# callmeray/PointMVSNet

Hardware: AMD Instinct MI355X
Metric: depth-maps/sec (DTU 640x512, 3 src views, 2 flow iters) (higher is better)
Workload: dtype f32

## Files before the change

include/pointflow_hip.h:

```cpp
#ifndef POINTFLOW_HIP_H_
#define POINTFLOW_HIP_H_

#include <stdint.h>

#ifdef __cplusplus
extern "C" {
#endif

#define PF_OK 0
#define PF_ERR_INVALID_ARG (-1)
#define PF_ERR_UNSUPPORTED (-2)

#define PF_STATUS_BAD_INDEX 1u

#define PF_MAX_VIEWS 8
#define PF_GEMM_TILE 64

#define PF_CAM_KREF_INV 0
#define PF_CAM_RREF_INV 9
#define PF_CAM_TREF 18
#define PF_CAM_MEAN 21
#define PF_CAM_STD 24
#define PF_CAM_VIEWS 27
#define PF_CAM_VIEW_STRIDE 21
#define PF_CAM_FLOATS(V) (PF_CAM_VIEWS + PF_CAM_VIEW_STRIDE * (V))

const char* pf_version(void);
const char* pf_error_string(int code);
int pf_device_info(int* cu_count, int* lds_bytes_per_block, char* arch_host, int arch_len);
int pf_debug_timestamp(long long* slot, void* stream);
int pf_check_status(unsigned* status_host, void* stream);

int pf_gather_knn_forward_f32(const float* feature, const int64_t* index, float* out,
                              int64_t B, int64_t C, int64_t N, int64_t K, void* stream);
int pf_gather_knn_forward_f64(const double* feature, const int64_t* index, double* out,
                              int64_t B, int64_t C, int64_t N, int64_t K, void* stream);
int pf_gather_knn_backward_f32(const float* grad_out, const int64_t* index, float* grad_in,
                               int64_t B, int64_t C, int64_t N, int64_t K, const uint32_t* inv_order,
                               const uint32_t* inv_start, void* stream);
int pf_gather_knn_backward_f64(const double* grad_out, const int64_t* index, double* grad_in,
                               int64_t B, int64_t C, int64_t N, int64_t K, const uint32_t* inv_order,
                               const uint32_t* inv_start, void* stream);

int pf_knn_lattice_f32(const float* xyz, const int64_t* strides_host, int64_t B, int64_t D, int64_t H,
                       int64_t W, int kernel_size, int knn, int64_t* idx_out, uint8_t* code_out,
                       void* stream);

int pf_fetch_forward_f32(const float* maps, const float* pts, const float* K, const float* E, float* out,
                         int64_t B, int64_t V, int64_t C, int64_t H, int64_t W, int64_t N, void* stream);
int pf_fetch_backward_f32(const float* grad_out, const float* pts, const float* K, const float* E,
                          float* grad_maps, int64_t B, int64_t V, int64_t C, int64_t H, int64_t W,
                          int64_t N, void* stream);

int pf_fetch_variance_f32(const float* maps, const float* pts, const float* K, const float* E, float* out,
                          int64_t B, int64_t V, int64_t C, int64_t H, int64_t W, int64_t N,
                          int ref_override, void* stream);
int pf_frustum_variance_f32(const float* maps, const float* kinv, const float* rinv, const float* t,
                            const float* depths, const float* K, const float* E, float* out, float* world,
                            int64_t B, int64_t V, int64_t C, int64_t H, int64_t W, int64_t D, void* stream);

int pf_frustum_variance_cl_f32(const float* maps_cl, const float* kinv, const float* rinv, const float* t,
                               const float* depths, const float* K, const float* E, float* out, float* world,
                               int64_t B, int64_t V, int64_t C, int64_t H, int64_t W, int64_t D, void* stream);
int pf_nchw_to_nhwc_f32(const float* in, float* out, int64_t P, int64_t C, int64_t S, void* stream);

int pf_resize_bilinear_f32(const float* in, float* out, int64_t P, int64_t IH, int64_t IW, int64_t OH,
                           int64_t OW, void* stream);

int pf_flow_pyramid_f32(const float* in1, int c1, int h1, int w1, const float* in2, int c2, int h2, int w2,
                        const float* in3, int c3, int h3, int w3, int V, int h, int w, float* out1, float* out2,
                        float* out3, const float* const* in_scale, const float* const* in_shift, void* stream);

int pf_flow_features_f32(const float* maps1, const float* maps2, const float* maps3, int c1, int c2, int c3,
                         int V, int h, int w, const float* depth_in, int dh, int dw, const float* interval,
                         const float* cam, int ratio, float* feature, float* xyz, void* stream);

int pf_stat_blocks(int G, int Ng);
int pf_gemm_blocks(int G, int Ng);

int pf_bn_finalize_f32(const double* partials, int T, int pcols, int col0, int C, double count,
                       double unbias_n, const float* gamma, const float* beta, float* running_mean,
                       float* running_var, float momentum, float eps, int G, int groups_per_stat,
                       float* scale, float* shift, int ld_affine, void* stream);

typedef struct pf_bn_job {
  const double* partials;
  int32_t T, pcols, col0, C;
  double count, unbias_n;
  const float* gamma;
  const float* beta;
  float* running_mean;
  float* running_var;
  float momentum, eps;
  int32_t G, groups_per_stat;
  float* scale;
  float* shift;
  int32_t ld_affine;
  int32_t rows4;
} pf_bn_job;
int pf_bn_finalize_jobs_f32(const pf_bn_job* jobs, int njobs, void* stream);


int pf_pointwise_gemm_f32(const float* X, int x_point_major, int64_t ldx, const float* Wt, float* Y,
                          int64_t ldy, int G, int Ng, int K, int Nc, int Nc_store, const float* in_scale,
                          const float* in_shift, const pf_bn_job* in_bn, int groups_per_stat, double* col_partials,
                          void* stream);

int pf_edge_stats_f32(const float* LE, int64_t ldle, int C, const int64_t* idx, int k, int G, int Ng,
                      double* partials, const uint8_t* codes, int lat_ks, int lat_h, int lat_w, void* stream);


int pf_edge_apply_f32(const float* LE, int64_t ldle, int C, const int64_t* idx, int k, int G, int Ng,
                      const float* scale, const float* shift, int ld_affine, int groups_per_stat,
                      int concat, float* Y, int64_t ldy, const uint8_t* codes, int lat_ks, int lat_h, int lat_w,
                      void* stream);

int pf_edge_backward_reduce_f32(const float* LE, int64_t ldle, int C, const int64_t* idx, int k, int G, int Ng,
                                const float* grad_y, int64_t ldg, const float* scale, const float* shift,
                                const float* mean, const float* invstd, int ld_affine, int groups_per_stat,
                                int concat, double* partials, void* stream);
int pf_edge_backward_apply_f32(const float* LE, int64_t ldle, int C, const int64_t* idx, int k, int G, int Ng,
                               const float* grad_y, int64_t ldg, const float* scale, const float* shift,
                               const float* mean, const float* invstd, const float* c1, const float* c2,
                               int ld_affine, int groups_per_stat, int concat, float* grad_le,
                               const uint32_t* inv_order, const uint32_t* inv_start, void* stream);

int pf_edge_backward_sums_f32(const float* LE, int64_t ldle, int C, const int64_t* idx, int k, int G, int Ng,
                              const float* grad_y, int64_t ldg, const float* scale, const float* shift,
                              const float* mean, const float* invstd, int ld_affine, int groups_per_stat, int concat,
                              double* partials, float* grad_le, float* grad_acc, int64_t ld_acc, int plane,
                              void* stream);
int pf_edge_backward_finish_f32(const float* LE, int64_t ldle, int C, int k, int G, int Ng, const float* grad_y,
                                int64_t ldg, const float* scale, const float* shift, const float* mean,
                                const float* invstd, const float* c1, const float* c2, int ld_affine,
                                int groups_per_stat, int concat, float* grad_le, const uint32_t* inv_order,
                                const uint32_t* inv_start, int plane, void* stream);

int pf_edge_backward_coeffs_f32(const double* partials, int G, int T, int cbn, int C, int concat, int groups_per_stat,
                                int Ng, int k, float* c1, float* c2, float* dgamma, float* dbeta, int accumulate,
                                void* stream);

int64_t pf_knn_inverse_workspace(int G, int Ng, int k);
int pf_knn_inverse(const int64_t* idx, int k, int G, int Ng, uint32_t* order, uint32_t* start, void* workspace,
                   int64_t workspace_bytes, void* stream);

int pf_norm_blocks(int64_t S);
int pf_channel_stats_f32(const float* x, int64_t N, int64_t C, int64_t S, double* partials, void* stream);
int pf_channel_affine_f32(const float* x, float* y, const float* scale, const float* shift, int64_t N, int64_t C,
                          int64_t S, int samples_per_stat, int relu, void* stream);
int pf_channel_bn_apply_f32(const float* x, float* y, const double* partials, int T, int64_t N, int64_t C, int64_t S,
                            int samples_per_stat, double count, const float* gamma, const float* beta,
                            float* running_mean, float* running_var, float momentum, float eps, int relu,
                            const float* addend, void* stream);
int pf_channel_bn_apply2_f32(const float* x1, const double* partials1, int T1, const float* gamma1, const float* beta1,
                             float* running_mean1, float* running_var1, float momentum1, float eps1, const float* x2,
                             const double* partials2, int T2, const float* gamma2, const float* beta2,
                             float* running_mean2, float* running_var2, float momentum2, float eps2, float* y, int64_t N,
                             int64_t C, int64_t S, int samples_per_stat, double count, void* stream);
int pf_channel_bn_fused_f32(const float* x, float* y, int64_t N, int64_t C, int64_t S, int samples_per_stat,
                            const float* gamma, const float* beta, float* running_mean, float* running_var,
                            float momentum, float eps, int relu, float* scale, float* shift, int ld_affine,
                            void* stream);

int pf_conv3d_blocks(int64_t Cin, int64_t Cout, int64_t Di, int64_t Hi, int64_t Wi, int stride);
int pf_conv3d_k3_f32(const float* x, const float* wp, float* y, int64_t N, int64_t Cin, int64_t Cout, int64_t Di,
                     int64_t Hi, int64_t Wi, int stride, const float* in_scale, const float* in_shift,
                     const pf_bn_job* in_bn, int samples_per_stat, double* partials, void* stream);
int pf_conv3d_pair_blocks(int64_t Cin, int64_t Cout, int64_t D, int64_t H, int64_t W);
int pf_conv3d_k3_pair_f32(const float* x, const float* wp, float* y, int64_t N, int64_t Cin, int64_t Cout, int64_t D,
                          int64_t H, int64_t W, double* partials, void* stream);
int pf_conv3d_k3_few_f32(const float* x, const float* w, float* y, int64_t N, int64_t Cin, int64_t Cout, int64_t D,
                         int64_t H, int64_t W, void* stream);

int pf_deconv3d_blocks(int64_t D, int64_t H, int64_t W);
int pf_deconv3d_k3s2_f32(const float* xa, const float* xb, const float* w, float* y, int64_t N, int64_t Cin,
                         int64_t Cout, int64_t D, int64_t H, int64_t W, const float* in_scale, const float* in_shift,
                         const pf_bn_job* in_bn, int samples_per_stat, double* partials, void* stream);

int pf_conv3d_bottom_supported(int64_t Cin, int64_t Cout, int stride);
int pf_conv3d_bottom_blocks(int64_t Di, int64_t Hi, int64_t Wi, int stride);
int pf_conv3d_bottom_f32(const float* x, const float* wp, float* y, int64_t N, int64_t Cin, int64_t Cout, int64_t Di,
                         int64_t Hi, int64_t Wi, int stride, const float* in_scale, const float* in_shift,
                         const pf_bn_job* in_bn, int samples_per_stat, double* partials, void* stream);
int pf_deconv3d_bottom_supported(int64_t Cin, int64_t Cout);
int pf_deconv3d_bottom_blocks(int64_t Di, int64_t Hi, int64_t Wi);
int pf_deconv3d_bottom_f32(const float* x, const float* wp, float* y, int64_t N, int64_t Cin, int64_t Cout, int64_t Di,
                           int64_t Hi, int64_t Wi, const float* in_scale, const float* in_shift, const pf_bn_job* in_bn,
                           int samples_per_stat, double* partials, void* stream);

int pf_conv2d_wide_supported(int64_t Cin, int64_t Cout, int kernel_size, int stride);
int pf_conv2d_wide_blocks(int64_t Cout, int64_t Hi, int64_t Wi, int stride);
int pf_conv2d_wide_f32(const float* x, const float* wp, float* y, int64_t N, int64_t Cin, int64_t Cout, int64_t Hi,
                       int64_t Wi, int kernel_size, int stride, const float* in_scale, const float* in_shift,
                       const pf_bn_job* in_bn, int samples_per_stat, double* partials, int out_channel_last,
                       void* stream);
int pf_conv2d_wide_sets_f32(const float* x, int x_layout, const float* wp, int64_t wp_set_stride, int sets, float* y,
                            int64_t N, int64_t Cin, int64_t Cout, int64_t Hi, int64_t Wi, int kernel_size, int stride,
                            const float* in_scale, const float* in_shift, const pf_bn_job* in_bn, int samples_per_stat,
                            double* partials, int out_channel_last, void* stream);

int pf_flow_head_f32(const float* Z, int64_t ldz, const float* scale, const float* shift, int ld_affine,
                     const pf_bn_job* in_bn, const float* w_out, const float* depth_in, int dh, int dw,
                     const float* interval, int h, int w, int ratio, float* flow_prob, float* depth_out,
                     void* stream);

int pf_softargmin_prob_f32(const float* cost, const float* params, float* depth, float* prob, int64_t B,
                           int64_t D, int64_t HW, void* stream);

int pf_eval_pack_map_f32(const float* src, float* dst, int h, int w, int flip_rows, void* stream);
int pf_eval_flow_prob_f32(const float* prob, float* dst, int h, int w, int flip_rows, void* stream);
int pf_eval_prob_filter_f32(const float* depth, const float* flow_conf, const float* init_conf, int h, int w, int ih,
                            int iw, float flow_threshold, float init_threshold, float* dst, int flip_rows,
                            void* stream);

#define PF_FUSE_VIEW_FLOATS 12
#define PF_FUSE_PAIR_FLOATS 16
int pf_fuse_stage_a_f32(const float* depth, const unsigned char* colour, const float* view_maps, const float* pair_maps,
                        int V, int h, int w, float disp_threshold, float depth_min, float depth_max, int* count,
                        float* point, unsigned char* colour_out, int* match, void* stream);
int pf_fuse_mark(const int* count, const int* match, unsigned char* used, unsigned char* emit, int V, int view, int h,
                 int w, int num_consistent, void* stream);
int pf_fuse_compact_f32(const unsigned char* emit, const int64_t* rank, const float* point, const unsigned char* colour,
                        int64_t n, int64_t rows, float* out_point, unsigned char* out_colour, void* stream);

#define PF_CLOUD_MAX_CELLS 131072
#define PF_CLOUD_MAX_POINTS 2000000000
int pf_cloud_cell_keys_f32(const float* points, int64_t n, float ox, float oy, float oz, float edge, int nx, int ny, int nz,
                           int64_t* keys, void* stream);
int pf_cloud_pack_f32(const float* points, const int64_t* order, int64_t n, int hashed, void* packed, void* stream);
int pf_cloud_thin_round(const void* packed, const int64_t* keys, int64_t n, int nx, int ny, int nz, float t,
                        const unsigned char* state_in, unsigned char* state_out, int* pending, void* stream);
int pf_cloud_nn_cells_f32(const float* query, int64_t nq, const void* packed, const int64_t* keys, int64_t nt, float ox,
                          float oy, float oz, float edge, int nx, int ny, int nz, int rings, float max_dist, float* dist,
                          int* index, unsigned char* done, void* stream);
int pf_cloud_nn_wave_f32(const float* query, const int64_t* todo, int64_t ntodo, int64_t nq, const void* packed,
                         const int64_t* keys, int64_t nt, float ox, float oy, float oz, float edge, int nx, int ny, int nz,
                         float max_dist, float* dist, int* index, void* stream);
int pf_cloud_obs_mask_f32(const float* points, int64_t n, const unsigned char* mask, int X, int Y, int Z, float bx, float by,
                          float bz, float res, unsigned char* inside, void* stream);
int pf_cloud_above_plane_f32(const float* points, int64_t n, float a, float b, float c, float d, unsigned char* above,
                             void* stream);

#define PF_PREPROCESS_TILE_X 256
int pf_preprocess_resize_u8(const unsigned char* src, int V, int h_src, int w_src, const int* xi, const float* xw,
                            const int* yi, const float* yw, int H, int W, int span, unsigned char* ref,
                            unsigned long long* sums, void* stream);
int pf_preprocess_standardise_f32(const unsigned char* ref, const unsigned long long* sums, int V, int H, int W,
                                  float* out, void* stream);

#define PF_SCAN_NEAREST 0
#define PF_SCAN_BILINEAR 1
#define PF_SCAN_CUBIC 2
#define PF_SCAN_LANCZOS4 4
#define PF_SCAN_FILTER_TILE_X 32
#define PF_SCAN_FILTER_TILE_Y 8
int pf_scan_filter_supported(int mode, int h, int w, int fh, int fw, int ih, int iw);
int pf_scan_filter_f32(const float* depth, const float* flow_prob, const float* flow_conf, int fh, int fw,
                       const float* init_conf, int ih, int iw, int V, int h, int w, int mode, const int* flow_ys,
                       const float* flow_yw, const int* flow_xs, const float* flow_xw, const int* init_ys,
                       const float* init_yw, const int* init_xs, const float* init_xw, float flow_threshold,
                       float init_threshold, float* filtered, int* kept, float* flow_resized, float* init_resized,
                       void* stream);

int pf_bn_train_rows_f32(const double* partials, int T, int pcols, int col0, int C, double count, double unbias_n,
                         const float* gamma, const float* beta, float* running_mean, float* running_var,
                         float momentum, float eps, int G, int groups_per_stat, float* rows, int ld_rows, int col_out,
                         int ch0, void* stream);
int pf_bn_bwd_reduce_f32(const float* g, const float* y, const float* rows, int64_t N, int64_t C, int64_t S,
// ... 100 lines not shown
```

pointmvsnet_amd/_lib.py:

```python
import ctypes
import os

import torch

_HERE = os.path.dirname(os.path.abspath(__file__))
LIB_PATH = os.environ.get("PF_LIB_PATH") or os.path.join(_HERE, "libpointflow_hip.so")

_vp, _i, _i64, _f, _d = ctypes.c_void_p, ctypes.c_int, ctypes.c_int64, ctypes.c_float, ctypes.c_double



class BnJob(ctypes.Structure):
    _fields_ = [("partials", _vp), ("T", ctypes.c_int32), ("pcols", ctypes.c_int32), ("col0", ctypes.c_int32),
                ("C", ctypes.c_int32), ("count", _d), ("unbias_n", _d), ("gamma", _vp), ("beta", _vp),
                ("running_mean", _vp), ("running_var", _vp), ("momentum", _f), ("eps", _f),
                ("G", ctypes.c_int32), ("groups_per_stat", ctypes.c_int32), ("scale", _vp), ("shift", _vp),
                ("ld_affine", ctypes.c_int32), ("rows4", ctypes.c_int32)]


class WgradItem(ctypes.Structure):
    _fields_ = [("gr", _vp), ("x", _vp)] + [(n, _i64) for n in ("N", "Cg", "Cx", "Do", "Ho", "Wo", "Di", "Hi", "Wi")] + \
               [(n, ctypes.c_int32) for n in ("KD", "KH", "KW", "stride", "pd", "ph", "pw", "x_samples_per_stat")] + \
               [("x_scale", _vp), ("x_shift", _vp), ("workspace", _vp), ("workspace_bytes", _i64)] + \
               [(n, _i64) for n in ("rows_P", "ldg", "ldx", "x_rows_per_stat")]


PROTOTYPES = {
    "pf_version": ([], ctypes.c_char_p),
    "pf_error_string": ([_i], ctypes.c_char_p),
    "pf_device_info": ([ctypes.POINTER(_i), ctypes.POINTER(_i), ctypes.c_char_p, _i], _i),
    "pf_debug_timestamp": ([_vp, _vp], _i),
    "pf_check_status": ([ctypes.POINTER(ctypes.c_uint), _vp], _i),
    "pf_gather_knn_forward_f32": ([_vp, _vp, _vp, _i64, _i64, _i64, _i64, _vp], _i),
    "pf_gather_knn_forward_f64": ([_vp, _vp, _vp, _i64, _i64, _i64, _i64, _vp], _i),
    "pf_gather_knn_backward_f32": ([_vp, _vp, _vp, _i64, _i64, _i64, _i64, _vp, _vp, _vp], _i),
    "pf_gather_knn_backward_f64": ([_vp, _vp, _vp, _i64, _i64, _i64, _i64, _vp, _vp, _vp], _i),
    "pf_knn_lattice_f32": ([_vp, ctypes.POINTER(_i64), _i64, _i64, _i64, _i64, _i, _i, _vp, _vp, _vp], _i),
    "pf_fetch_forward_f32": ([_vp, _vp, _vp, _vp, _vp, _i64, _i64, _i64, _i64, _i64, _i64, _vp], _i),
    "pf_fetch_backward_f32": ([_vp, _vp, _vp, _vp, _vp, _i64, _i64, _i64, _i64, _i64, _i64, _vp], _i),
    "pf_fetch_variance_f32": ([_vp, _vp, _vp, _vp, _vp, _i64, _i64, _i64, _i64, _i64, _i64, _i, _vp], _i),
    "pf_frustum_variance_f32": ([_vp, _vp, _vp, _vp, _vp, _vp, _vp, _vp, _vp, _i64, _i64, _i64, _i64, _i64, _i64, _vp], _i),
    "pf_frustum_variance_cl_f32": ([_vp, _vp, _vp, _vp, _vp, _vp, _vp, _vp, _vp, _i64, _i64, _i64, _i64, _i64, _i64, _vp], _i),
    "pf_nchw_to_nhwc_f32": ([_vp, _vp, _i64, _i64, _i64, _vp], _i),
    "pf_resize_bilinear_f32": ([_vp, _vp, _i64, _i64, _i64, _i64, _i64, _vp], _i),
    "pf_flow_pyramid_f32": ([_vp, _i, _i, _i, _vp, _i, _i, _i, _vp, _i, _i, _i, _i, _i, _i, _vp, _vp, _vp,
                             ctypes.POINTER(_vp), ctypes.POINTER(_vp), _vp], _i),
    "pf_flow_features_f32": ([_vp, _vp, _vp, _i, _i, _i, _i, _i, _i, _vp, _i, _i, _vp, _vp, _i, _vp, _vp, _vp], _i),
    "pf_stat_blocks": ([_i, _i], _i),
    "pf_gemm_blocks": ([_i, _i], _i),
    "pf_pointwise_gemm_f32": ([_vp, _i, _i64, _vp, _vp, _i64, _i, _i, _i, _i, _i, _vp, _vp, ctypes.POINTER(BnJob), _i,
                               _vp, _vp], _i),
    "pf_conv3d_blocks": ([_i64, _i64, _i64, _i64, _i64, _i], _i),
    "pf_conv3d_k3_f32": ([_vp, _vp, _vp, _i64, _i64, _i64, _i64, _i64, _i64, _i, _vp, _vp, ctypes.POINTER(BnJob), _i,
                          _vp, _vp], _i),
    "pf_conv3d_pair_blocks": ([_i64, _i64, _i64, _i64, _i64], _i),
    "pf_conv3d_k3_pair_f32": ([_vp, _vp, _vp, _i64, _i64, _i64, _i64, _i64, _i64, _vp, _vp], _i),
    "pf_conv3d_k3_few_f32": ([_vp, _vp, _vp, _i64, _i64, _i64, _i64, _i64, _i64, _vp], _i),
    "pf_deconv3d_blocks": ([_i64, _i64, _i64], _i),
    "pf_deconv3d_k3s2_f32": ([_vp, _vp, _vp, _vp, _i64, _i64, _i64, _i64, _i64, _i64, _vp, _vp, ctypes.POINTER(BnJob), _i,
                              _vp, _vp], _i),
    "pf_conv3d_bottom_supported": ([_i64, _i64, _i], _i),
    "pf_conv3d_bottom_blocks": ([_i64, _i64, _i64, _i], _i),
    "pf_conv3d_bottom_f32": ([_vp, _vp, _vp, _i64, _i64, _i64, _i64, _i64, _i64, _i, _vp, _vp, ctypes.POINTER(BnJob), _i,
                              _vp, _vp], _i),
    "pf_deconv3d_bottom_supported": ([_i64, _i64], _i),
    "pf_deconv3d_bottom_blocks": ([_i64, _i64, _i64], _i),
    "pf_deconv3d_bottom_f32": ([_vp, _vp, _vp, _i64, _i64, _i64, _i64, _i64, _i64, _vp, _vp, ctypes.POINTER(BnJob), _i,
                                _vp, _vp], _i),
    "pf_conv2d_wide_supported": ([_i64, _i64, _i, _i], _i),
    "pf_conv2d_wide_blocks": ([_i64, _i64, _i64, _i], _i),
    "pf_conv2d_wide_f32": ([_vp, _vp, _vp, _i64, _i64, _i64, _i64, _i64, _i, _i, _vp, _vp, ctypes.POINTER(BnJob), _i,
                            _vp, _i, _vp], _i),
    "pf_conv2d_wide_sets_f32": ([_vp, _i, _vp, _i64, _i, _vp, _i64, _i64, _i64, _i64, _i64, _i, _i, _vp, _vp,
                                 ctypes.POINTER(BnJob), _i, _vp, _i, _vp], _i),
    "pf_norm_blocks": ([_i64], _i),
    "pf_channel_stats_f32": ([_vp, _i64, _i64, _i64, _vp, _vp], _i),
    "pf_channel_affine_f32": ([_vp, _vp, _vp, _vp, _i64, _i64, _i64, _i, _i, _vp], _i),
    "pf_channel_bn_apply_f32": ([_vp, _vp, _vp, _i, _i64, _i64, _i64, _i, _d, _vp, _vp, _vp, _vp, _f, _f, _i, _vp, _vp], _i),
    "pf_channel_bn_apply2_f32": ([_vp, _vp, _i, _vp, _vp, _vp, _vp, _f, _f, _vp, _vp, _i, _vp, _vp, _vp, _vp, _f, _f, _vp,
                                  _i64, _i64, _i64, _i, _d, _vp], _i),
    "pf_channel_bn_fused_f32": ([_vp, _vp, _i64, _i64, _i64, _i, _vp, _vp, _vp, _vp, _f, _f, _i, _vp, _vp, _i, _vp], _i),
    "pf_edge_stats_f32": ([_vp, _i64, _i, _vp, _i, _i, _i, _vp, _vp, _i, _i, _i, _vp], _i),
    "pf_edge_backward_reduce_f32": ([_vp, _i64, _i, _vp, _i, _i, _i, _vp, _i64, _vp, _vp, _vp, _vp, _i, _i, _i, _vp, _vp], _i),
    "pf_edge_backward_apply_f32": ([_vp, _i64, _i, _vp, _i, _i, _i, _vp, _i64, _vp, _vp, _vp, _vp, _vp, _vp, _i, _i, _i,
                                    _vp, _vp, _vp, _vp], _i),
    "pf_edge_backward_sums_f32": ([_vp, _i64, _i, _vp, _i, _i, _i, _vp, _i64, _vp, _vp, _vp, _vp, _i, _i, _i, _vp, _vp, _vp,
                                   _i64, _i, _vp], _i),
    "pf_edge_backward_finish_f32": ([_vp, _i64, _i, _i, _i, _i, _vp, _i64, _vp, _vp, _vp, _vp, _vp, _vp, _i, _i, _i,
                                     _vp, _vp, _vp, _i, _vp], _i),
    "pf_knn_inverse_workspace": ([_i, _i, _i], _i64),
    "pf_knn_inverse": ([_vp, _i, _i, _i, _vp, _vp, _vp, _i64, _vp], _i),
    "pf_bn_finalize_f32": ([_vp, _i, _i, _i, _i, _d, _d, _vp, _vp, _vp, _vp, _f, _f, _i, _i, _vp, _vp, _i, _vp], _i),
    "pf_bn_finalize_jobs_f32": ([ctypes.POINTER(BnJob), _i, _vp], _i),
    "pf_edge_apply_f32": ([_vp, _i64, _i, _vp, _i, _i, _i, _vp, _vp, _i, _i, _i, _vp, _i64, _vp, _i, _i, _i, _vp], _i),
    "pf_flow_head_f32": ([_vp, _i64, _vp, _vp, _i, ctypes.POINTER(BnJob), _vp, _vp, _i, _i, _vp, _i, _i, _i, _vp, _vp,
                          _vp], _i),
    "pf_eval_pack_map_f32": ([_vp, _vp, _i, _i, _i, _vp], _i),
    "pf_eval_flow_prob_f32": ([_vp, _vp, _i, _i, _i, _vp], _i),
    "pf_eval_prob_filter_f32": ([_vp, _vp, _vp, _i, _i, _i, _i, _f, _f, _vp, _i, _vp], _i),
    "pf_fuse_stage_a_f32": ([_vp, _vp, _vp, _vp, _i, _i, _i, _f, _f, _f, _vp, _vp, _vp, _vp, _vp], _i),
    "pf_fuse_mark": ([_vp, _vp, _vp, _vp, _i, _i, _i, _i, _i, _vp], _i),
    "pf_fuse_compact_f32": ([_vp, _vp, _vp, _vp, _i64, _i64, _vp, _vp, _vp], _i),
    "pf_cloud_cell_keys_f32": ([_vp, _i64, _f, _f, _f, _f, _i, _i, _i, _vp, _vp], _i),
    "pf_cloud_pack_f32": ([_vp, _vp, _i64, _i, _vp, _vp], _i),
    "pf_cloud_thin_round": ([_vp, _vp, _i64, _i, _i, _i, _f, _vp, _vp, _vp, _vp], _i),
    "pf_cloud_nn_cells_f32": ([_vp, _i64, _vp, _vp, _i64, _f, _f, _f, _f, _i, _i, _i, _i, _f, _vp, _vp, _vp, _vp], _i),
    "pf_cloud_nn_wave_f32": ([_vp, _vp, _i64, _i64, _vp, _vp, _i64, _f, _f, _f, _f, _i, _i, _i, _f, _vp, _vp, _vp], _i),
    "pf_cloud_obs_mask_f32": ([_vp, _i64, _vp, _i, _i, _i, _f, _f, _f, _f, _vp, _vp], _i),
    "pf_cloud_above_plane_f32": ([_vp, _i64, _f, _f, _f, _f, _vp, _vp], _i),
    "pf_preprocess_resize_u8": ([_vp, _i, _i, _i, _vp, _vp, _vp, _vp, _i, _i, _i, _vp, _vp, _vp], _i),
    "pf_preprocess_standardise_f32": ([_vp, _vp, _i, _i, _i, _vp, _vp], _i),
    "pf_scan_filter_supported": ([_i] * 7, _i),
    "pf_scan_filter_f32": ([_vp, _vp, _vp, _i, _i, _vp, _i, _i, _i, _i, _i, _i] + [_vp] * 8 + [_f, _f, _vp, _vp, _vp, _vp, _vp], _i),
    "pf_softargmin_prob_f32": ([_vp, _vp, _vp, _vp, _i64, _i64, _i64, _vp], _i),
    "pf_bn_train_rows_f32": ([_vp, _i, _i, _i, _i, _d, _d, _vp, _vp, _vp, _vp, _f, _f, _i, _i, _vp, _i, _i, _i, _vp], _i),
    "pf_bn_bwd_reduce_f32": ([_vp, _vp, _vp, _i64, _i64, _i64, _i, _i, _vp, _vp], _i),
    "pf_softargmin_backward_f32": ([_vp, _vp, _vp, _vp, _vp, _i64, _i64, _i64, _vp], _i),
    "pf_flow_head_train_f32": ([_vp, _i64, _vp, _vp, _i64, _vp, _vp, _vp], _i),
    "pf_flow_head_backward_workspace": ([_i64], _i64),
    "pf_flow_head_backward_f32": ([_vp, _i64, _vp, _vp, _vp, _vp, _i64, _vp, _vp, _i, _vp, _i64, _vp], _i),
    "pf_rmsprop_f32": ([_vp, _vp, _vp, _vp, _i64, _f, _f, _f, _vp], _i),
    "pf_masked_mae_f32": ([_vp, _vp, _vp, _i, _i, _i, _i, _i, _f, _vp, _vp, _vp], _i),
    "pf_masked_mae_backward_f32": ([_vp, _vp, _vp, _vp, _i, _i, _i, _i, _i, _vp, _vp], _i),
    "pf_wgrad_reduce_batch_f32": ([_vp, _vp, _vp, _vp, _vp, _vp, _vp, _i, _i, _vp], _i),
    "pf_conv_wgrad_batch_f32": ([ctypes.POINTER(WgradItem), _i, _vp], _i),
    "pf_bn_bwd_apply_fused_f32": ([_vp, _vp, _vp, _vp, _i, _d, _vp, _i64, _i64, _i64, _i, _i, _vp, _vp, _i, _vp], _i),
    "pf_bn_bwd_plane_supported": ([_i64, _i], _i),
    "pf_bn_bwd_plane_f32": ([_vp, _vp, _vp, _i64, _i64, _i64, _i, _vp, _vp, _vp, _i, _vp], _i),
    "pf_edge_backward_coeffs_f32": ([_vp, _i, _i, _i, _i, _i, _i, _i, _i, _vp, _vp, _vp, _vp, _i, _vp], _i),
    "pf_bn_bwd_coeffs_f32": ([_vp, _i, _i, _i, _i, _d, _i, _i, _vp, _vp, _vp, _vp, _i, _vp], _i),
    "pf_bn_bwd_apply_f32": ([_vp, _vp, _vp, _vp, _vp, _i64, _i64, _i64, _i, _i, _vp], _i),
    "pf_rows_bn_blocks": ([_i, _i], _i),
    "pf_rows_bn_bwd_reduce_f32": ([_vp, _i64, _vp, _i64, _vp, _i, _i, _i, _i, _i, _vp, _vp], _i),
    "pf_rows_bn_bwd_apply_f32": ([_vp, _i64, _vp, _i64, _vp, _vp, _vp, _i64, _i, _i, _i, _i, _i, _vp], _i),
    "pf_rows_affine_f32": ([_vp, _i64, _vp, _vp, _i64, _i, _i, _i, _i, _i, _vp], _i),
    "pf_conv_wgrad_workspace": ([_i64] * 9 + [_i] * 4, _i64),
    "pf_conv_wgrad_f32": ([_vp, _vp, _vp] + [_i64] * 9 + [_i] * 7 + [_vp, _vp, _i, _vp, _i64, _i, _vp], _i),
    "pf_conv_wgrad_plan": ([_i64] * 9 + [_i] * 4 + [ctypes.POINTER(_i)], _i),
    "pf_rows_wgrad_plan": ([_i64, _i, _i, ctypes.POINTER(_i)], _i),
    "pf_rows_wgrad_workspace": ([_i64, _i, _i], _i64),
    "pf_rows_wgrad_f32": ([_vp, _i64, _vp, _i64, _vp, _i64, _i, _i, _vp, _vp, _i64, _vp, _i64, _i, _vp], _i),
    "pf_deconv2d_k5s2_supported": ([_i64, _i64], _i),
    "pf_deconv2d_k5s2_f32": ([_vp, _vp, _vp, _i64, _i64, _i64, _i64, _i64, _vp], _i),
    "pf_conv3d_k3_c1_f32": ([_vp, _vp, _vp, _i64, _i64, _i64, _i64, _i64, _vp], _i),
    "pf_sort_pairs_workspace": ([_i64, _i64], _i64),
    "pf_sort_pairs_by_key": ([_vp, _i64, _i64, _vp, _vp, _vp, _i64, _vp], _i),
    "pf_warp_taps_flow_f32": ([_vp, _vp, _vp, _i, _i, _i, _vp, _vp, _vp], _i),
    "pf_warp_taps_frustum_f32": ([_vp, _vp, _vp, _vp, _vp, _vp, _i, _i, _i, _i, _i, _vp, _vp, _vp], _i),
    "pf_variance_grad_f32": ([_vp, _i, _vp, _i, _vp, _i, _i, _i, _i, _i64, _vp, _vp, _vp, _i64, _i, _vp, _vp], _i),
    "pf_warp_gather_f32": ([_vp, _vp, _vp, _vp, _i, _i, _i, _i, _i, _vp, _vp], _i),
    "pf_flow_depth_grad_f32": ([_vp, _i64, _i, _vp, _i, _i, _vp, _vp], _i),
    "pf_resize_bilinear_backward_f32": ([_vp, _i, _i, _i, _i, _i, _i, _i, _i, _vp, _vp], _i),
    "pf_pack_desc_bytes": ([], _i),
    "pf_pack_gather_f32": ([_vp, _i, ctypes.c_longlong, _vp], _i),
}

_lib = None


def load():
    global _lib
    if _lib is not None:
        return _lib
    if not os.path.exists(LIB_PATH):
        raise RuntimeError(
            "pointmvsnet_amd: %s is missing. Build it with `python -m pointmvsnet_amd.build` "
            "(hipcc --offload-arch=gfx950). There is no CPU or eager fallback for the hot path." % LIB_PATH)
    try:
        lib = ctypes.CDLL(LIB_PATH)
    except OSError as exc:
        raise RuntimeError("pointmvsnet_amd: cannot load %s: %s" % (LIB_PATH, exc))
    for name, (argtypes, restype) in PROTOTYPES.items():
        fn = getattr(lib, name)
        fn.argtypes = argtypes
        fn.restype = restype
    _lib = lib
    return lib


def check(code, what=""):
    if code != 0:
        msg = load().pf_error_string(int(code)).decode()
        raise RuntimeError("pointflow_hip %s failed (%d): %s" % (what, code, msg))


def ptr(t):
    return None if t is None else ctypes.c_void_p(t.data_ptr())


def stream():
    return ctypes.c_void_p(torch._C._cuda_getCurrentRawStream(torch._C._cuda_getDevice()))


class _NoGuard(object):
    def __enter__(self):
        return None

    def __exit__(self, *exc):
        return False


_NO_GUARD = _NoGuard()


def on_device(dev):
    if dev.index is None or dev.index == torch._C._cuda_getDevice():
        return _NO_GUARD
    return torch.cuda.device(dev)


def require_gpu(*tensors):
    for t in tensors:
        if t is not None and not t.is_cuda:
            raise RuntimeError("pointmvsnet_amd: expected a GPU (HIP) tensor; this operator has no CPU path")


def status():
    val = ctypes.c_uint(0)
    check(load().pf_check_status(ctypes.byref(val), stream()), "pf_check_status")
    return int(val.value)


class KernelTimer(object):

    def __init__(self, only=None):
        self.only = only
        self.records = []

    def wants(self, name):
        return self.only is None or name == self.only

    @staticmethod
    def _pair_overhead_ms():
        vals = []
        for _ in range(21):
# ... 57 lines not shown
```

pointmvsnet_amd/csrc/edgeconv.hip:

```cpp
#include <stdlib.h>

#include "pf_common.h"
#include "pf_bn_resolve.h"

namespace {

typedef float f32x16 __attribute__((ext_vector_type(16)));

constexpr int TILE = PF_GEMM_TILE;

constexpr int GT = 128;
constexpr int LDA = GT + 2;

template <bool POINT_MAJOR, int NT>
__global__ __launch_bounds__(256, 2) void pointwise_gemm_kernel(
    const float* __restrict__ X, int64_t ldx, const float* __restrict__ Wt, float* __restrict__ Y, int64_t ldy,
    int Ng, int K, int Nc_store, const float* __restrict__ in_scale, const float* __restrict__ in_shift,
    int groups_per_stat, double* __restrict__ partials, int T) {
  constexpr int NC = NT * 32;
  constexpr int KC = NT == 4 ? 16 : 32;
  constexpr int NA = KC * GT / 256;
  constexpr int NW = KC * NC / 256;
  __shared__ __attribute__((aligned(16))) float As[2][KC][LDA];
  __shared__ __attribute__((aligned(16))) float Ws[2][KC][NC];
// ... 248 lines not shown
          av[3] = fmaxf(fmaf(av[3], s1.w, s0.w), 0.0f);
        }
#pragma unroll
        for (int i = 0; i < 4; ++i)
#pragma unroll
          for (int t = 0; t < NT; ++t)
            acc[t] = __builtin_amdgcn_mfma_f32_32x32x2f32(av[i], bcur[i][t], acc[t], 0, 0, 0);
#pragma unroll
        for (int i = 0; i < 4; ++i)
#pragma unroll
          for (int t = 0; t < NT; ++t) bcur[i][t] = bnxt[i][t];
        __builtin_amdgcn_sched_barrier(0);
      }
    }
  };

  float4 a0[J0], a1[J1 > 0 ? J1 : 1];
  if (tb < tiles) load_half(row_ptr(tb), a0, 0, J0);
  for (int tile = tb; tile < tiles; tile += T) {
    const int n0 = tile * GT + 32 * wave;
    const int rows = min(32, Ng - n0);
    f32x16 acc[NT];
#pragma unroll
    for (int t = 0; t < NT; ++t)
#pragma unroll
      for (int q = 0; q < 16; ++q) acc[t][q] = 0.0f;
    if (J1 > 0) load_half(row_ptr(tile), a1, J0, J1);
    mma_half(a0, 0, J0, acc);
    if (tile + T < tiles) load_half(row_ptr(tile + T), a0, 0, J0);
    if (J1 > 0) mma_half(a1, J0, J1, acc);
    if (rows > 0) {
      float* yrow = Y + ((int64_t)g * Ng + n0 + 4 * hi) * ldy + lo;
#pragma unroll
      for (int t = 0; t < NT; ++t) {
        const int col = 32 * t + lo;
        float cs = 0.0f, cq = 0.0f;
        if (rows == 32) {
#pragma unroll
          for (int q = 0; q < 16; ++q) {
            const float v = acc[t][q];
            if (col < Nc_store) yrow[(int64_t)((q & 3) + 8 * (q >> 2)) * ldy + 32 * t] = v;
            cs += v;
            cq += v * v;
          }
        } else {
#pragma unroll
          for (int q = 0; q < 16; ++q) {
            const int row = (q & 3) + 8 * (q >> 2) + 4 * hi;
            const float v = acc[t][q];
            if (row < rows) {
              if (col < Nc_store) yrow[(int64_t)((q & 3) + 8 * (q >> 2)) * ldy + 32 * t] = v;
              cs += v;
              cq += v * v;
            }
          }
        }
        csum[t] += (double)cs;
        csq[t] += (double)cq;
      }
    }
  }

  if (partials != nullptr) {
    __syncthreads();
#pragma unroll
    for (int t = 0; t < NT; ++t) {
      double s = csum[t], q = csq[t];
      s += __shfl_xor(s, 32);
      q += __shfl_xor(q, 32);
      if (lane < 32) {
        red[((wave * NC) + 32 * t + lane) * 2 + 0] = s;
        red[((wave * NC) + 32 * t + lane) * 2 + 1] = q;
      }
    }
    __syncthreads();
    if (tid < NC) {
      double s = 0.0, q = 0.0;
#pragma unroll
      for (int w = 0; w < 4; ++w) {
        s += red[((w * NC) + tid) * 2 + 0];
        q += red[((w * NC) + tid) * 2 + 1];
      }
      double* o = partials + (((int64_t)g * T + tb) * NC + tid) * 2;
      o[0] = s;
      o[1] = q;
    }
  }
}

__device__ __forceinline__ float4 ld4(const float* p) { return *reinterpret_cast<const float4*>(p); }

template <int C, int K>
__device__ __forceinline__ void gather_rows(const float* __restrict__ LE, int64_t ldle, const int64_t* __restrict__ ip,
                                            int64_t gbase, int Ng, int q, float4 (&e)[K], bool& bad) {
  long long ii[K];
  static_assert(K % 2 == 0, "K must be even");
#pragma unroll
  for (int j = 0; j < K / 2; ++j) {
    const longlong2 v = *reinterpret_cast<const longlong2*>(ip + 2 * j);
    ii[2 * j] = v.x;
    ii[2 * j + 1] = v.y;
  }
#pragma unroll
  for (int j = 0; j < K; ++j) {
    long long i = ii[j];
    if (i < 0 || i >= Ng) {
      bad = true;
      i = i < 0 ? 0 : Ng - 1;
    }
    e[j] = ld4(LE + (gbase + i) * ldle + C + 4 * q);
  }
}

struct Lattice {
  int ks, H, W;
  int band;
};

__device__ __forceinline__ int xcd_tile(int tb, const Lattice& lat) {
  if (lat.band == 0) return tb;
  const int x = tb & 7, j = tb >> 3;
  const int d = j / lat.band, o = j - d * lat.band;
  return d * (lat.band * 8) + x * lat.band + o;
}

__device__ __forceinline__ void build_code_lut(int* lut, const Lattice& lat) {
  const int hk = lat.ks >> 1, k2 = lat.ks * lat.ks;
  for (int c = threadIdx.x; c < 256; c += blockDim.x) {
    int off = 0;
    if (c < k2 * lat.ks) {
      const int pd = c / k2, rem = c - pd * k2, ph = rem / lat.ks, pw = rem - ph * lat.ks;
      off = (pd - hk) * lat.H * lat.W + (ph - hk) * lat.W + (pw - hk);
    }
    lut[c] = off;
  }
  __syncthreads();
}

template <int C>
__device__ __forceinline__ void gather_rows_codes(const float* __restrict__ LE, int64_t ldle,
                                                  const uint8_t* __restrict__ cp, const int* lut, int64_t gbase, int n,
                                                  int Ng, int q, float4 (&e)[16]) {
  const uint4 cw = *reinterpret_cast<const uint4*>(cp);
  const unsigned w[4] = {cw.x, cw.y, cw.z, cw.w};
#pragma unroll
  for (int j = 0; j < 16; ++j) {
    const int code = (int)((w[j >> 2] >> (8 * (j & 3))) & 255u);
    int i = n + lut[code];
    i = i < 0 ? 0 : (i > Ng - 1 ? Ng - 1 : i);
    e[j] = ld4(LE + (gbase + i) * ldle + C + 4 * q);
  }
}

template <int C, int K>
__global__ __launch_bounds__(256) void edge_stats_kernel(const float* __restrict__ LE, int64_t ldle,
                                                         const int64_t* __restrict__ idx, int k, int Ng,
                                                         double* __restrict__ partials, int T,
                                                         unsigned* __restrict__ status,
                                                         const uint8_t* __restrict__ codes, Lattice lat) {
  constexpr int Q = C / 4;
  constexpr int PPB = 256 / Q;
  __shared__ double red[256 * 8];
  __shared__ int lut[256];
  if (K == 16 && codes != nullptr) build_code_lut(lut, lat);
  const int tid = threadIdx.x;
  const int q = tid % Q, pl = tid / Q;
  const int g = blockIdx.y, tb = blockIdx.x;
  const int tiles = (Ng + TILE - 1) / TILE;
  const int64_t gbase = (int64_t)g * Ng;
  double ds[4] = {0, 0, 0, 0}, dq[4] = {0, 0, 0, 0};
  bool bad = false;
  const int tile0 = xcd_tile(tb, lat);
  for (int tile = tile0; tile < tiles; tile += T) {
    const int n0 = tile * TILE;
    for (int p = pl; p < TILE; p += PPB) {
      const int n = n0 + p;
      if (n >= Ng) break;
      const int64_t row = gbase + n;
      const float4 l = ld4(LE + row * ldle + 4 * q);
      const int64_t* ip = idx + row * k;
      float4 s = {0, 0, 0, 0}, s2 = {0, 0, 0, 0};
      if constexpr (K > 0) {
        float4 e[K > 0 ? K : 1];
        if constexpr (K == 16) {
          if (codes != nullptr) gather_rows_codes<C>(LE, ldle, codes + row * 16, lut, gbase, n, Ng, q, e);
          else gather_rows<C, 16>(LE, ldle, ip, gbase, Ng, q, e, bad);
        } else {
          gather_rows<C, (K > 0 ? K : 2)>(LE, ldle, ip, gbase, Ng, q, e, bad);
        }
#pragma unroll
        for (int j = 0; j < K; ++j) {
          const float dx = e[j].x - l.x, dy = e[j].y - l.y, dz = e[j].z - l.z, dw = e[j].w - l.w;
          s.x += dx; s.y += dy; s.z += dz; s.w += dw;
          s2.x += dx * dx; s2.y += dy * dy; s2.z += dz * dz; s2.w += dw * dw;
        }
      } else {
        for (int j = 0; j < k; ++j) {
          int64_t i = ip[j];
          if (i < 0 || i >= Ng) {
            bad = true;
            i = i < 0 ? 0 : Ng - 1;
          }
          const float4 e = ld4(LE + (gbase + i) * ldle + C + 4 * q);
          const float dx = e.x - l.x, dy = e.y - l.y, dz = e.z - l.z, dw = e.w - l.w;
          s.x += dx; s.y += dy; s.z += dz; s.w += dw;
          s2.x += dx * dx; s2.y += dy * dy; s2.z += dz * dz; s2.w += dw * dw;
        }
      }
      ds[0] += (double)s.x; ds[1] += (double)s.y; ds[2] += (double)s.z; ds[3] += (double)s.w;
      dq[0] += (double)s2.x; dq[1] += (double)s2.y; dq[2] += (double)s2.z; dq[3] += (double)s2.w;
    }
  }
  if (bad) atomicOr(status, PF_STATUS_BAD_INDEX);
#pragma unroll
  for (int c = 0; c < 4; ++c) {
    red[tid * 8 + c] = ds[c];
    red[tid * 8 + 4 + c] = dq[c];
  }
  __syncthreads();
  if (tid < 2 * C) {
    const int qq = tid / 8, comp = tid % 8;
    double acc = 0.0;
    for (int s = 0; s < PPB; ++s) acc += red[(s * Q + qq) * 8 + comp];
    double* o = partials + (((int64_t)g * T + tile0) * C + 4 * qq + (comp & 3)) * 2 + (comp >> 2);
    *o = acc;
  }
}

template <int C, int K>
__global__ __launch_bounds__(256) void edge_apply_kernel(const float* __restrict__ LE, int64_t ldle,
                                                         const int64_t* __restrict__ idx, int k, int Ng,
                                                         const float* __restrict__ scale,
                                                         const float* __restrict__ shift, int ld_affine,
                                                         int groups_per_stat, int concat, float* __restrict__ Y,
                                                         int64_t ldy, int T, const uint8_t* __restrict__ codes,
                                                         Lattice lat) {
  constexpr int Q = C / 4;
  constexpr int PPB = 256 / Q;
  __shared__ int lut[256];
  if (K == 16 && codes != nullptr) build_code_lut(lut, lat);
  const int tid = threadIdx.x;
  const int q = tid % Q, pl = tid / Q;
  const int g = blockIdx.y, tb = blockIdx.x;
  const int tiles = (Ng + TILE - 1) / TILE;
  const int64_t gbase = (int64_t)g * Ng;
  const int64_t so = (int64_t)(g / groups_per_stat) * ld_affine;
  const int doff = concat ? C : 0;
  const float4 dsc = ld4(scale + so + doff + 4 * q), dsh = ld4(shift + so + doff + 4 * q);
  float4 csc = {0, 0, 0, 0}, csh = {0, 0, 0, 0};
  if (concat) {
    csc = ld4(scale + so + 4 * q);
    csh = ld4(shift + so + 4 * q);
  }
  const float kf = (float)k;
  bool bad = false;
  for (int tile = xcd_tile(tb, lat); tile < tiles; tile += T) {
    const int n0 = tile * TILE;
    for (int p = pl; p < TILE; p += PPB) {
      const int n = n0 + p;
      if (n >= Ng) break;
      const int64_t row = gbase + n;
      const float4 l = ld4(LE + row * ldle + 4 * q);
      const int64_t* ip = idx + row * k;
      float4 a = {0, 0, 0, 0};
      if constexpr (K > 0) {
        float4 e[K > 0 ? K : 1];
        if constexpr (K == 16) {
          if (codes != nullptr) gather_rows_codes<C>(LE, ldle, codes + row * 16, lut, gbase, n, Ng, q, e);
          else gather_rows<C, 16>(LE, ldle, ip, gbase, Ng, q, e, bad);
        } else {
          gather_rows<C, (K > 0 ? K : 2)>(LE, ldle, ip, gbase, Ng, q, e, bad);
        }
#pragma unroll
        for (int j = 0; j < K; ++j) {
          a.x += fmaxf(fmaf(e[j].x - l.x, dsc.x, dsh.x), 0.0f);
          a.y += fmaxf(fmaf(e[j].y - l.y, dsc.y, dsh.y), 0.0f);
          a.z += fmaxf(fmaf(e[j].z - l.z, dsc.z, dsh.z), 0.0f);
          a.w += fmaxf(fmaf(e[j].w - l.w, dsc.w, dsh.w), 0.0f);
        }
      } else {
        for (int j = 0; j < k; ++j) {
          int64_t i = ip[j];
          i = i < 0 ? 0 : (i >= Ng ? Ng - 1 : i);
          const float4 e = ld4(LE + (gbase + i) * ldle + C + 4 * q);
          a.x += fmaxf(fmaf(e.x - l.x, dsc.x, dsh.x), 0.0f);
          a.y += fmaxf(fmaf(e.y - l.y, dsc.y, dsh.y), 0.0f);
          a.z += fmaxf(fmaf(e.z - l.z, dsc.z, dsh.z), 0.0f);
          a.w += fmaxf(fmaf(e.w - l.w, dsc.w, dsh.w), 0.0f);
        }
      }
      float4 yd = {a.x / kf, a.y / kf, a.z / kf, a.w / kf};
      float* yo = Y + row * ldy + 4 * q;
      if (concat) {
        float4 yc = {fmaxf(fmaf(l.x, csc.x, csh.x), 0.0f), fmaxf(fmaf(l.y, csc.y, csh.y), 0.0f),
                     fmaxf(fmaf(l.z, csc.z, csh.z), 0.0f), fmaxf(fmaf(l.w, csc.w, csh.w), 0.0f)};
        *reinterpret_cast<float4*>(yo) = yc;
        *reinterpret_cast<float4*>(yo + C) = yd;
      } else {
        *reinterpret_cast<float4*>(yo) = yd;
      }
    }
  }
  (void)bad;
}

struct EdgeBwdAffine {
  const float* scale;
  const float* shift;
  const float* mean;
  const float* invstd;
  const float* c1;
  const float* c2;
  int ld, groups_per_stat, concat;
};

template <int C, int K, bool SUMS>
__global__ __launch_bounds__(256) void edge_bwd_reduce_kernel(const float* __restrict__ LE, int64_t ldle,
                                                              const int64_t* __restrict__ idx, int k, int Ng,
                                                              const float* __restrict__ Gy, int64_t ldg,
                                                              EdgeBwdAffine A, double* __restrict__ partials, int T,
                                                              unsigned* __restrict__ status, float* __restrict__ sums,
                                                              float* __restrict__ gacc, int64_t lda, int band) {
  constexpr int Q = C / 4;
  constexpr int PPB = 256 / Q;
  __shared__ double red[256 * 16];
  const int tid = threadIdx.x;
  const int q = tid % Q, pl = tid / Q;
  const int g = blockIdx.y, tb = blockIdx.x;
  const int tiles = (Ng + TILE - 1) / TILE;
  const int64_t gbase = (int64_t)g * Ng;
  const int64_t so = (int64_t)(g / A.groups_per_stat) * A.ld;
  const int doff = A.concat ? C : 0;
  const float4 a = ld4(A.scale + so + doff + 4 * q), b = ld4(A.shift + so + doff + 4 * q);
  const float4 mu = ld4(A.mean + so + doff + 4 * q), is = ld4(A.invstd + so + doff + 4 * q);
  float4 ac = {0, 0, 0, 0}, bc = {0, 0, 0, 0}, muc = {0, 0, 0, 0}, isc = {0, 0, 0, 0};
  if (A.concat) {
    ac = ld4(A.scale + so + 4 * q);
    bc = ld4(A.shift + so + 4 * q);
    muc = ld4(A.mean + so + 4 * q);
    isc = ld4(A.invstd + so + 4 * q);
  }
  const float kf = (float)k;
  double acc[16];
#pragma unroll
  for (int i = 0; i < 16; ++i) acc[i] = 0.0;
  bool bad = false;
  const Lattice xo{0, 1, 1, band};
  const int tile0 = xcd_tile(tb, xo);
  for (int tile = tile0; tile < tiles; tile += T) {
    const int n0 = tile * TILE;
    for (int p = pl; p < TILE; p += PPB) {
      const int n = n0 + p;
      if (n >= Ng) break;
      const int64_t row = gbase + n;
      const float4 l = ld4(LE + row * ldle + 4 * q);
      float4 gy = ld4(Gy + row * ldg + doff + 4 * q);
      if (SUMS && gacc != nullptr) {
        float* ga = gacc + row * lda + doff + 4 * q;
        const float4 h = ld4(ga);
        gy = make_float4(gy.x + h.x, gy.y + h.y, gy.z + h.z, gy.w + h.w);
        *reinterpret_cast<float4*>(ga) = gy;
      }
      const float gd[4] = {gy.x / kf, gy.y / kf, gy.z / kf, gy.w / kf};
      const float lv[4] = {l.x, l.y, l.z, l.w};
      const float av[4] = {a.x, a.y, a.z, a.w}, bv[4] = {b.x, b.y, b.z, b.w};
      const float mv[4] = {mu.x, mu.y, mu.z, mu.w}, iv[4] = {is.x, is.y, is.z, is.w};
      float sg[4] = {0, 0, 0, 0}, sx[4] = {0, 0, 0, 0}, sd[4] = {0, 0, 0, 0};
      const int64_t* ip = idx + row * k;
      auto pair = [&](const float4& e) {
        const float ev[4] = {e.x, e.y, e.z, e.w};
#pragma unroll
        for (int c = 0; c < 4; ++c) {
          const float d = ev[c] - lv[c];
          const float u = fmaf(d, av[c], bv[c]);
          const float gg = u > 0.0f ? gd[c] : 0.0f;
          sg[c] += gg;
          sx[c] += gg * ((d - mv[c]) * iv[c]);
          if (SUMS) sd[c] += d;
        }
      };
      if constexpr (K > 0) {
        float4 e[K > 0 ? K : 1];
        gather_rows<C, (K > 0 ? K : 2)>(LE, ldle, ip, gbase, Ng, q, e, bad);
#pragma unroll
        for (int j = 0; j < K; ++j) pair(e[j]);
      } else {
        for (int j = 0; j < k; ++j) {
          int64_t i = ip[j];
          if (i < 0 || i >= Ng) {
            bad = true;
            i = i < 0 ? 0 : Ng - 1;
          }
          pair(ld4(LE + (gbase + i) * ldle + C + 4 * q));
        }
      }
#pragma unroll
      for (int c = 0; c < 4; ++c) {
        acc[c] += (double)sg[c];
        acc[4 + c] += (double)sx[c];
      }
      if (SUMS) {
        float* o = sums + row * ldle + 4 * q;
        *reinterpret_cast<float4*>(o) = make_float4(sg[0], sg[1], sg[2], sg[3]);
        *reinterpret_cast<float4*>(o + C) = make_float4((sd[0] - kf * mv[0]) * iv[0], (sd[1] - kf * mv[1]) * iv[1],
                                                        (sd[2] - kf * mv[2]) * iv[2], (sd[3] - kf * mv[3]) * iv[3]);
      }
      if (A.concat) {
        float4 gc4 = ld4(Gy + row * ldg + 4 * q);
        if (SUMS && gacc != nullptr) {
          float* ga = gacc + row * lda + 4 * q;
          const float4 h = ld4(ga);
// ... 447 lines not shown
  const float interval = interval_p[0];
#pragma unroll
  for (int d = 0; d < 5; ++d) {
    const float p = e[d] / den;
    flow_prob[(int64_t)d * h * w + i] = p;
    flow += p * ((float)(d - 2) * interval);
  }
  const float scy = (float)dh / (float)h, scx = (float)dw / (float)w;
  int sy = (int)floorf((float)y * scy);
  int sx = (int)floorf((float)x * scx);
  sy = sy > dh - 1 ? dh - 1 : sy;
  sx = sx > dw - 1 ? dw - 1 : sx;
  depth_out[i] = depth_in[sy * dw + sx] + flow;
}

}

extern "C" {

int pf_stat_blocks(int G, int Ng) {
  if (G <= 0 || Ng <= 0) return 0;
  const int tiles = (Ng + TILE - 1) / TILE;
#ifndef PF_STAT_CAP
#define PF_STAT_CAP 4096
#endif
  int cap = PF_STAT_CAP / G;
  cap = cap < 32 ? 32 : cap;
  if (tiles <= cap) return tiles;
  const int per = (tiles + cap - 1) / cap;
  return (tiles + per - 1) / per;
}

int pf_gemm_blocks(int G, int Ng) {
  if (G <= 0 || Ng <= 0) return 0;
  const int tiles = (Ng + GT - 1) / GT;
#ifndef PF_GEMM_CAP
#define PF_GEMM_CAP 512
#endif
  int cap = PF_GEMM_CAP / G;
  cap = cap < 16 ? 16 : cap;
  if (tiles <= cap) return tiles;
  const int per = (tiles + cap - 1) / cap;
  return (tiles + per - 1) / per;
}

static int bn_materialize_rows(const pf_bn_job* in_bn, hipStream_t s) {
  PF_REQUIRE(in_bn->scale != nullptr && in_bn->shift != nullptr && in_bn->ld_affine >= in_bn->C);
  pf_bn_job j = *in_bn;
  j.running_mean = j.running_var = nullptr;
  return pf_bn_finalize_jobs_f32(&j, 1, s);
}

int pf_pointwise_gemm_f32(const float* X, int x_point_major, int64_t ldx, const float* Wt, float* Y, int64_t ldy,
                          int G, int Ng, int K, int Nc, int Nc_store, const float* in_scale,
                          const float* in_shift, const pf_bn_job* in_bn, int groups_per_stat, double* col_partials,
                          void* stream) {
  PF_REQUIRE(in_bn == nullptr || in_scale == nullptr);
  if (in_bn != nullptr && G > 0 && Ng > 0) {
    PF_REQUIRE(groups_per_stat >= 1 && G % groups_per_stat == 0);
    const int rc = pf_bn_in_check(in_bn, K, G / groups_per_stat);
    if (rc != PF_OK && rc != PF_ERR_UNSUPPORTED) return rc;
    const int kj = (K + 7) / 8, nt = Nc / 32;
    const bool shape = (kj == 17 && nt == 2) || (kj == 4 && nt == 2) || (kj == 8 && nt == 4) || (kj == 28 && nt == 2) ||
                       (kj == 8 && nt == 2) || (kj == 8 && nt == 1);
    const bool direct = rc == PF_OK && shape && x_point_major && (K % 4) == 0 && (ldx % 4) == 0 &&
                        kj * 8 * Nc <= 16384 && (reinterpret_cast<uintptr_t>(X) % 16) == 0 && K <= 256;
    if (!direct) {
      const int rc2 = bn_materialize_rows(in_bn, (hipStream_t)stream);
      if (rc2 != PF_OK) return rc2;
      PF_REQUIRE(in_bn->ld_affine == K);
      return pf_pointwise_gemm_f32(X, x_point_major, ldx, Wt, Y, ldy, G, Ng, K, Nc, Nc_store, in_bn->scale,
                                   in_bn->shift, nullptr, groups_per_stat, col_partials, stream);
    }
  }
  PF_REQUIRE(G >= 0 && Ng >= 0 && K >= 1 && Nc >= 32 && Nc_store >= 1 && Nc_store <= Nc);
  PF_REQUIRE(Nc % 32 == 0 && groups_per_stat >= 1);
  if (Nc != 32 && Nc != 64 && Nc != 128) return PF_ERR_UNSUPPORTED;
  PF_REQUIRE((in_scale == nullptr) == (in_shift == nullptr));
  PF_REQUIRE(G <= 65535);
  if (G == 0 || Ng == 0) return PF_OK;
  PF_REQUIRE(X && Wt && Y && ldy >= Nc_store);
  if (x_point_major) PF_REQUIRE(ldx >= K);
  const int T = pf_gemm_blocks(G, Ng);
  dim3 grid((unsigned)T, (unsigned)G);
  hipStream_t s = (hipStream_t)stream;
  {
    const pf_bn_job no_bn = {};
    const int kj = (K + 7) / 8, nt = Nc / 32;
    const bool direct = x_point_major && (K % 4) == 0 && (ldx % 4) == 0 && kj * 8 * Nc <= 16384 &&
                        (reinterpret_cast<uintptr_t>(X) % 16) == 0;
#define PF_GEMM_DIRECT(KJV, NTV)                                                                                   \
  if (direct && kj == KJV && nt == NTV) {                                                                          \
    if (in_bn != nullptr)                                                                                          \
      hipLaunchKernelGGL((pointwise_gemm_direct_kernel<KJV, NTV, 2>), grid, dim3(256), 0, s, X, ldx, Wt, Y, ldy,   \
                         Ng, K, Nc_store, in_scale, in_shift, groups_per_stat, col_partials, T, *in_bn);           \
    else if (in_scale != nullptr)                                                                                  \
      hipLaunchKernelGGL((pointwise_gemm_direct_kernel<KJV, NTV, 1>), grid, dim3(256), 0, s, X, ldx, Wt, Y, ldy,   \
                         Ng, K, Nc_store, in_scale, in_shift, groups_per_stat, col_partials, T, no_bn);            \
    else                                                                                                           \
      hipLaunchKernelGGL((pointwise_gemm_direct_kernel<KJV, NTV, 0>), grid, dim3(256), 0, s, X, ldx, Wt, Y, ldy,   \
                         Ng, K, Nc_store, in_scale, in_shift, groups_per_stat, col_partials, T, no_bn);            \
    return pf_launch_status();                                                                                     \
  }
    PF_GEMM_DIRECT(17, 2)
    PF_GEMM_DIRECT(4, 2)
    PF_GEMM_DIRECT(8, 4)
    PF_GEMM_DIRECT(28, 2)
    PF_GEMM_DIRECT(8, 2)
    PF_GEMM_DIRECT(8, 1)
#undef PF_GEMM_DIRECT
  }
#define PF_GEMM_LAUNCH(PM, NTV)                                                                                  \
  hipLaunchKernelGGL((pointwise_gemm_kernel<PM, NTV>), grid, dim3(256), 0, s, X, ldx, Wt, Y, ldy, Ng, K, Nc_store, \
                     in_scale, in_shift, groups_per_stat, col_partials, T)
  if (x_point_major) {
    if (Nc == 32) PF_GEMM_LAUNCH(true, 1);
    else if (Nc == 64) PF_GEMM_LAUNCH(true, 2);
    else PF_GEMM_LAUNCH(true, 4);
  } else {
    if (Nc == 32) PF_GEMM_LAUNCH(false, 1);
    else if (Nc == 64) PF_GEMM_LAUNCH(false, 2);
    else PF_GEMM_LAUNCH(false, 4);
  }
#undef PF_GEMM_LAUNCH
  return pf_launch_status();
}

static int check_lattice(const int64_t* idx, const uint8_t* codes, int k, int Ng, int lat_ks, int lat_h, int lat_w,
                         Lattice& lat) {
  lat.ks = 0;
  lat.H = lat.W = 1;
  lat.band = 0;
  if (codes == nullptr) {
    PF_REQUIRE(idx != nullptr);
    if (lat_ks == 0 && lat_h >= 1 && lat_w >= 1 && (int64_t)lat_h * lat_w > 1 && Ng % ((int64_t)lat_h * lat_w) == 0) {
      lat.H = lat_h;
      lat.W = lat_w;
    }
    return PF_OK;
  }
  PF_REQUIRE(k == 16 && (lat_ks == 3 || lat_ks == 5) && lat_h >= 1 && lat_w >= 1);
  PF_REQUIRE(Ng % (lat_h * lat_w) == 0);
  lat.ks = lat_ks;
  lat.H = lat_h;
  lat.W = lat_w;
  return PF_OK;
}

static int xcd_band(int64_t plane, int unit, int64_t Ng, int64_t blocks) {
  static const bool on = !(getenv("PF_EDGE_XCD") && atoi(getenv("PF_EDGE_XCD")) == 0);
  if (!on || plane <= 1 || plane % unit != 0 || (plane / unit) % 8 != 0 || Ng % plane != 0 || blocks != Ng / unit) return 0;
  return (int)(plane / unit / 8);
}
static void lattice_band(Lattice& lat, int Ng, int T) { lat.band = xcd_band((int64_t)lat.H * lat.W, TILE, Ng, T); }

int pf_edge_stats_f32(const float* LE, int64_t ldle, int C, const int64_t* idx, int k, int G, int Ng,
                      double* partials, const uint8_t* codes, int lat_ks, int lat_h, int lat_w, void* stream) {
  PF_REQUIRE(G >= 0 && Ng >= 0 && k >= 1 && ldle >= 2 * (int64_t)C && (ldle % 4) == 0 && G <= 65535);
  if (C != 32 && C != 64 && C != 128) return PF_ERR_UNSUPPORTED;
  if (G == 0 || Ng == 0) return PF_OK;
  PF_REQUIRE(LE && partials);
  Lattice lat;
  {
    const int rc = check_lattice(idx, codes, k, Ng, lat_ks, lat_h, lat_w, lat);
    if (rc != PF_OK) return rc;
  }
  unsigned* status = pf_status_ptr();
  PF_REQUIRE(status != nullptr);
  const int T = pf_stat_blocks(G, Ng);
  lattice_band(lat, Ng, T);
  dim3 grid((unsigned)T, (unsigned)G);
  hipStream_t s = (hipStream_t)stream;
#define PF_ES(CV, KV) hipLaunchKernelGGL((edge_stats_kernel<CV, KV>), grid, dim3(256), 0, s, LE, ldle, idx, k, Ng, partials, T, status, codes, lat)
  if (k == 16) {
    if (C == 32) PF_ES(32, 16); else if (C == 64) PF_ES(64, 16); else PF_ES(128, 16);
  } else {
    if (C == 32) PF_ES(32, 0); else if (C == 64) PF_ES(64, 0); else PF_ES(128, 0);
  }
#undef PF_ES
  return pf_launch_status();
}

int pf_bn_finalize_jobs_f32(const pf_bn_job* jobs, int njobs, void* stream) {
  PF_REQUIRE(jobs != nullptr && njobs >= 1 && njobs <= kBnJobs);
  BnJobs packed;
  int cmax = 0;
  for (int i = 0; i < njobs; ++i) {
    const pf_bn_job& j = jobs[i];
    PF_REQUIRE(j.T >= 1 && j.pcols >= 1 && j.col0 >= 0 && j.C >= 1 && j.col0 + j.C <= j.pcols && j.count > 0.0);
    PF_REQUIRE(j.G >= 1 && j.groups_per_stat >= 1 && (j.G % j.groups_per_stat) == 0 && j.ld_affine >= j.C);
    PF_REQUIRE(j.partials && j.gamma && j.beta && j.scale && j.shift);
    PF_REQUIRE((j.running_mean == nullptr) == (j.running_var == nullptr));
    packed.j[i] = j;
    cmax = j.C > cmax ? j.C : cmax;
  }
  for (int i = njobs; i < kBnJobs; ++i) packed.j[i] = jobs[0];
  const int cb = bn_channels_per_block();
  hipLaunchKernelGGL(bn_finalize_kernel, dim3((unsigned)pf_cdiv(cmax, cb), (unsigned)njobs), dim3(kBnThreads), 0,
                     (hipStream_t)stream, packed, cb);
  return pf_launch_status();
}

int pf_bn_finalize_f32(const double* partials, int T, int pcols, int col0, int C, double count, double unbias_n,
                       const float* gamma, const float* beta, float* running_mean, float* running_var,
                       float momentum, float eps, int G, int groups_per_stat, float* scale, float* shift,
                       int ld_affine, void* stream) {
  pf_bn_job j;
  j.partials = partials;
  j.T = T;
  j.pcols = pcols;
  j.col0 = col0;
  j.C = C;
  j.count = count;
  j.unbias_n = unbias_n;
  j.gamma = gamma;
  j.beta = beta;
  j.running_mean = running_mean;
  j.running_var = running_var;
  j.momentum = momentum;
  j.eps = eps;
  j.G = G;
  j.groups_per_stat = groups_per_stat;
  j.scale = scale;
  j.shift = shift;
  j.ld_affine = ld_affine;
  j.rows4 = 0;
  return pf_bn_finalize_jobs_f32(&j, 1, stream);
}

int pf_edge_apply_f32(const float* LE, int64_t ldle, int C, const int64_t* idx, int k, int G, int Ng,
                      const float* scale, const float* shift, int ld_affine, int groups_per_stat, int concat,
                      float* Y, int64_t ldy, const uint8_t* codes, int lat_ks, int lat_h, int lat_w, void* stream) {
  PF_REQUIRE(G >= 0 && Ng >= 0 && k >= 1 && ldle >= 2 * (int64_t)C && (ldle % 4) == 0 && G <= 65535);
  PF_REQUIRE(groups_per_stat >= 1 && (ldy % 4) == 0 && ldy >= (concat ? 2 : 1) * (int64_t)C);
  PF_REQUIRE((ld_affine % 4) == 0 && ld_affine >= (concat ? 2 : 1) * C);
  if (C != 32 && C != 64 && C != 128) return PF_ERR_UNSUPPORTED;
  if (G == 0 || Ng == 0) return PF_OK;
  PF_REQUIRE(LE && scale && shift && Y);
  Lattice lat;
  {
    const int rc = check_lattice(idx, codes, k, Ng, lat_ks, lat_h, lat_w, lat);
    if (rc != PF_OK) return rc;
  }
  const int T = pf_stat_blocks(G, Ng);
  lattice_band(lat, Ng, T);
  dim3 grid((unsigned)T, (unsigned)G);
  hipStream_t s = (hipStream_t)stream;
#define PF_EA(CV, KV)                                                                                         \
  hipLaunchKernelGGL((edge_apply_kernel<CV, KV>), grid, dim3(256), 0, s, LE, ldle, idx, k, Ng, scale, shift, \
                     ld_affine, groups_per_stat, concat, Y, ldy, T, codes, lat)
  if (k == 16) {
    if (C == 32) PF_EA(32, 16); else if (C == 64) PF_EA(64, 16); else PF_EA(128, 16);
  } else {
    if (C == 32) PF_EA(32, 0); else if (C == 64) PF_EA(64, 0); else PF_EA(128, 0);
  }
#undef PF_EA
  return pf_launch_status();
}

extern "C++" {
static int edge_backward_reduce(const float* LE, int64_t ldle, int C, const int64_t* idx, int k, int G, int Ng,
                                const float* grad_y, int64_t ldg, const float* scale, const float* shift,
                                const float* mean, const float* invstd, int ld_affine, int groups_per_stat,
                                int concat, double* partials, float* sums, float* gacc, int64_t lda, int plane,
                                void* stream) {
  PF_REQUIRE(G >= 0 && Ng >= 0 && k >= 1 && ldle >= 2 * (int64_t)C && (ldle % 4) == 0 && G <= 65535);
  PF_REQUIRE(gacc == nullptr || (sums != nullptr && (lda % 4) == 0 && lda >= (concat ? 2 : 1) * (int64_t)C));
  PF_REQUIRE(groups_per_stat >= 1 && (ldg % 4) == 0 && ldg >= (concat ? 2 : 1) * (int64_t)C);
  PF_REQUIRE((ld_affine % 4) == 0 && ld_affine >= (concat ? 2 : 1) * C);
  if (C != 32 && C != 64) return PF_ERR_UNSUPPORTED;
  if (G == 0 || Ng == 0) return PF_OK;
  PF_REQUIRE(LE && idx && grad_y && scale && shift && mean && invstd && partials);
  unsigned* status = pf_status_ptr();
  PF_REQUIRE(status != nullptr);
  const EdgeBwdAffine A{scale, shift, mean, invstd, nullptr, nullptr, ld_affine, groups_per_stat, concat};
  const int T = pf_stat_blocks(G, Ng);
  const int band = xcd_band(plane, TILE, Ng, T);
  dim3 grid((unsigned)T, (unsigned)G);
  hipStream_t s = (hipStream_t)stream;
#define PF_EBR(CV, KV, SV) hipLaunchKernelGGL((edge_bwd_reduce_kernel<CV, KV, SV>), grid, dim3(256), 0, s, LE, ldle, idx, k, Ng, grad_y, ldg, A, partials, T, status, sums, gacc, lda, band)
  if (sums != nullptr) {
    if (k == 16) {
      if (C == 32) PF_EBR(32, 16, true); else PF_EBR(64, 16, true);
    } else {
      if (C == 32) PF_EBR(32, 0, true); else PF_EBR(64, 0, true);
    }
  } else if (k == 16) {
    if (C == 32) PF_EBR(32, 16, false); else PF_EBR(64, 16, false);
  } else {
    if (C == 32) PF_EBR(32, 0, false); else PF_EBR(64, 0, false);
  }
#undef PF_EBR
  return pf_launch_status();
}
}

int pf_edge_backward_reduce_f32(const float* LE, int64_t ldle, int C, const int64_t* idx, int k, int G, int Ng,
                                const float* grad_y, int64_t ldg, const float* scale, const float* shift,
                                const float* mean, const float* invstd, int ld_affine, int groups_per_stat,
                                int concat, double* partials, void* stream) {
  return edge_backward_reduce(LE, ldle, C, idx, k, G, Ng, grad_y, ldg, scale, shift, mean, invstd, ld_affine,
                              groups_per_stat, concat, partials, nullptr, nullptr, 0, 0, stream);
}

int pf_edge_backward_sums_f32(const float* LE, int64_t ldle, int C, const int64_t* idx, int k, int G, int Ng,
                              const float* grad_y, int64_t ldg, const float* scale, const float* shift,
                              const float* mean, const float* invstd, int ld_affine, int groups_per_stat, int concat,
                              double* partials, float* grad_le, float* grad_acc, int64_t ld_acc, int plane,
                              void* stream) {
  PF_REQUIRE(grad_le != nullptr || G == 0 || Ng == 0);
  PF_REQUIRE(plane >= 0);
  return edge_backward_reduce(LE, ldle, C, idx, k, G, Ng, grad_y, ldg, scale, shift, mean, invstd, ld_affine,
                              groups_per_stat, concat, partials, grad_le, grad_acc, ld_acc, plane, stream);
}

extern "C++" {
template <bool FINISH>
static void edge_backward_inverse_launch(const float* LE, int64_t ldle, int C, int k, int G, int Ng, const float* grad_y,
                                         int64_t ldg, const EdgeBwdAffine& A, const uint32_t* inv_order,
                                         const uint32_t* inv_start, float* grad_le, int plane, hipStream_t s) {
  const int64_t rows = (int64_t)G * Ng;
  const int ppb = 256 / (C / 4);
  int64_t blocks = pf_cdiv(rows, ppb);
  if (blocks > 16384) blocks = 16384;
  const int band = G == 1 ? xcd_band(plane, ppb, Ng, blocks) : 0;
  static const int dbg = getenv("PF_EDGE_FINISH_DBG") ? atoi(getenv("PF_EDGE_FINISH_DBG")) : 0;
  if (C == 32)
    hipLaunchKernelGGL((edge_bwd_inverse_kernel<32, FINISH>), dim3((unsigned)blocks), dim3(256), 0, s, LE, ldle, k, Ng,
                       grad_y, ldg, A, inv_order, inv_start, grad_le, rows, dbg, band);
  else
    hipLaunchKernelGGL((edge_bwd_inverse_kernel<64, FINISH>), dim3((unsigned)blocks), dim3(256), 0, s, LE, ldle, k, Ng,
                       grad_y, ldg, A, inv_order, inv_start, grad_le, rows, dbg, band);
}
}

int pf_edge_backward_apply_f32(const float* LE, int64_t ldle, int C, const int64_t* idx, int k, int G, int Ng,
                               const float* grad_y, int64_t ldg, const float* scale, const float* shift,
                               const float* mean, const float* invstd, const float* c1, const float* c2,
                               int ld_affine, int groups_per_stat, int concat, float* grad_le,
                               const uint32_t* inv_order, const uint32_t* inv_start, void* stream) {
  PF_REQUIRE(G >= 0 && Ng >= 0 && k >= 1 && ldle >= 2 * (int64_t)C && (ldle % 4) == 0 && G <= 65535);
  PF_REQUIRE((inv_order == nullptr) == (inv_start == nullptr));
  PF_REQUIRE(groups_per_stat >= 1 && (ldg % 4) == 0 && ldg >= (concat ? 2 : 1) * (int64_t)C);
  PF_REQUIRE((ld_affine % 4) == 0 && ld_affine >= (concat ? 2 : 1) * C);
  if (C != 32 && C != 64) return PF_ERR_UNSUPPORTED;
  if (G == 0 || Ng == 0) return PF_OK;
  PF_REQUIRE(LE && idx && grad_y && scale && shift && mean && invstd && c1 && c2 && grad_le);
  hipStream_t s = (hipStream_t)stream;
  const bool scatter = inv_order == nullptr;
  if (scatter) {
    const int zrc = pf_zero_async(grad_le, sizeof(float) * (size_t)G * Ng * ldle, s);
    if (zrc != PF_OK) return zrc;
  }
  const EdgeBwdAffine A{scale, shift, mean, invstd, c1, c2, ld_affine, groups_per_stat, concat};
  const int T = pf_stat_blocks(G, Ng);
  dim3 grid((unsigned)T, (unsigned)G);
#define PF_EBA(CV, KV, SV) hipLaunchKernelGGL((edge_bwd_apply_kernel<CV, KV, SV>), grid, dim3(256), 0, s, LE, ldle, idx, k, Ng, grad_y, ldg, A, grad_le, T)
  if (scatter) {
    if (k == 16) {
      if (C == 32) PF_EBA(32, 16, true); else PF_EBA(64, 16, true);
    } else {
      if (C == 32) PF_EBA(32, 0, true); else PF_EBA(64, 0, true);
    }
    return pf_launch_status();
  }
  if (k == 16) {
    if (C == 32) PF_EBA(32, 16, false); else PF_EBA(64, 16, false);
  } else {
    if (C == 32) PF_EBA(32, 0, false); else PF_EBA(64, 0, false);
  }
#undef PF_EBA
  edge_backward_inverse_launch<false>(LE, ldle, C, k, G, Ng, grad_y, ldg, A, inv_order, inv_start, grad_le, 0, s);
  return pf_launch_status();
}

int pf_edge_backward_finish_f32(const float* LE, int64_t ldle, int C, int k, int G, int Ng, const float* grad_y,
                                int64_t ldg, const float* scale, const float* shift, const float* mean,
                                const float* invstd, const float* c1, const float* c2, int ld_affine,
                                int groups_per_stat, int concat, float* grad_le, const uint32_t* inv_order,
                                const uint32_t* inv_start, int plane, void* stream) {
  PF_REQUIRE(G >= 0 && Ng >= 0 && k >= 1 && ldle >= 2 * (int64_t)C && (ldle % 4) == 0 && G <= 65535 && plane >= 0);
  PF_REQUIRE(groups_per_stat >= 1 && (ldg % 4) == 0 && ldg >= (concat ? 2 : 1) * (int64_t)C);
  PF_REQUIRE((ld_affine % 4) == 0 && ld_affine >= (concat ? 2 : 1) * C);
  if (C != 32 && C != 64) return PF_ERR_UNSUPPORTED;
  if (G == 0 || Ng == 0) return PF_OK;
  PF_REQUIRE(LE && grad_y && scale && shift && mean && invstd && c1 && c2 && grad_le && inv_order && inv_start);
  const EdgeBwdAffine A{scale, shift, mean, invstd, c1, c2, ld_affine, groups_per_stat, concat};
  edge_backward_inverse_launch<true>(LE, ldle, C, k, G, Ng, grad_y, ldg, A, inv_order, inv_start, grad_le, plane,
                                     (hipStream_t)stream);
  return pf_launch_status();
}

int pf_flow_head_f32(const float* Z, int64_t ldz, const float* scale, const float* shift, int ld_affine,
                     const pf_bn_job* in_bn, const float* w_out, const float* depth_in, int dh, int dw,
                     const float* interval, int h, int w, int ratio, float* flow_prob, float* depth_out,
                     void* stream) {
  PF_REQUIRE(h >= 1 && w >= 1 && dh >= 1 && dw >= 1 && ratio >= 1 && h % ratio == 0 && w % ratio == 0);
  PF_REQUIRE(ldz >= 16 && (ldz % 4) == 0 && (int64_t)h * w <= INT32_MAX);
  PF_REQUIRE(Z && w_out && depth_in && interval && flow_prob && depth_out);
  PF_REQUIRE((in_bn != nullptr) != (scale != nullptr) && (scale == nullptr) == (shift == nullptr));
  dim3 grid((unsigned)pf_cdiv((int64_t)h * w, 256));
  hipStream_t s = (hipStream_t)stream;
  if (in_bn != nullptr) {
// ... 24 lines not shown
```

pointmvsnet_amd/csrc/fetch.hip:

```cpp
#include <type_traits>

#include <stdlib.h>

#include "pf_common.h"

namespace {

__global__ __launch_bounds__(256) void fetch_fwd_kernel(const float* __restrict__ maps,
                                                        const float* __restrict__ pts,
                                                        const float* __restrict__ Kmat,
                                                        const float* __restrict__ Emat, float* __restrict__ out,
                                                        int V, int C, int H, int W, int64_t N) {
  const int64_t n = (int64_t)blockIdx.x * blockDim.x + threadIdx.x;
  const int v = blockIdx.y;
  const int64_t b = blockIdx.z;
  if (n >= N) return;
  const float* pb = pts + b * 3 * N;
  PfTaps t;
  pf_project_taps(pb[n], pb[N + n], pb[2 * N + n], Kmat + (b * V + v) * 9,
                  Emat ? Emat + (b * V + v) * 12 : nullptr, H, W, t);
  const int64_t HW = (int64_t)H * W;
  const float* m = maps + (b * V + v) * C * HW;
  float* o = out + (b * V + v) * C * N + n;
  for (int c = 0; c < C; ++c) o[(int64_t)c * N] = pf_sample(m + (int64_t)c * HW, t);
}

__global__ __launch_bounds__(256) void fetch_bwd_kernel(const float* __restrict__ gout,
                                                        const float* __restrict__ pts,
                                                        const float* __restrict__ Kmat,
                                                        const float* __restrict__ Emat,
                                                        float* __restrict__ gmaps, int V, int C, int H, int W,
                                                        int64_t N) {
  const int64_t n = (int64_t)blockIdx.x * blockDim.x + threadIdx.x;
  const int v = blockIdx.y;
  const int64_t b = blockIdx.z;
  if (n >= N) return;
  const float* pb = pts + b * 3 * N;
  PfTaps t;
  pf_project_taps(pb[n], pb[N + n], pb[2 * N + n], Kmat + (b * V + v) * 9,
                  Emat ? Emat + (b * V + v) * 12 : nullptr, H, W, t);
  const int64_t HW = (int64_t)H * W;
  float* gm = gmaps + (b * V + v) * C * HW;
  const float* g = gout + (b * V + v) * C * N + n;
  for (int c = 0; c < C; ++c) {
    const float go = g[(int64_t)c * N];
    float* plane = gm + (int64_t)c * HW;
#pragma unroll
    for (int k = 0; k < 4; ++k)
      if (t.ok[k]) unsafeAtomicAdd(plane + t.off[k], go * t.wgt[k]);
  }
}

__device__ __forceinline__ float pf_bilerp(float a, float b, float c, float d, float w0, float w1, float w2, float w3) {
  return fmaf(d, w3, fmaf(c, w2, fmaf(b, w1, a * w0)));
}
__device__ __forceinline__ float pf_variance(float s, float s2, float inv_v) {
  const float m1 = s * inv_v;
  return fmaf(-m1, m1, s2 * inv_v);
}

struct Frustum {
  const float* kinv;
  const float* rinv;
  const float* t;
  const float* depths;
  float* world;
  int D;
};

template <int V, bool FRUSTUM>
__global__ __launch_bounds__(256) void fetch_variance_kernel(const float* __restrict__ maps,
                                                             const float* __restrict__ pts, Frustum fr,
                                                             const float* __restrict__ Kmat,
                                                             const float* __restrict__ Emat,
                                                             float* __restrict__ out, int C, int H, int W,
                                                             int64_t N, int ref_override) {
  const int64_t n = (int64_t)blockIdx.x * blockDim.x + threadIdx.x;
  const int64_t b = blockIdx.y;
  if (n >= N) return;
  float X, Y, Z;
  if (FRUSTUM) {
    const int hw = H * W;
    const int d = (int)(n / hw);
    const int pix = (int)(n - (int64_t)d * hw);
    const int py = pix / W, px = pix - py * W;
    const float gx = (float)px + 0.5f, gy = (float)py + 0.5f;
    const float* ki = fr.kinv + b * 9;
    const float* ri = fr.rinv + b * 9;
    const float* tt = fr.t + b * 3;
    const float depth = fr.depths[b * fr.D + d];
    const float u0 = fmaf(ki[2], 1.0f, fmaf(ki[1], gy, ki[0] * gx));
    const float u1 = fmaf(ki[5], 1.0f, fmaf(ki[4], gy, ki[3] * gx));
    const float u2 = fmaf(ki[8], 1.0f, fmaf(ki[7], gy, ki[6] * gx));
    const float c0 = u0 * depth - tt[0], c1 = u1 * depth - tt[1], c2 = u2 * depth - tt[2];
    X = fmaf(ri[2], c2, fmaf(ri[1], c1, ri[0] * c0));
    Y = fmaf(ri[5], c2, fmaf(ri[4], c1, ri[3] * c0));
    Z = fmaf(ri[8], c2, fmaf(ri[7], c1, ri[6] * c0));
    if (fr.world != nullptr) {
      float* wb = fr.world + b * 3 * N;
      wb[n] = X;
      wb[N + n] = Y;
      wb[2 * N + n] = Z;
    }
  } else {
    const float* pb = pts + b * 3 * N;
    X = pb[n];
    Y = pb[N + n];
    Z = pb[2 * N + n];
  }
  PfTaps t[V];
#pragma unroll
  for (int v = 0; v < V; ++v)
    pf_project_taps(X, Y, Z, Kmat + (b * V + v) * 9, Emat ? Emat + (b * V + v) * 12 : nullptr, H, W, t[v]);
  const int64_t HW = (int64_t)H * W;
  const int ref_off = (int)(n % HW);
  const float* mb = maps + b * V * C * HW;
  float* o = out + b * C * N + n;
#pragma unroll 2
  for (int c = 0; c < C; ++c) {
    float s = 0.0f, s2 = 0.0f;
#pragma unroll
    for (int v = 0; v < V; ++v) {
      const float* plane = mb + ((int64_t)v * C + c) * HW;
      const float f = (v == 0 && ref_override)
                          ? plane[ref_off]
                          : pf_bilerp(plane[t[v].off[0]], plane[t[v].off[1]], plane[t[v].off[2]], plane[t[v].off[3]],
                                      t[v].wgt[0], t[v].wgt[1], t[v].wgt[2], t[v].wgt[3]);
      if (v == 0) {
        s = f;
        s2 = f * f;
      } else {
        s = s + f;
        s2 = fmaf(f, f, s2);
      }
    }
    o[(int64_t)c * N] = pf_variance(s, s2, 1.0f / (float)V);
  }
}

__global__ __launch_bounds__(256) void nchw_to_nhwc_kernel(const float* __restrict__ in, float* __restrict__ out,
                                                           int C, int64_t S) {
  __shared__ float tile[64][65];
  const int64_t p = blockIdx.z;
  const int64_t s0 = (int64_t)blockIdx.x * 64;
  const int c0 = blockIdx.y * 64;
  const int tx = threadIdx.x & 63, ty = threadIdx.x >> 6;
  for (int r = ty; r < 64; r += 4) {
    const int c = c0 + r;
    const int64_t s = s0 + tx;
    tile[r][tx] = (c < C && s < S) ? in[(p * C + c) * S + s] : 0.0f;
  }
  __syncthreads();
  for (int r = ty; r < 64; r += 4) {
    const int64_t s = s0 + r;
    const int c = c0 + tx;
    if (s < S && c < C) out[(p * S + s) * C + c] = tile[tx][r];
  }
}

template <int V>
__global__ __launch_bounds__(256) void frustum_variance_cl_kernel(const float* __restrict__ maps, Frustum fr,
                                                                  const float* __restrict__ Kmat,
                                                                  const float* __restrict__ Emat,
                                                                  float* __restrict__ out, int C, int H, int W,
                                                                  int64_t N) {
  constexpr int PTS = 64;
  __shared__ float tile[64 + 3][PTS + 1];
  const int q = threadIdx.x & 15, pl = threadIdx.x >> 4;
  const int64_t b = blockIdx.y;
  const int hw = H * W;
  unsigned ptile = blockIdx.x;
  if ((PF_XCD & PF_XCD_FRUSTUM) != 0 && hw % PTS == 0 && (int64_t)gridDim.x * PTS == N && (gridDim.x & 7u) == 0u)
    ptile = pf_xcd_band(ptile, (unsigned)(hw / PTS));
  const int64_t n0 = (int64_t)ptile * PTS;
  const float* ki = fr.kinv + b * 9;
  const float* ri = fr.rinv + b * 9;
  const float* tt = fr.t + b * 3;
  const float* mb = maps + b * V * (int64_t)hw * C;
  for (int c0 = 0; c0 < C; c0 += 64) {
#pragma unroll 1
    for (int pass = 0; pass < PTS / 16; ++pass) {
      const int p = pass * 16 + pl;
      int64_t n = n0 + p;
      n = n < N ? n : N - 1;
      const int d = (int)(n / hw);
      const int pix = (int)(n - (int64_t)d * hw);
      const int py = pix / W, px = pix - py * W;
      const float gx = (float)px + 0.5f, gy = (float)py + 0.5f;
      const float depth = fr.depths[b * fr.D + d];
      const float u0 = fmaf(ki[2], 1.0f, fmaf(ki[1], gy, ki[0] * gx));
      const float u1 = fmaf(ki[5], 1.0f, fmaf(ki[4], gy, ki[3] * gx));
      const float u2 = fmaf(ki[8], 1.0f, fmaf(ki[7], gy, ki[6] * gx));
      const float q0 = u0 * depth - tt[0], q1 = u1 * depth - tt[1], q2 = u2 * depth - tt[2];
      const float X = fmaf(ri[2], q2, fmaf(ri[1], q1, ri[0] * q0));
      const float Y = fmaf(ri[5], q2, fmaf(ri[4], q1, ri[3] * q0));
      const float Z = fmaf(ri[8], q2, fmaf(ri[7], q1, ri[6] * q0));
      if (c0 == 0 && q < 3) tile[64 + q][p] = q == 0 ? X : (q == 1 ? Y : Z);
      PfTaps t[V];
      if (V > 1) {
        const int vq = 1 + (q % (V > 1 ? V - 1 : 1));
        PfTaps mine;
        pf_project_taps(X, Y, Z, Kmat + (b * V + vq) * 9, Emat ? Emat + (b * V + vq) * 12 : nullptr, H, W, mine);
#pragma unroll
        for (int v = 1; v < V; ++v) {
#pragma unroll
          for (int k = 0; k < 4; ++k) {
            t[v].off[k] = __shfl(mine.off[k], v - 1, 16);
            t[v].wgt[k] = __shfl(mine.wgt[k], v - 1, 16);
          }
        }
      }
      const int c = c0 + 4 * q;
      if (c < C) {
        const float4 r0 = *reinterpret_cast<const float4*>(mb + (int64_t)pix * C + c);
        float s[4] = {r0.x, r0.y, r0.z, r0.w};
        float s2[4] = {r0.x * r0.x, r0.y * r0.y, r0.z * r0.z, r0.w * r0.w};
#pragma unroll
        for (int v = 1; v < V; ++v) {
          const float* mv = mb + (int64_t)v * hw * C + c;
          const float4 a = *reinterpret_cast<const float4*>(mv + (int64_t)t[v].off[0] * C);
          const float4 bb = *reinterpret_cast<const float4*>(mv + (int64_t)t[v].off[1] * C);
          const float4 cc = *reinterpret_cast<const float4*>(mv + (int64_t)t[v].off[2] * C);
          const float4 dd = *reinterpret_cast<const float4*>(mv + (int64_t)t[v].off[3] * C);
          const float w0 = t[v].wgt[0], w1 = t[v].wgt[1], w2 = t[v].wgt[2], w3 = t[v].wgt[3];
          const float f[4] = {pf_bilerp(a.x, bb.x, cc.x, dd.x, w0, w1, w2, w3), pf_bilerp(a.y, bb.y, cc.y, dd.y, w0, w1, w2, w3),
                              pf_bilerp(a.z, bb.z, cc.z, dd.z, w0, w1, w2, w3), pf_bilerp(a.w, bb.w, cc.w, dd.w, w0, w1, w2, w3)};
#pragma unroll
          for (int i = 0; i < 4; ++i) {
            s[i] = s[i] + f[i];
            s2[i] = fmaf(f[i], f[i], s2[i]);
          }
        }
#pragma unroll
        for (int i = 0; i < 4; ++i) tile[4 * q + i][p] = pf_variance(s[i], s2[i], 1.0f / (float)V);
      }
    }
    __syncthreads();
    const int tx = threadIdx.x & 63, ty = threadIdx.x >> 6;
    const bool inb = n0 + tx < N;
    const int rows = min(64, C - c0);
    for (int r = ty; r < rows; r += 4)
      if (inb) out[(b * C + c0 + r) * N + n0 + tx] = tile[r][tx];
    if (c0 == 0 && fr.world != nullptr && ty < 3 && inb) fr.world[(b * 3 + ty) * N + n0 + tx] = tile[64 + ty][tx];
    __syncthreads();
  }
}

__device__ __forceinline__ void resize_axis(int o, float scale, int in_size, int& i0, int& i1, float& l0,
                                            float& l1) {
  float src = scale * ((float)o + 0.5f) - 0.5f;
  src = src < 0.0f ? 0.0f : src;
  i0 = (int)src;
  if (i0 > in_size - 1) i0 = in_size - 1;
  i1 = i0 + ((i0 < in_size - 1) ? 1 : 0);
  l1 = fminf(fmaxf(src - (float)i0, 0.0f), 1.0f);
  l0 = 1.0f - l1;
}

__global__ __launch_bounds__(256) void resize_bilinear_kernel(const float* __restrict__ in,
                                                              float* __restrict__ out, int IH, int IW, int OH,
                                                              int OW, float sy, float sx) {
  const int64_t p = blockIdx.y;
  const int i = blockIdx.x * blockDim.x + threadIdx.x;
  if (i >= OH * OW) return;
  const int oy = i / OW, ox = i - oy * OW;
  const float* src = in + p * IH * IW;
  float v;
  if (IH == OH && IW == OW) {
    v = src[i];
  } else {
    int y0, y1, x0, x1;
    float ly0, ly1, lx0, lx1;
    resize_axis(oy, sy, IH, y0, y1, ly0, ly1);
    resize_axis(ox, sx, IW, x0, x1, lx0, lx1);
    const float a = src[y0 * IW + x0], b = src[y0 * IW + x1];
    const float c = src[y1 * IW + x0], d = src[y1 * IW + x1];
    v = ly0 * (lx0 * a + lx1 * b) + ly1 * (lx0 * c + lx1 * d);
  }
  out[p * OH * OW + i] = v;
}

struct PyramidLevel {
  const float* in;
  float* out;
  const float* scale;
  const float* shift;
  int C, IH, IW;
};
struct Pyramid {
  PyramidLevel l[3];
};

__global__ __launch_bounds__(256) void pyramid_resize_kernel(Pyramid py, int V, int OH, int OW, int cq_max) {
  const PyramidLevel L = py.l[blockIdx.z];
  const int v = blockIdx.y / cq_max, cq = blockIdx.y - v * cq_max;
  const int i = blockIdx.x * blockDim.x + threadIdx.x;
  if (4 * cq >= L.C || i >= OH * OW) return;
  const int oy = i / OW, ox = i - oy * OW;
  const int plane = L.IH * L.IW;
  const float* src = L.in + ((int64_t)v * L.C + 4 * cq) * plane;
  float r[4];
  float sc[4] = {1.0f, 1.0f, 1.0f, 1.0f}, sh[4] = {0.0f, 0.0f, 0.0f, 0.0f};
  const bool aff = L.scale != nullptr;
  if (aff) {
#pragma unroll
    for (int c = 0; c < 4; ++c) {
      sc[c] = L.scale[(int64_t)v * L.C + 4 * cq + c];
      sh[c] = L.shift[(int64_t)v * L.C + 4 * cq + c];
    }
  }
  auto act = [&](float x, int c) { return aff ? fmaxf(fmaf(x, sc[c], sh[c]), 0.0f) : x; };
  if (L.IH == OH && L.IW == OW) {
#pragma unroll
    for (int c = 0; c < 4; ++c) r[c] = act(src[(int64_t)c * plane + i], c);
  } else {
    int y0, y1, x0, x1;
    float ly0, ly1, lx0, lx1;
    resize_axis(oy, (float)L.IH / (float)OH, L.IH, y0, y1, ly0, ly1);
    resize_axis(ox, (float)L.IW / (float)OW, L.IW, x0, x1, lx0, lx1);
#pragma unroll
    for (int c = 0; c < 4; ++c) {
      const float* pc = src + (int64_t)c * plane;
      const float a = act(pc[y0 * L.IW + x0], c), b = act(pc[y0 * L.IW + x1], c);
      const float cc = act(pc[y1 * L.IW + x0], c), d = act(pc[y1 * L.IW + x1], c);
      r[c] = ly0 * (lx0 * a + lx1 * b) + ly1 * (lx0 * cc + lx1 * d);
    }
  }
  *reinterpret_cast<float4*>(L.out + ((int64_t)v * OH * OW + i) * L.C + 4 * cq) = make_float4(r[0], r[1], r[2], r[3]);
}

constexpr int kFeatLanes = 8;
constexpr int kFeatPY = 4, kFeatPX = 8;
static_assert(kFeatPY * kFeatPX * kFeatLanes == 256, "one point per 8 lanes");

template <int V, bool ROLLV>
__global__ __launch_bounds__(256) void flow_features_hyp_kernel(const float* __restrict__ maps1,
                                                                const float* __restrict__ maps2,
                                                                const float* __restrict__ maps3, int c1, int c2,
                                                                int c3, int h, int w,
                                                                const float* __restrict__ depth_in, int dh, int dw,
                                                                const float* __restrict__ interval_p,
                                                                const float* __restrict__ cam, int ratio,
                                                                float* __restrict__ feature, float* __restrict__ xyz) {
  constexpr int PTS = kFeatPY * kFeatPX;
  constexpr int kUnrollV = ROLLV ? 1 : V;
  __shared__ int tap_off[PTS][V * 5][4];
  __shared__ float tap_wgt[PTS][V * 5][4];
  __shared__ float nxyz[PTS][5][4];
  const int hs = h / ratio, ws = w / ratio;
  const int64_t Ng = (int64_t)5 * hs * ws;
  const int q = threadIdx.x & (kFeatLanes - 1);
  const int pl = threadIdx.x / kFeatLanes;
  const int tiles_x = (w + kFeatPX - 1) / kFeatPX;
  const unsigned blk = (PF_XCD & PF_XCD_FETCH) ? pf_xcd_chunk(blockIdx.x, gridDim.x) : blockIdx.x;
  const int bx = (int)blk % tiles_x, by = (int)blk / tiles_x;
  const int y_raw = by * kFeatPY + pl / kFeatPX, x_raw = bx * kFeatPX + pl % kFeatPX;
  const bool live = y_raw < h && x_raw < w;
  const int y = live ? y_raw : h - 1, x = live ? x_raw : w - 1;
  const int g = (y % ratio) * ratio + (x % ratio);
  const int64_t loc0 = (int64_t)(y / ratio) * ws + x / ratio;

  const float scy = (float)dh / (float)h, scx = (float)dw / (float)w;
  int sy = (int)floorf((float)y * scy);
  int sx = (int)floorf((float)x * scx);
  sy = sy > dh - 1 ? dh - 1 : sy;
  sx = sx > dw - 1 ? dw - 1 : sx;
  const float depth0 = depth_in[sy * dw + sx];
  const float interval = interval_p[0];
  const float* Ki = cam + PF_CAM_KREF_INV;
  const float* Ri = cam + PF_CAM_RREF_INV;
  const float* t0 = cam + PF_CAM_TREF;
  const float px = (float)x + 0.5f, py = (float)y + 0.5f;
  const float u0 = fmaf(Ki[2], 1.0f, fmaf(Ki[1], py, Ki[0] * px));
  const float u1 = fmaf(Ki[5], 1.0f, fmaf(Ki[4], py, Ki[3] * px));
  const float u2 = fmaf(Ki[8], 1.0f, fmaf(Ki[7], py, Ki[6] * px));
  auto world = [&](int d, float& X, float& Y, float& Z) {
    const float depth = depth0 + interval * (float)(d - 2);
    const float q0 = u0 * depth - t0[0], q1 = u1 * depth - t0[1], q2 = u2 * depth - t0[2];
    X = fmaf(Ri[2], q2, fmaf(Ri[1], q1, Ri[0] * q0));
    Y = fmaf(Ri[5], q2, fmaf(Ri[4], q1, Ri[3] * q0));
    Z = fmaf(Ri[8], q2, fmaf(Ri[7], q1, Ri[6] * q0));
  };
  for (int p = q; p < V * 5; p += kFeatLanes) {
    const int v = p / 5, d = p - v * 5;
    float X, Y, Z;
    world(d, X, Y, Z);
    PfTaps t;
    const float* cv = cam + PF_CAM_VIEWS + v * PF_CAM_VIEW_STRIDE;
    pf_project_taps(X, Y, Z, cv, cv + 9, h, w, t);
#pragma unroll
    for (int k = 0; k < 4; ++k) {
      tap_off[pl][p][k] = t.off[k];
      tap_wgt[pl][p][k] = t.wgt[k];
    }
  }
  if (q < 5) {
    float X, Y, Z;
    world(q, X, Y, Z);
    const float nx = (X - cam[PF_CAM_MEAN + 0]) / cam[PF_CAM_STD + 0];
    const float ny = (Y - cam[PF_CAM_MEAN + 1]) / cam[PF_CAM_STD + 1];
    const float nz = (Z - cam[PF_CAM_MEAN + 2]) / cam[PF_CAM_STD + 2];
    nxyz[pl][q][0] = nx;
    nxyz[pl][q][1] = ny;
    nxyz[pl][q][2] = nz;
    if (live) {
      float* xo = xyz + (int64_t)g * 3 * Ng + (int64_t)q * hs * ws + loc0;
      xo[0] = nx;
      xo[Ng] = ny;
      xo[2 * Ng] = nz;
    }
  }
  __syncthreads();

  const int ctot = c1 + c2 + c3 + 24;
  float* frow0 = feature + ((int64_t)g * Ng + loc0) * ctot;
  const int64_t dstride = (int64_t)hs * ws * ctot;
  const int64_t hw = (int64_t)h * w;
  int ch = 0;
#pragma unroll 1
  for (int level = 0; level < 3; ++level) {
    const float* maps = level == 0 ? maps1 : (level == 1 ? maps2 : maps3);
    const int cl = level == 0 ? c1 : (level == 1 ? c2 : c3);
#pragma unroll 1
    for (int c0 = 0; c0 < cl; c0 += 4 * kFeatLanes) {
      const int c = c0 + 4 * q;
      if (c < cl) {
        float s[5][4], s2[5][4];
#pragma unroll
        for (int d = 0; d < 5; ++d)
#pragma unroll
          for (int i = 0; i < 4; ++i) s[d][i] = s2[d][i] = 0.0f;
#pragma unroll kUnrollV
        for (int v = 0; v < V; ++v) {
          const float* mv = maps + (int64_t)v * hw * cl + c;
#pragma unroll
          for (int d = 0; d < 5; ++d) {
            const int4 o = *reinterpret_cast<const int4*>(&tap_off[pl][v * 5 + d][0]);
            const float4 wg = *reinterpret_cast<const float4*>(&tap_wgt[pl][v * 5 + d][0]);
            const float4 a = *reinterpret_cast<const float4*>(mv + (int64_t)o.x * cl);
            const float4 b = *reinterpret_cast<const float4*>(mv + (int64_t)o.y * cl);
            const float4 cc = *reinterpret_cast<const float4*>(mv + (int64_t)o.z * cl);
            const float4 dd = *reinterpret_cast<const float4*>(mv + (int64_t)o.w * cl);
            const float f[4] = {pf_bilerp(a.x, b.x, cc.x, dd.x, wg.x, wg.y, wg.z, wg.w),
                                pf_bilerp(a.y, b.y, cc.y, dd.y, wg.x, wg.y, wg.z, wg.w),
                                pf_bilerp(a.z, b.z, cc.z, dd.z, wg.x, wg.y, wg.z, wg.w),
                                pf_bilerp(a.w, b.w, cc.w, dd.w, wg.x, wg.y, wg.z, wg.w)};
#pragma unroll
            for (int i = 0; i < 4; ++i) {
              s[d][i] = s[d][i] + f[i];
              s2[d][i] = fmaf(f[i], f[i], s2[d][i]);
            }
          }
        }
        if (live) {
#pragma unroll
          for (int d = 0; d < 5; ++d) {
            float o[4];
// ... 56 lines not shown
  __syncthreads();
  if (q != 0 || !ok) return;
  acc = ((sh[0][lane] + sh[1][lane]) + sh[2][lane]) + sh[3][lane];
  depth[b * HW + i] = acc;
  const float fi = (acc - start) / interval;
  float lo = floorf(fi), hi = ceilf(fi);
  lo = fminf(fmaxf(lo, 0.0f), (float)(D - 1));
  hi = fminf(fmaxf(hi, 0.0f), (float)(D - 1));
  const float plo = expf(-c[(int64_t)(int)lo * HW] - mx) / den;
  const float phi = expf(-c[(int64_t)(int)hi * HW] - mx) / den;
  prob[b * HW + i] = plo + phi;
}

template <typename F>
int dispatch_views(int V, F&& f) {
  switch (V) {
    case 1: return f(std::integral_constant<int, 1>());
    case 2: return f(std::integral_constant<int, 2>());
    case 3: return f(std::integral_constant<int, 3>());
    case 4: return f(std::integral_constant<int, 4>());
    case 5: return f(std::integral_constant<int, 5>());
    case 6: return f(std::integral_constant<int, 6>());
    case 7: return f(std::integral_constant<int, 7>());
    case 8: return f(std::integral_constant<int, 8>());
    default: return PF_ERR_UNSUPPORTED;
  }
}

}

extern "C" {

int pf_fetch_forward_f32(const float* maps, const float* pts, const float* K, const float* E, float* out,
                         int64_t B, int64_t V, int64_t C, int64_t H, int64_t W, int64_t N, void* stream) {
  PF_REQUIRE(B >= 0 && V >= 0 && C >= 0 && H >= 1 && W >= 1 && N >= 0);
  PF_REQUIRE(B <= 65535 && V <= 65535 && H * W <= INT32_MAX && C <= INT32_MAX);
  if (B == 0 || V == 0 || C == 0 || N == 0) return PF_OK;
  PF_REQUIRE(maps && pts && K && out);
  dim3 grid((unsigned)pf_cdiv(N, 256), (unsigned)V, (unsigned)B);
  hipLaunchKernelGGL(fetch_fwd_kernel, grid, dim3(256), 0, (hipStream_t)stream, maps, pts, K, E, out, (int)V,
                     (int)C, (int)H, (int)W, N);
  return pf_launch_status();
}

int pf_fetch_backward_f32(const float* grad_out, const float* pts, const float* K, const float* E,
                          float* grad_maps, int64_t B, int64_t V, int64_t C, int64_t H, int64_t W, int64_t N,
                          void* stream) {
  PF_REQUIRE(B >= 0 && V >= 0 && C >= 0 && H >= 1 && W >= 1 && N >= 0);
  PF_REQUIRE(B <= 65535 && V <= 65535 && H * W <= INT32_MAX && C <= INT32_MAX);
  if (B == 0 || V == 0 || C == 0) return PF_OK;
  PF_REQUIRE(grad_maps != nullptr);
  {
    const int zrc = pf_zero_async(grad_maps, sizeof(float) * (size_t)(B * V * C * H * W), (hipStream_t)stream);
    if (zrc != PF_OK) return zrc;
  }
  if (N == 0) return PF_OK;
  PF_REQUIRE(grad_out && pts && K);
  dim3 grid((unsigned)pf_cdiv(N, 256), (unsigned)V, (unsigned)B);
  hipLaunchKernelGGL(fetch_bwd_kernel, grid, dim3(256), 0, (hipStream_t)stream, grad_out, pts, K, E, grad_maps,
                     (int)V, (int)C, (int)H, (int)W, N);
  return pf_launch_status();
}

int pf_fetch_variance_f32(const float* maps, const float* pts, const float* K, const float* E, float* out,
                          int64_t B, int64_t V, int64_t C, int64_t H, int64_t W, int64_t N, int ref_override,
                          void* stream) {
  PF_REQUIRE(B >= 0 && V >= 1 && C >= 0 && H >= 1 && W >= 1 && N >= 0);
  PF_REQUIRE(B <= 65535 && H * W <= INT32_MAX && C <= INT32_MAX);
  if (V > PF_MAX_VIEWS) return PF_ERR_UNSUPPORTED;
  if (B == 0 || C == 0 || N == 0) return PF_OK;
  PF_REQUIRE(maps && pts && K && out);
  dim3 grid((unsigned)pf_cdiv(N, 256), (unsigned)B);
  return dispatch_views((int)V, [&](auto vtag) {
    constexpr int VV = decltype(vtag)::value;
    hipLaunchKernelGGL((fetch_variance_kernel<VV, false>), grid, dim3(256), 0, (hipStream_t)stream, maps, pts,
                       Frustum{}, K, E, out, (int)C, (int)H, (int)W, N, ref_override);
    return pf_launch_status();
  });
}

int pf_frustum_variance_f32(const float* maps, const float* kinv, const float* rinv, const float* t,
                            const float* depths, const float* K, const float* E, float* out, float* world,
                            int64_t B, int64_t V, int64_t C, int64_t H, int64_t W, int64_t D, void* stream) {
  PF_REQUIRE(B >= 0 && V >= 1 && C >= 0 && H >= 1 && W >= 1 && D >= 0);
  PF_REQUIRE(B <= 65535 && H * W <= INT32_MAX && C <= INT32_MAX && D <= INT32_MAX);
  if (V > PF_MAX_VIEWS) return PF_ERR_UNSUPPORTED;
  const int64_t N = D * H * W;
  if (B == 0 || N == 0) return PF_OK;
  PF_REQUIRE(maps && kinv && rinv && t && depths && K && out);
  Frustum fr;
  fr.kinv = kinv;
  fr.rinv = rinv;
  fr.t = t;
  fr.depths = depths;
  fr.world = world;
  fr.D = (int)D;
  dim3 grid((unsigned)pf_cdiv(N, 256), (unsigned)B);
  return dispatch_views((int)V, [&](auto vtag) {
    constexpr int VV = decltype(vtag)::value;
    hipLaunchKernelGGL((fetch_variance_kernel<VV, true>), grid, dim3(256), 0, (hipStream_t)stream, maps, nullptr, fr,
                       K, E, out, (int)C, (int)H, (int)W, N, 1);
    return pf_launch_status();
  });
}

int pf_nchw_to_nhwc_f32(const float* in, float* out, int64_t P, int64_t C, int64_t S, void* stream) {
  PF_REQUIRE(P >= 0 && C >= 1 && S >= 1 && P <= 65535 && C <= INT32_MAX && pf_cdiv(C, 64) <= 65535);
  if (P == 0) return PF_OK;
  PF_REQUIRE(in && out);
  dim3 grid((unsigned)pf_cdiv(S, 64), (unsigned)pf_cdiv(C, 64), (unsigned)P);
  hipLaunchKernelGGL(nchw_to_nhwc_kernel, grid, dim3(256), 0, (hipStream_t)stream, in, out, (int)C, S);
  return pf_launch_status();
}

int pf_frustum_variance_cl_f32(const float* maps_cl, const float* kinv, const float* rinv, const float* t,
                               const float* depths, const float* K, const float* E, float* out, float* world,
                               int64_t B, int64_t V, int64_t C, int64_t H, int64_t W, int64_t D, void* stream) {
  PF_REQUIRE(B >= 0 && V >= 1 && C >= 0 && H >= 1 && W >= 1 && D >= 0);
  PF_REQUIRE(B <= 65535 && H * W <= INT32_MAX && C <= INT32_MAX && D <= INT32_MAX);
  if (V > PF_MAX_VIEWS || (C % 4) != 0) return PF_ERR_UNSUPPORTED;
  const int64_t N = D * H * W;
  if (B == 0 || N == 0 || C == 0) return PF_OK;
  PF_REQUIRE(maps_cl && kinv && rinv && t && depths && K && out);
  PF_REQUIRE(H * W * C <= (int64_t)INT32_MAX * 4);
  Frustum fr;
  fr.kinv = kinv;
  fr.rinv = rinv;
  fr.t = t;
  fr.depths = depths;
  fr.world = world;
  fr.D = (int)D;
  dim3 grid((unsigned)pf_cdiv(N, 64), (unsigned)B);
  return dispatch_views((int)V, [&](auto vtag) {
    constexpr int VV = decltype(vtag)::value;
    hipLaunchKernelGGL((frustum_variance_cl_kernel<VV>), grid, dim3(256), 0, (hipStream_t)stream, maps_cl, fr, K, E,
                       out, (int)C, (int)H, (int)W, N);
    return pf_launch_status();
  });
}

int pf_resize_bilinear_f32(const float* in, float* out, int64_t P, int64_t IH, int64_t IW, int64_t OH,
                           int64_t OW, void* stream) {
  PF_REQUIRE(P >= 0 && IH >= 1 && IW >= 1 && OH >= 1 && OW >= 1);
  PF_REQUIRE(P <= 65535 && IH * IW <= INT32_MAX && OH * OW <= INT32_MAX);
  if (P == 0) return PF_OK;
  PF_REQUIRE(in && out);
  dim3 grid((unsigned)pf_cdiv(OH * OW, 256), (unsigned)P);
  const float sy = (float)IH / (float)OH, sx = (float)IW / (float)OW;
  hipLaunchKernelGGL(resize_bilinear_kernel, grid, dim3(256), 0, (hipStream_t)stream, in, out, (int)IH, (int)IW,
                     (int)OH, (int)OW, sy, sx);
  return pf_launch_status();
}

int pf_flow_pyramid_f32(const float* in1, int c1, int h1, int w1, const float* in2, int c2, int h2, int w2,
                        const float* in3, int c3, int h3, int w3, int V, int h, int w, float* out1, float* out2,
                        float* out3, const float* const* in_scale, const float* const* in_shift, void* stream) {
  PF_REQUIRE(V >= 1 && h >= 1 && w >= 1 && c1 >= 0 && c2 >= 0 && c3 >= 0);
  PF_REQUIRE((in_scale == nullptr) == (in_shift == nullptr));
  const float* sc[3] = {nullptr, nullptr, nullptr};
  const float* sh[3] = {nullptr, nullptr, nullptr};
  for (int l = 0; in_scale != nullptr && l < 3; ++l) {
    PF_REQUIRE((in_scale[l] == nullptr) == (in_shift[l] == nullptr));
    sc[l] = in_scale[l];
    sh[l] = in_shift[l];
  }
  PF_REQUIRE(h1 >= 1 && w1 >= 1 && h2 >= 1 && w2 >= 1 && h3 >= 1 && w3 >= 1);
  if ((c1 % 4) != 0 || (c2 % 4) != 0 || (c3 % 4) != 0) return PF_ERR_UNSUPPORTED;
  PF_REQUIRE((int64_t)h * w <= INT32_MAX && (int64_t)h1 * w1 <= INT32_MAX && (int64_t)h2 * w2 <= INT32_MAX &&
             (int64_t)h3 * w3 <= INT32_MAX);
  int cmax = c1 > c2 ? c1 : c2;
  cmax = cmax > c3 ? cmax : c3;
  if (cmax == 0) return PF_OK;
  PF_REQUIRE((c1 == 0 || (in1 && out1)) && (c2 == 0 || (in2 && out2)) && (c3 == 0 || (in3 && out3)));
  PF_REQUIRE((int64_t)V * (cmax / 4) <= 65535);
  Pyramid py;
  py.l[0] = PyramidLevel{in1, out1, sc[0], sh[0], c1, h1, w1};
  py.l[1] = PyramidLevel{in2, out2, sc[1], sh[1], c2, h2, w2};
  py.l[2] = PyramidLevel{in3, out3, sc[2], sh[2], c3, h3, w3};
  dim3 grid((unsigned)pf_cdiv((int64_t)h * w, 256), (unsigned)(V * (cmax / 4)), 3);
  hipLaunchKernelGGL(pyramid_resize_kernel, grid, dim3(256), 0, (hipStream_t)stream, py, V, h, w, cmax / 4);
  return pf_launch_status();
}

int pf_flow_features_f32(const float* maps1, const float* maps2, const float* maps3, int c1, int c2, int c3,
                         int V, int h, int w, const float* depth_in, int dh, int dw, const float* interval,
                         const float* cam, int ratio, float* feature, float* xyz, void* stream) {
  PF_REQUIRE(c1 >= 0 && c2 >= 0 && c3 >= 0 && V >= 1 && h >= 1 && w >= 1 && dh >= 1 && dw >= 1 && ratio >= 1);
  if ((c1 % 4) != 0 || (c2 % 4) != 0 || (c3 % 4) != 0) return PF_ERR_UNSUPPORTED;
  PF_REQUIRE(h % ratio == 0 && w % ratio == 0);
  PF_REQUIRE(ratio * ratio <= 65535);
  if (V > PF_MAX_VIEWS) return PF_ERR_UNSUPPORTED;
  PF_REQUIRE(maps1 && maps2 && maps3 && depth_in && interval && cam && feature && xyz);
  const int64_t Ng = (int64_t)5 * (h / ratio) * (w / ratio);
  (void)Ng;
  PF_REQUIRE(pf_cdiv(h, kFeatPY) * pf_cdiv(w, kFeatPX) * 5 <= INT32_MAX);
  dim3 gridh((unsigned)(pf_cdiv(h, kFeatPY) * pf_cdiv(w, kFeatPX)));
  return dispatch_views(V, [&](auto vtag) {
    constexpr int VV = decltype(vtag)::value;
    hipLaunchKernelGGL((flow_features_hyp_kernel<VV, false>), gridh, dim3(256), 0, (hipStream_t)stream, maps1, maps2,
                       maps3, c1, c2, c3, h, w, depth_in, dh, dw, interval, cam, ratio, feature, xyz);
    return pf_launch_status();
  });
}

int pf_softargmin_prob_f32(const float* cost, const float* params, float* depth, float* prob, int64_t B,
                           int64_t D, int64_t HW, void* stream) {
  PF_REQUIRE(B >= 0 && D >= 1 && HW >= 0 && B <= 65535 && D <= INT32_MAX);
  if (B == 0 || HW == 0) return PF_OK;
  PF_REQUIRE(cost && params && depth && prob);
  dim3 grid((unsigned)pf_cdiv(HW, 64), (unsigned)B);
  hipLaunchKernelGGL(softargmin_prob_kernel, grid, dim3(256), 0, (hipStream_t)stream, cost, params, depth, prob,
                     (int)D, HW);
  return pf_launch_status();
}

}
```

pointmvsnet_amd/csrc/pf_bn_resolve.h:

```cpp
#pragma once

#include "pf_common.h"

#ifndef PF_RESOLVE_BATCH
#define PF_RESOLVE_BATCH 5
#endif
constexpr int kResolveBatch = PF_RESOLVE_BATCH;
constexpr int kResolveMaxRows = 4096;
static inline int pf_bn_in_check(const pf_bn_job* j, int C, int stat_groups) {
  PF_REQUIRE(j != nullptr && j->partials != nullptr && j->gamma != nullptr && j->beta != nullptr);
  PF_REQUIRE(j->T >= 1 && j->pcols >= 1 && j->col0 >= 0 && j->C == C && C >= 1 && C <= 256 && j->col0 + C <= j->pcols);
  PF_REQUIRE(j->count > 0.0 && j->G >= 1 && j->groups_per_stat >= 1 && (j->G % j->groups_per_stat) == 0);
  PF_REQUIRE(j->G / j->groups_per_stat == stat_groups);
  if ((int64_t)j->groups_per_stat * j->T > kResolveMaxRows) return PF_ERR_UNSUPPORTED;
  return PF_OK;
}

#if defined(__HIPCC__)
template <int THREADS>
__device__ __forceinline__ void pf_bn_resolve(const pf_bn_job& J, int s, float* sm_scale, float* sm_shift,
                                              double* red) {
  const int tid = threadIdx.x;
  const int C = J.C;
  const int per_stat = J.groups_per_stat * J.T;
  int slices = THREADS / C;
  if (slices > per_stat) slices = per_stat;
  const int per = (per_stat + slices - 1) / slices;
  const int c = tid % C, sl = tid / C;
  double a = 0.0, b = 0.0;
  if (sl < slices) {
    const double2* base = reinterpret_cast<const double2*>(J.partials) + (int64_t)s * per_stat * J.pcols + J.col0 + c;
    const int r0 = sl * per, r1 = min(per_stat, r0 + per);
    for (int r = r0; r < r1; r += kResolveBatch) {
      double2 v[kResolveBatch];
#pragma unroll
      for (int u = 0; u < kResolveBatch; ++u) v[u] = base[(int64_t)min(r + u, r1 - 1) * J.pcols];
#pragma unroll
      for (int u = 0; u < kResolveBatch; ++u) {
        a += (r + u < r1) ? v[u].x : 0.0;
        b += (r + u < r1) ? v[u].y : 0.0;
      }
    }
  }
  red[2 * tid + 0] = a;
  red[2 * tid + 1] = b;
  __syncthreads();
  if (tid < C) {
    double sum = 0.0, sq = 0.0;
    for (int i = 0; i < slices; ++i) {
      sum += red[2 * (i * C + tid) + 0];
      sq += red[2 * (i * C + tid) + 1];
    }
    const double mean = sum / J.count;
    double var = sq / J.count - mean * mean;
    var = var < 0.0 ? 0.0 : var;
    const float invstd = (float)(1.0 / sqrt(var + (double)J.eps));
    const float a_ = invstd * J.gamma[tid];
    sm_scale[tid] = a_;
    sm_shift[tid] = J.beta[tid] - (float)mean * a_;
  }
  __syncthreads();
}
#endif
```

pointmvsnet_amd/model.py:

```python
import collections
import os

import torch
import torch.nn as nn
import torch.nn.functional as F

from . import networks as _networks
from . import pointflow
from . import train_ops
from .functions.functions import get_pixel_grids, get_propability_map
from .networks import (EdgeConv, EdgeConvNoC, ImageConv, VolumeConv, MAELoss, Valid_MAELoss, tower_pair_supported,
                       tower_pair_views)
from .nn.mlp import SharedMLP
from .utils.feature_fetcher import ChannelLast, FeatureFetcher, frustum_variance
from .utils.torch_utils import get_knn_3d

_HYPOTHESES = (-2, -1, 0, 1, 2)

FUSED_TRAIN = 1

TRAIN_FORK = int(os.environ.get("PF_TRAIN_FORK", "2"))
_FORK_STREAMS = {}


# ... 183 lines not shown
        entries = [("K_coarse", (B, V, 3, 3)), ("ext", (B, V, 3, 4)), ("Kinv0", (B, 1, 3, 3)), ("Rinv0", (B, 1, 3, 3)),
                   ("t0", (B, 1, 3, 1)), ("depths", (B, self.D)), ("d_start", (B,)), ("d_int", (B,)),
                   ("mean", (B, 3, 1)), ("std", (B, 3, 1)), ("sa_params", (B, 3))]
        for i in range(len(self.img_scales)):
            entries += [("interval%d" % i, (B,)), ("K_flow%d" % i, (B, V, 3, 3)), ("Kinv_flow%d" % i, (B, 1, 3, 3)),
                        ("pack%d" % i, (B, 27 + 21 * V + 1))]
        self._layout, off = {}, 0
        for name, shape in entries:
            n = 1
            for d in shape:
                n *= d
            self._layout[name] = (off, n, shape)
            off += (n + 3) // 4 * 4
        self.host = torch.zeros(off, dtype=torch.float32)
        if torch.cuda.is_available():
            self.host = self.host.pin_memory()
        self.dev = torch.zeros(off, dtype=torch.float32, device=device)
        self._copied = None

    def _h(self, name):
        off, n, shape = self._layout[name]
        return self.host[off:off + n].view(shape)

    def d(self, name):
        off, n, shape = self._layout[name]
        return self.dev[off:off + n].view(shape)

    def matches(self, device, B, V, num_depth, img_scales, inter_scales, is_test):
        return (self.device == device and (self.B, self.V, self.D) == (B, V, int(num_depth))
                and self.img_scales == tuple(img_scales) and self.inter_scales == tuple(inter_scales)
                and self.is_test == bool(is_test))

    def fill_host_(self, data_batch):
        cam = _Cameras(_host_cams(data_batch), self.is_test)
        if cam.num_depth != self.D:
            raise RuntimeError("TrainPlan: num_depth changed (%d -> %d); build a new plan" % (self.D, cam.num_depth))
        mean_h = data_batch["mean_host"] if "mean_host" in data_batch else data_batch["mean"].detach().cpu()
        std_h = data_batch["std_host"] if "std_host" in data_batch else data_batch["std"].detach().cpu()
        if self._copied is not None:
            self._copied.synchronize()
        self._h("K_coarse").copy_(cam.K_coarse)
        self._h("ext").copy_(cam.ext)
        self._h("Kinv0").copy_(torch.inverse(cam.K_coarse[:, 0]).unsqueeze(1))
        self._h("Rinv0").copy_(cam.R_inv[:, 0:1])
        self._h("t0").copy_(cam.t[:, 0:1])
        for b in range(self.B):
            self._h("depths")[b].copy_(torch.linspace(float(cam.depth_start[b]), float(cam.depth_end[b]), self.D))
        self._h("d_start").copy_(cam.depth_start)
        self._h("d_int").copy_(cam.depth_interval)
        self._h("sa_params").copy_(torch.stack([cam.depth_start, cam.depth_end, cam.depth_interval], dim=1))
        self._h("mean").copy_(mean_h.float().reshape(self.B, 3, 1))
        self._h("std").copy_(std_h.float().reshape(self.B, 3, 1))
        for i, (s, inter) in enumerate(zip(self.img_scales, self.inter_scales)):
            K_flow = cam.flow_intrinsics(s)
            self._h("interval%d" % i).copy_(inter * cam.depth_interval)
            self._h("K_flow%d" % i).copy_(K_flow)
            self._h("Kinv_flow%d" % i).copy_(torch.inverse(K_flow[:, 0]).unsqueeze(1))
            self._h("pack%d" % i).copy_(cam.packed(K_flow, mean_h.float().reshape(self.B, 3),
                                                   std_h.float().reshape(self.B, 3), inter * cam.depth_interval))
        return self

    def upload_(self):
        self.dev.copy_(self.host, non_blocking=True)
        if self.dev.is_cuda:
            self._copied = torch.cuda.Event()
            self._copied.record()
        return self

    def update_(self, data_batch):
        return self.fill_host_(data_batch).upload_()


class PointMVSNet(nn.Module):
    def __init__(self, img_base_channels=8, vol_base_channels=8, flow_channels=(64, 64, 16, 1), k=16):
        super(PointMVSNet, self).__init__()
        self.k = k
        self.feature_fetcher = FeatureFetcher()
        self.coarse_img_conv = ImageConv(img_base_channels)
        self.coarse_vol_conv = VolumeConv(self.coarse_img_conv.out_channels, vol_base_channels)
        self.flow_img_conv = ImageConv(img_base_channels)
        self.flow_edge_conv = nn.ModuleList([EdgeConvNoC(136, 32), EdgeConv(32, 32), EdgeConv(64, 64)])
        self.flow_mlp = nn.Sequential(
            SharedMLP(32 + 32 * 2 + 64 * 2, flow_channels[:-1]),
            nn.Conv1d(flow_channels[-2], flow_channels[-1], 1, bias=False),
        )
        self._grid_cache = {}
        self._plan = None
        self._tplan = None

    def _pixel_grid(self, h, w, device):
        key = (h, w, str(device))
        if key not in self._grid_cache:
            self._grid_cache[key] = get_pixel_grids(h, w).to(device)
        return self._grid_cache[key]

    def _hypotheses(self, device):
        key = ("hyp", str(device))
        if key not in self._grid_cache:
            self._grid_cache[key] = torch.tensor(_HYPOTHESES, dtype=torch.float32, device=device)
        return self._grid_cache[key]

    def _needs_graph(self):
        return torch.is_grad_enabled() and any(p.requires_grad for p in self.parameters())

    def make_plan(self, data_batch, img_scales, inter_scales, isTest):
        img_list = data_batch["img_list"]
        B, V, _, H, W = img_list.shape
        D = int(_host_cams(data_batch)[0, 0, 1, 3, 2].long())
        plan = ScenePlan(img_list.device, B, V, H, W, img_scales, inter_scales, isTest, D)
        return plan.update_(data_batch)

    def forward(self, data_batch, img_scales, inter_scales, isFlow, isTest=False):
        img_list = data_batch["img_list"]
        if not img_list.is_cuda:
            raise RuntimeError("pointmvsnet_amd.PointMVSNet runs on a GPU (HIP) device only; the CPU "
                               "restatement lives in oracle/ and is test infrastructure")
        B, V, _, H, W = img_list.shape
        if self._needs_graph() or B > 1:
            return self._forward_autograd(data_batch, img_scales, inter_scales, isFlow, isTest)
        D = int(_host_cams(data_batch)[0, 0, 1, 3, 2].long())
        plan = self._plan
        if plan is None or not plan.matches(img_list.device, B, V, H, W, img_scales, inter_scales, isTest, D):
            plan = self._plan = ScenePlan(img_list.device, B, V, H, W, img_scales, inter_scales, isTest, D)
        plan.update_(data_batch)
        return self.run(plan, img_list, isFlow)

    def run(self, plan, img_list, isFlow=True):
        dev = img_list.device
        main = torch.cuda.current_stream()
        pointflow.stamp("start")
        if isFlow and pointflow.CONCURRENCY < 1 and tower_pair_supported(self.coarse_img_conv, self.flow_img_conv,
                                                                         img_list):
            coarse_cl, pyramids = tower_pair_views(self.coarse_img_conv, self.flow_img_conv, img_list)
            pointflow.stamp("coarse_tower_end")
            preds = self.run_coarse_stage(plan, ChannelLast(coarse_cl))
            return self.run_flows(plan, pyramids, preds)
        feature_list = self.run_coarse_tower(img_list)
        pointflow.stamp("coarse_tower_end")
        if not isFlow:
            preds = self.run_coarse_stage(plan, feature_list)
            pointflow.flush_counters()
            return preds
        if pointflow.CONCURRENCY < 1:
            pyramids = self.run_flow_tower(img_list, raw=True)
            preds = self.run_coarse_stage(plan, feature_list)
            return self.run_flows(plan, pyramids, preds)
        side = pointflow.side_stream(dev, 0)
        side.wait_stream(main)
        with torch.cuda.stream(side):
            pyramids = self.run_flow_tower(img_list, raw=True)
            pointflow.stamp("flow_tower_end")
            for p in pyramids.values():
                if isinstance(p, pointflow.RawLevel):
                    for t in (p.raw,) + (tuple(pointflow.affine_rows(p.affine)) if p.affine is not None else ()):
                        t.record_stream(main)
                else:
                    p.record_stream(main)
        preds = self.run_coarse_stage(plan, feature_list)
        main.wait_stream(side)
        return self.run_flows(plan, pyramids, preds)

    def run_coarse_tower(self, img_list):
        out = self.coarse_img_conv.forward_views(img_list, need=("conv3",), channel_last=("conv3",))
        if "conv3_cl" in out:
            return ChannelLast(out["conv3_cl"].contiguous())
        return out["conv3"].contiguous()

    def run_flow_tower(self, img_list, raw=False):
        if raw and img_list.shape[0] == 1:
            out = self.flow_img_conv.forward_views(img_list, raw=("conv1", "conv2", "conv3"))
            return {n: out[n + "_raw"] if n + "_raw" in out else out[n] for n in ("conv1", "conv2", "conv3")}
        return self.flow_img_conv.forward_views(img_list)

    def run_coarse_stage(self, plan, feature_list):
        B, D = plan.B, plan.D
        preds = collections.OrderedDict()
        if isinstance(feature_list, ChannelLast):
            FH, FW, C = feature_list.maps.shape[2:]
        else:
            C, FH, FW = feature_list.shape[2:]
        cost, world_points = frustum_variance(feature_list, plan.d("Kinv0"), plan.d("Rinv0"), plan.d("t0"),
                                              plan.d("depths"), plan.d("K_coarse"), plan.d("ext"))
        pointflow.stamp("warp_end")
        preds["world_points"] = world_points
        filtered = self.coarse_vol_conv.forward_fused(cost.view(B, C, D, FH, FW)).squeeze(1)
        pred_depth, prob_map = pointflow.soft_argmin_params(filtered, plan.d("sa_params"))
        pointflow.stamp("coarse_stage_end")
        preds["coarse_depth_map"] = pred_depth
        preds["coarse_prob_map"] = prob_map
        return preds

    def run_flows(self, plan, pyramids, preds):
        B, H, W = plan.B, plan.H, plan.W
        pred_depth = preds["coarse_depth_map"]
        names = ("conv1", "conv2", "conv3")
        for it, img_scale in enumerate(plan.img_scales):
            h, w = int(H * img_scale), int(W * img_scale)
            ratio = int(img_scale * 8) if (plan.is_test and img_scale != 0.125) else 1
            packed = plan.d("pack%d" % it)
            outs, probs = [], []
            for b in range(B):
                pyr_b = [pyramids[n] if isinstance(pyramids[n], pointflow.RawLevel) else pyramids[n][b].contiguous()
                         for n in names]
                d_b, p_b = pointflow.flow_iteration(pyr_b, pred_depth[b, 0], packed[b, -1:], packed[b], h, w, ratio,
                                                    self.flow_edge_conv, self.flow_mlp, k=self.k)
                outs.append(d_b)
                probs.append(p_b)
            pred_depth = torch.stack(outs, dim=0).unsqueeze(1) if B > 1 else outs[0].view(1, 1, h, w)
            flow_prob = torch.stack(probs, dim=0) if B > 1 else probs[0].unsqueeze(0)
            preds["flow{}_prob".format(it + 1)] = flow_prob
            preds["flow{}".format(it + 1)] = pred_depth
            pointflow.stamp("flow%d_end" % (it + 1))
        pointflow.flush_counters()
        return preds

    def make_train_plan(self, data_batch, img_scales, inter_scales, isTest=False):
        img_list = data_batch["img_list"]
        B, V = img_list.shape[:2]
        D = int(_host_cams(data_batch)[0, 0, 1, 3, 2].long())
        return TrainPlan(img_list.device, B, V, D, img_scales, inter_scales, isTest).update_(data_batch)

    def _forward_autograd(self, data_batch, img_scales, inter_scales, isFlow, isTest, tplan=None):
        img_list = data_batch["img_list"]
        dev = img_list.device
        B, V, _, H, W = img_list.shape
        if tplan is None:
            D = int(_host_cams(data_batch)[0, 0, 1, 3, 2].long())
            tplan = self._tplan
            if tplan is None or not tplan.matches(dev, B, V, D, img_scales, inter_scales, isTest):
                tplan = self._tplan = TrainPlan(dev, B, V, D, img_scales, inter_scales, isTest)
            tplan.update_(data_batch)
        return self.run_autograd(tplan, img_list, isFlow)

    def _coarse_cost_autograd(self, feature_list, world_points, K_coarse, ext, D):
        B, V, C = feature_list.shape[:3]
        point_features = self.feature_fetcher(feature_list, world_points, K_coarse, ext)
        ref = feature_list[:, 0].unsqueeze(2).expand(-1, -1, D, -1, -1).contiguous().view(B, C, -1)
        point_features = torch.cat([ref.unsqueeze(1), point_features[:, 1:]], dim=1)
        avg = point_features.mean(dim=1)
        return (point_features ** 2).mean(dim=1) - avg ** 2

    def _fused_train(self, img_list):
        return bool(FUSED_TRAIN and _networks.FUSED_TRAIN and img_list.shape[0] == 1 and self.training
                    and torch.is_grad_enabled()
                    and train_ops.tower_supported(self.coarse_img_conv, img_list[0])
                    and train_ops.tower_supported(self.flow_img_conv, img_list[0]))

    def run_autograd(self, tplan, img_list, isFlow=True):
        if not self._fused_train(img_list):
            return self._run_autograd(tplan, img_list, isFlow, False)
        from .train_packs import TrainPacks
        packs = getattr(self, "_train_packs", None)
        if packs is None or packs.stale():
            packs = TrainPacks(self)
            object.__setattr__(self, "_train_packs", packs)
        with torch.cuda.device(img_list.device):
            packs.run()
        side = self._fork_stream(img_list.device) if (TRAIN_FORK and isFlow and img_list.is_cuda) else None
        with train_ops.use_packs(packs), pointflow.deferred_counters(), train_ops.side_stream(side, TRAIN_FORK):
            return self._run_autograd(tplan, img_list, isFlow, True)

    def _fork_stream(self, dev):
        streams = _FORK_STREAMS
        key = (dev.type, dev.index if dev.index is not None else torch.cuda.current_device())
        if key not in streams:
            streams[key] = torch.cuda.Stream(device=dev)
            quiet = getattr(torch.autograd.graph, "set_warn_on_accumulate_grad_stream_mismatch", None)
            if quiet is not None:
                quiet(False)
        return streams[key]

    def _run_autograd(self, tplan, img_list, isFlow, fused):
        dev = img_list.device
        B, V, _, H, W = img_list.shape
        isTest, img_scales = tplan.is_test, tplan.img_scales
        preds = collections.OrderedDict()
        K_coarse = tplan.d("K_coarse")
        ext = tplan.d("ext")

        names = ("conv1", "conv2", "conv3")
        levels = side = None
        if fused and isFlow and TRAIN_FORK and img_list.is_cuda:
            main = torch.cuda.current_stream(dev)
            side = self._fork_stream(dev)
            side.wait_stream(main)
            with torch.cuda.stream(side):
                levels = train_ops.tower_train(self.flow_img_conv, img_list[0], names)
        if fused:
            maps3 = train_ops.tower_train(self.coarse_img_conv, img_list[0], ("conv3",))["conv3"]
            feature_list = maps3.unsqueeze(0)
        else:
            coarse_maps = [self.coarse_img_conv(img_list[:, v])["conv3"] for v in range(V)]
            feature_list = torch.stack(coarse_maps, dim=1)
        C, FH, FW = feature_list.shape[2:]
        D = tplan.D
        depths = tplan.d("depths")
        R_inv0 = tplan.d("Rinv0")
        t0 = tplan.d("t0")
        if not (fused and C % 4 == 0 and V <= 8):
            grid = self._pixel_grid(FH, FW, dev).view(1, 1, 3, -1).expand(B, 1, 3, -1)
            uv = torch.matmul(tplan.d("Kinv0"), grid)
            cam_points = (uv.unsqueeze(3) * depths.view(B, 1, 1, D, 1)).view(B, 1, 3, -1)
            world_points = torch.matmul(R_inv0, cam_points - t0).transpose(1, 2).contiguous().view(B, 3, -1)
            preds["world_points"] = world_points

        if fused and C % 4 == 0 and V <= 8:
            cost, world_points = train_ops.coarse_volume_train(maps3, tplan.d("Kinv0"), R_inv0, t0, depths,
# ... 218 lines not shown
```

pointmvsnet_amd/networks.py:

```python
import torch
import torch.nn as nn
import torch.nn.functional as F

from . import _lib
from . import pointflow
from .functions.gather_knn import gather_knn
from .nn.conv import *
from .nn.conv import Conv2d, Conv3d, Deconv3d


class _EdgeConvTrain(torch.autograd.Function):

    @staticmethod
    def forward(ctx, feature, knn_inds, w1, w2, gamma, beta, bn, concat):
        B, cin, N = feature.shape
        C = w1.shape[0]
        k = knn_inds.shape[2]
        width = (2 if concat else 1) * C
        x = feature.detach().float().contiguous()
        idx = knn_inds.contiguous()
        out = torch.empty((B * N, width), dtype=torch.float32, device=x.device)
        keep = {}
        with _lib.on_device(x.device):
            pointflow.edge_conv_fused(x, False, 0, cin, B, N, idx, w1, w2, bn, concat, out, width,
# ... 36 lines not shown
        if not torch.is_grad_enabled():
            return False
        return feature.requires_grad or any(p.requires_grad for p in self.parameters())

    def _forward_autograd(self, feature, knn_inds):
        k = knn_inds.shape[2]
        local_feature = self.conv1(feature)
        edge_feature = self.conv2(feature)
        neighbour = gather_knn(edge_feature, knn_inds)
        central = local_feature.unsqueeze(-1).expand(-1, -1, -1, k)
        diff = neighbour - central
        edge = torch.cat([central, diff], dim=1) if self.concat else diff
        edge = F.relu(self.bn(edge), inplace=True)
        return torch.mean(edge, dim=3)

    def _forward_fused(self, feature, knn_inds):
        B, cin, N = feature.shape
        cout = self.conv1.weight.shape[0]
        width = (2 if self.concat else 1) * cout
        x = feature.detach().float().contiguous()
        idx = knn_inds.contiguous()
        out = torch.empty((B * N, width), dtype=torch.float32, device=x.device)
        with _lib.on_device(x.device):
            pointflow.edge_conv_fused(x, False, 0, cin, B, N, idx, self.conv1.weight, self.conv2.weight,
                                      self.bn, self.concat, out, width, groups_per_stat=B)
            pointflow.flush_counters()
        return out.view(B, N, width).transpose(1, 2).contiguous()

    def forward(self, feature, knn_inds):
        _lib.require_gpu(feature, knn_inds)
        if feature.dim() != 3 or knn_inds.dim() != 3 or knn_inds.dtype != torch.int64:
            raise RuntimeError("EdgeConv: expected feature (B,C,N) and int64 knn_inds (B,N,k)")
        if self._needs_graph(feature):
            if (FUSED_TRAIN and self.bn.training and self.bn.momentum is not None and self.bn.affine
                    and self.conv1.weight.shape[0] in (32, 64) and knn_inds.shape[2] >= 1):
                return _EdgeConvTrain.apply(feature, knn_inds, self.conv1.weight, self.conv2.weight,
                                            self.bn.weight, self.bn.bias, self.bn, self.concat)
            return self._forward_autograd(feature, knn_inds)
        if self.conv1.weight.shape[0] not in (32, 64) or knn_inds.shape[2] < 1:
            with torch.no_grad():
                return self._forward_autograd(feature, knn_inds)
        if feature.dtype == torch.float32:
            from . import graph
            return graph.module_forward(self, self._forward_fused, feature, knn_inds)
        return self._forward_fused(feature, knn_inds)


class EdgeConv(_EdgeConvBase):
    concat = True


class EdgeConvNoC(_EdgeConvBase):
    concat = False


def _deconv_block_ok(block):
    conv = getattr(block, "conv", None)
    return (type(conv) is nn.ConvTranspose3d and conv.kernel_size == (3, 3, 3) and conv.stride == (2, 2, 2)
            and conv.padding == (1, 1, 1) and conv.output_padding == (1, 1, 1) and conv.dilation == (1, 1, 1)
            and conv.groups == 1 and conv.bias is None)


def _deconv_fusable(block, x):
    return _deconv_block_ok(block) and x[0, 0].numel() >= 2048


def _conv3d_fusable(conv, x):
    return (type(conv) is nn.Conv3d and conv.kernel_size == (3, 3, 3) and conv.padding == (1, 1, 1)
            and conv.stride in ((1, 1, 1), (2, 2, 2)) and conv.dilation == (1, 1, 1) and conv.groups == 1
            and conv.bias is None and conv.in_channels % 4 == 0 and conv.out_channels <= 32
            and x[0, 0].numel() // (conv.stride[0] ** 3) >= 2048)


def _block_fused(block, x, samples_per_stat):
    skip = None
    if isinstance(x, tuple):
        x, skip = x
    if (skip is not None or hasattr(block, "bn")) and _deconv_fusable(block, x):
        training_bn = block.bn is not None and (block.bn.training or not block.bn.track_running_stats)
        y, partials = pointflow.deconv3d_k3s2(x.contiguous(), None if skip is None else skip.contiguous(),
                                              block.conv.weight, training_bn)
        if block.bn is not None:
            return pointflow.batch_norm_act_(y, block.bn, block.relu, samples_per_stat, partials=partials)
        return F.relu(y, inplace=True) if block.relu else y
    if not hasattr(block, "bn"):
        if (type(block) is nn.Conv3d and block.kernel_size == (3, 3, 3) and block.padding == (1, 1, 1)
                and block.stride == (1, 1, 1) and block.dilation == (1, 1, 1) and block.groups == 1
                and block.bias is None and block.out_channels <= 4 and block.in_channels * block.out_channels <= 256):
            return pointflow.conv3d_k3_few((x if skip is None else x + skip).contiguous(), block.weight)
        return block(x if skip is None else x + skip)
    if skip is not None:
        x = x + skip
    conv = block.conv
    training_bn = block.bn is not None and (block.bn.training or not block.bn.track_running_stats)
    if _conv3d_fusable(conv, x):
        y, partials = pointflow.conv3d_k3(x.contiguous(), conv.weight, conv.stride[0], training_bn)
        if block.bn is not None:
            return pointflow.batch_norm_act_(y, block.bn, block.relu, samples_per_stat, partials=partials)
        return F.relu(y, inplace=True) if block.relu else y
    pointflow.warn_library_fallback("VolumeConv layer", conv)
    y = block._crop(conv(x), x)
    if block.bn is not None:
        return pointflow.batch_norm_act_(y.contiguous(), block.bn, block.relu, samples_per_stat)
    return F.relu(y, inplace=True) if block.relu else y


class ImageConv(nn.Module):

    def __init__(self, base_channels):
        super(ImageConv, self).__init__()
        b = base_channels
        self.base_channels = b
        self.out_channels = 8 * b

        def stage(cin, cout, last_plain=False):
            tail = nn.Conv2d(cout, cout, 3, padding=1, bias=False) if last_plain \
                else Conv2d(cout, cout, 3, 1, padding=1)
            return nn.Sequential(Conv2d(cin, cout, 5, stride=2, padding=2),
                                 Conv2d(cout, cout, 3, 1, padding=1), tail)

        self.conv0 = nn.Sequential(Conv2d(3, b, 3, 1, padding=1), Conv2d(b, b, 3, 1, padding=1))
        self.conv1 = stage(b, 2 * b)
        self.conv2 = stage(2 * b, 4 * b)
        self.conv3 = stage(4 * b, 8 * b, last_plain=True)

    def forward(self, imgs):
        if pointflow.hip_inference(imgs, self):
            def run(x):
                out = self.forward_views(x.unsqueeze(1), need=("conv0", "conv1", "conv2", "conv3"))
                pointflow.flush_counters()
                return {k: v[:, 0] for k, v in out.items()}
            from . import graph
            return graph.module_forward(self, run, imgs)
        out = {}
        x = imgs
        for name in ("conv0", "conv1", "conv2", "conv3"):
            x = getattr(self, name)(x)
            out[name] = x
        return out

    def forward_views(self, img_list, need=("conv1", "conv2", "conv3"), channel_last=(), raw=()):
        B, V = img_list.shape[:2]
        x = img_list.transpose(0, 1).reshape(V * B, *img_list.shape[2:]).float().contiguous()
        pending = None
        blocks = [(name, blk) for name in ("conv0", "conv1", "conv2", "conv3") for blk in getattr(self, name)]
        out = {}
        for i, (name, block) in enumerate(blocks):
            stage_end = i + 1 == len(blocks) or blocks[i + 1][0] != name
            nxt = blocks[i + 1][1] if i + 1 < len(blocks) else None
            nconv = None if nxt is None else (nxt.conv if hasattr(nxt, "bn") else nxt)
            wanted = stage_end and name in need
            as_raw = wanted and name in raw and B == 1 and (nconv is None or pointflow.conv2d_wide_preferred(nconv))
            defer = (as_raw or not wanted) and nconv is not None and pointflow.conv2d_wide_preferred(nconv)
            lazy = bool(defer) and not as_raw
            conv = block.conv if hasattr(block, "bn") else block
            cl = (wanted and name in channel_last and not hasattr(block, "bn") and conv.out_channels >= 32
                  and pointflow.conv2d_wide_preferred(conv))
            x, pending = _conv2d_block_fused(block, x, pending, B, defer, lazy, channel_last_out=cl)
            if as_raw:
                out[name + "_raw"] = pointflow.RawLevel(x, pending)
            elif wanted:
                out[name + "_cl" if cl else name] = x.view(V, B, *x.shape[1:]).transpose(0, 1)
        return out


def tower_pair_supported(coarse, flow, img_list):
    if img_list.shape[0] != 1 or coarse.base_channels != flow.base_channels or coarse.out_channels < 32:
        return False
    if not pointflow.conv2d_wide_stacked_supported([coarse.conv0[0].conv, flow.conv0[0].conv]):
        return False
    for tower in (coarse, flow):
        for name in ("conv0", "conv1", "conv2", "conv3"):
            for blk in getattr(tower, name):
                conv, bn = (blk.conv, blk.bn) if hasattr(blk, "bn") else (blk, None)
                if not pointflow.conv2d_wide_preferred(conv):
                    return False
                if bn is not None and not (blk.relu and (bn.training or not bn.track_running_stats)):
                    return False
    return True


def tower_pair_views(coarse, flow, img_list):
    V = img_list.shape[1]
    x = img_list[0].float().contiguous()
    blocks = [(name, cb, fb) for name in ("conv0", "conv1", "conv2", "conv3")
              for cb, fb in zip(getattr(coarse, name), getattr(flow, name))]
    pending = None
    levels = {}
    for i, (name, cb, fb) in enumerate(blocks):
        last = i + 1 == len(blocks)
        stage_end = last or blocks[i + 1][0] != name
        has_bn = hasattr(cb, "bn")
        convs = [cb.conv, fb.conv] if has_bn else [cb, fb]
        if i == 0:
            y, partials = pointflow.conv2d_wide_stacked(x, convs, has_bn)
        else:
            y, partials = pointflow.conv2d_wide_sets(x, convs, pending, 1, has_bn, interleaved=(i == 1),
                                                     channel_last_sets=(0,) if last else ())
        raw_level = stage_end and name != "conv0"
        pending = pointflow.bn_affine_rows_sets(y, [cb.bn, fb.bn], 1, partials, lazy=not raw_level,
                                                interleaved=(i == 0)) if has_bn else None
        if raw_level:
            levels[name] = pointflow.RawLevel(y[V:], None if pending is None else pending.rows_of(1))
        x = y
    C = x.shape[1]
    return x[:V].view(1, V, x.shape[2], x.shape[3], C), levels


def _conv2d_block_fused(block, x, pending, samples_per_stat, defer, lazy=False, channel_last_out=False):
    conv, bn, relu = (block.conv, block.bn, block.relu) if hasattr(block, "bn") else (block, None, False)
    training_bn = bn is not None and (bn.training or not bn.track_running_stats)
    if pointflow.conv2d_wide_preferred(conv):
        y, partials = pointflow.conv2d_wide(x, conv, pending, samples_per_stat, training_bn,
                                            channel_last_out=channel_last_out)
    else:
        pointflow.warn_library_fallback("ImageConv layer", conv)
        if pending is not None:
            x = pointflow.channel_affine_(x, pending, True, samples_per_stat)
        y = block._crop(conv(x), x).contiguous() if hasattr(block, "_crop") else conv(x).contiguous()
        partials = None
    if bn is None:
        return (F.relu(y, inplace=True) if relu else y), None
    if defer and relu:
        return y, pointflow.bn_affine_rows(y, bn, samples_per_stat, partials, lazy=lazy)
    return pointflow.batch_norm_act_(y, bn, relu, samples_per_stat, partials=partials), None


class VolumeConv(nn.Module):

    def __init__(self, in_channels, base_channels):
        super(VolumeConv, self).__init__()
        b = base_channels
        self.in_channels = in_channels
        self.out_channels = 8 * b
        self.base_channels = b
        self.conv1_0 = Conv3d(in_channels, 2 * b, 3, stride=2, padding=1)
        self.conv2_0 = Conv3d(2 * b, 4 * b, 3, stride=2, padding=1)
        self.conv3_0 = Conv3d(4 * b, 8 * b, 3, stride=2, padding=1)
        self.conv0_1 = Conv3d(in_channels, b, 3, 1, padding=1)
        self.conv1_1 = Conv3d(2 * b, 2 * b, 3, 1, padding=1)
        self.conv2_1 = Conv3d(4 * b, 4 * b, 3, 1, padding=1)
        self.conv3_1 = Conv3d(8 * b, 8 * b, 3, 1, padding=1)
        self.conv4_0 = Deconv3d(8 * b, 4 * b, 3, 2, padding=1, output_padding=1)
        self.conv5_0 = Deconv3d(4 * b, 2 * b, 3, 2, padding=1, output_padding=1)
        self.conv6_0 = Deconv3d(2 * b, b, 3, 2, padding=1, output_padding=1)
        self.conv6_2 = nn.Conv3d(b, 1, 3, padding=1, bias=False)

    def _bottom_fusable(self):
        blocks = (self.conv3_0, self.conv3_1, self.conv4_0)
        return (all(b.bn is not None and b.relu for b in blocks)
                and pointflow.conv3d_bottom_supported(self.conv3_0.conv)
                and pointflow.conv3d_bottom_supported(self.conv3_1.conv)
                and pointflow.deconv3d_bottom_supported(self.conv4_0.conv))

    def forward_fused(self, x):
        B = x.shape[0]
        f = lambda blk, t: _block_fused(blk, t, B)
        blk0, blk6 = self.conv0_1, self.conv6_0
        train0 = blk0.bn is not None and blk0.relu and (blk0.bn.training or not blk0.bn.track_running_stats)
        if train0 and _conv3d_fusable(blk0.conv, x):
            full = pointflow.conv3d_k3(x.contiguous(), blk0.conv.weight, 1, True)
        else:
            full = f(blk0, x)
        pointflow.stamp("conv0_1_end")
        half = f(self.conv1_0, x)
        quarter = f(self.conv2_0, half)
        if self._bottom_fusable():
            b0, b1, b2 = self.conv3_0, self.conv3_1, self.conv4_0
            y0, p0 = pointflow.conv3d_bottom(quarter.contiguous(), b0.conv, None, B, True)
            y1, p1 = pointflow.conv3d_bottom(y0, b1.conv, pointflow.bn_affine_rows(y0, b0.bn, B, p0, lazy=True), B, True)
            pointflow.stamp("unet_encoder_end")
            y2, p2 = pointflow.deconv3d_bottom(y1, b2.conv, pointflow.bn_affine_rows(y1, b1.bn, B, p1, lazy=True), B, True)
            up = pointflow.batch_norm_act_(y2, b2.bn, b2.relu, B, partials=p2)
        else:
            eighth = f(self.conv3_1, f(self.conv3_0, quarter))
            pointflow.stamp("unet_encoder_end")
            up = f(self.conv4_0, eighth)
        pointflow.stamp("unet_bottom_end")
        half = f(self.conv1_1, half)
        quarter = f(self.conv2_1, quarter)
        up = f(self.conv5_0, (up, quarter))
        if (isinstance(full, tuple) and _deconv_fusable(blk6, up) and blk6.bn is not None and blk6.relu
                and (blk6.bn.training or not blk6.bn.track_running_stats)):
            y6, p6 = pointflow.deconv3d_k3s2(up.contiguous(), half.contiguous(), blk6.conv.weight, True)
            raw0, p0 = full
            return f(self.conv6_2, pointflow.batch_norm_act2_(raw0, blk0.bn, p0, y6, blk6.bn, p6, B))
        up = f(blk6, (up, half))
        if isinstance(full, tuple):
            raw, partials = full
            summed = pointflow.batch_norm_act_(raw, blk0.bn, blk0.relu, B, partials=partials, addend=up.contiguous())
        else:
            summed = up + full
        return f(self.conv6_2, summed)

    def forward(self, x):
        if pointflow.hip_inference(x, self):
            def run(v):
                y = self.forward_fused(v)
                pointflow.flush_counters()
                return y
            from . import graph
            return graph.module_forward(self, run, x)
        full = self.conv0_1(x)
        half = self.conv1_0(x)
        quarter = self.conv2_0(half)
        eighth = self.conv3_1(self.conv3_0(quarter))
        half = self.conv1_1(half)
        quarter = self.conv2_1(quarter)
        up = self.conv4_0(eighth)
        up = self.conv5_0(up + quarter)
        up = self.conv6_0(up + half)
        return self.conv6_2(up + full)


class MAELoss(nn.Module):

    def forward(self, pred_depth_image, gt_depth_image, depth_interval):
        interval = depth_interval.view(-1)
        valid = (gt_depth_image != 0.0).float()
        count = valid.sum(dim=(1, 2, 3)) + 1e-7
        err = (valid * (pred_depth_image - gt_depth_image).abs()).sum(dim=(1, 2, 3))
        return ((err / interval) / count).sum()


class Valid_MAELoss(nn.Module):

    def __init__(self, valid_threshold=2.0):
        super(Valid_MAELoss, self).__init__()
        self.valid_threshold = valid_threshold

    def forward(self, pred_depth_image, gt_depth_image, depth_interval, before_depth_image):
        interval = depth_interval.view(-1)
        if before_depth_image.size(2) != pred_depth_image.size(2):
            before_depth_image = F.interpolate(before_depth_image, tuple(pred_depth_image.shape[2:]))
        prior_err = (gt_depth_image - before_depth_image).abs() / interval.view(-1, 1, 1, 1)
        valid = (gt_depth_image != 0.0).float() * (prior_err < self.valid_threshold).float()
        count = valid.sum(dim=(1, 2, 3)) + 1e-7
        err = (valid * (pred_depth_image - gt_depth_image).abs()).sum(dim=(1, 2, 3))
        return ((err / interval) / count).sum()
```

pointmvsnet_amd/pointflow.py:

```python
import contextlib
import ctypes

import torch

from . import _lib
from .utils.torch_utils import knn_lattice

_F32 = torch.float32


def hip_inference(x, module):
    if not (torch.is_tensor(x) and x.is_cuda and x.dtype == _F32):
        return False
    if not torch.is_grad_enabled():
        return True
    return not (x.requires_grad or any(p.requires_grad for p in module.parameters()))


_LIBRARY_WARNED = set()


def warn_library_fallback(what, conv):
    key = (what, type(conv).__name__, conv.in_channels, conv.out_channels, tuple(conv.kernel_size), tuple(conv.stride))
    if key in _LIBRARY_WARNED:
# ... 704 lines not shown


def pack_conv3d_bottom_weight(weight):
    def make():
        cout, cin = weight.shape[:2]
        w = weight.detach().to(_F32).permute(2, 3, 4, 1, 0).reshape(3, 3, 3, cin // 16, 4, 4, cout)
        return w.permute(0, 1, 2, 3, 4, 6, 5).contiguous()
    return _cached_pack(("c3b", id(weight)), (weight,), make)


def pack_deconv3d_bottom_weight(weight):
    def make():
        cin, cout = weight.shape[:2]
        w = weight.detach().to(_F32).permute(2, 3, 4, 0, 1).reshape(27, cin // 16, 4, 4, cout)
        return w.permute(0, 1, 2, 4, 3).contiguous()
    return _cached_pack(("d3b", id(weight)), (weight,), make)


def conv3d_bottom(x, conv, in_affine, samples_per_stat, want_stats):
    N, Cin, Di, Hi, Wi = x.shape
    stride = int(conv.stride[0])
    Do, Ho, Wo = (Di - 1) // stride + 1, (Hi - 1) // stride + 1, (Wi - 1) // stride + 1
    wp = pack_conv3d_bottom_weight(conv.weight)
    y = torch.empty((N, 64, Do, Ho, Wo), dtype=_F32, device=x.device)
    partials = None
    if want_stats:
        T = int(_lib.load().pf_conv3d_bottom_blocks(Di, Hi, Wi, stride))
        partials = torch.empty((N, T, 64, 2), dtype=torch.float64, device=x.device)
    sc, sh, in_bn = _split_affine(in_affine)
    _lib.call("pf_conv3d_bottom_f32", _lib.ptr(x), _lib.ptr(wp), _lib.ptr(y), N, Cin, 64, Di, Hi, Wi, stride,
              _lib.ptr(sc), _lib.ptr(sh), in_bn, int(samples_per_stat), _lib.ptr(partials), _lib.stream(),
              algo_bytes=4.0 * N * (Cin * Di * Hi * Wi + 64 * Do * Ho * Wo) + 4.0 * 27 * Cin * 64,
              flops=2.0 * N * Do * Ho * Wo * 27 * Cin * 64)
    return y, partials


def deconv3d_bottom(x, conv, in_affine, samples_per_stat, want_stats):
    N, Cin, Di, Hi, Wi = x.shape
    wp = pack_deconv3d_bottom_weight(conv.weight)
    y = torch.empty((N, 32, 2 * Di, 2 * Hi, 2 * Wi), dtype=_F32, device=x.device)
    partials = None
    if want_stats:
        T = int(_lib.load().pf_deconv3d_bottom_blocks(Di, Hi, Wi))
        partials = torch.empty((N, T, 32, 2), dtype=torch.float64, device=x.device)
    sc, sh, in_bn = _split_affine(in_affine)
    _lib.call("pf_deconv3d_bottom_f32", _lib.ptr(x), _lib.ptr(wp), _lib.ptr(y), N, Cin, 32, Di, Hi, Wi,
              _lib.ptr(sc), _lib.ptr(sh), in_bn, int(samples_per_stat), _lib.ptr(partials), _lib.stream(),
              algo_bytes=4.0 * N * Di * Hi * Wi * (Cin + 8 * 32) + 4.0 * 27 * Cin * 32,
              flops=2.0 * N * Di * Hi * Wi * 27 * Cin * 32)
    return y, partials


def conv3d_k3_few(x, weight):
    N, Cin, D, H, W = x.shape
    Cout = weight.shape[0]
    y = torch.empty((N, Cout, D, H, W), dtype=_F32, device=x.device)
    w = weight.detach().to(_F32).contiguous()
    _lib.call("pf_conv3d_k3_few_f32", _lib.ptr(x), _lib.ptr(w), _lib.ptr(y), N, Cin, Cout, D, H, W, _lib.stream(),
              algo_bytes=4.0 * N * D * H * W * (Cin + Cout))
    return y


def pack_conv3d_weight(weight):
    def make():
        cout, cin = weight.shape[:2]
        ncp = (cout + 15) // 16 * 16
        wp = torch.zeros((cin // 4, 27, 4, ncp), dtype=_F32, device=weight.device)
        wp[..., :cout] = weight.detach().to(_F32).permute(1, 2, 3, 4, 0).reshape(cin // 4, 4, 27, cout).transpose(1, 2)
        return wp
    return _cached_pack(("c3", id(weight)), (weight,), make)


def batch_norm_act_(x, bn, relu, samples_per_stat, partials=None, addend=None):
    N, C = x.shape[:2]
    S = x[0, 0].numel()
    G = N // samples_per_stat
    dev = x.device
    if bn.training or not bn.track_running_stats:
        if bn.momentum is None:
            raise NotImplementedError("cumulative-average BatchNorm momentum is not supported")
        if partials is None and N * S <= FUSED_BN_MAX:
            _bn_fused(x, x, bn, relu, samples_per_stat)
            bump_counter(bn, G)
            return x if addend is None else x.add_(addend)
        if partials is None:
            T = int(_lib.load().pf_norm_blocks(S))
            partials = torch.empty((N, T, C, 2), dtype=torch.float64, device=dev)
            _lib.call("pf_channel_stats_f32", _lib.ptr(x), N, C, S, _lib.ptr(partials), _lib.stream(),
                      algo_bytes=4.0 * N * C * S)
        track = bn.track_running_stats and bn.running_mean is not None
        if addend is not None and (addend.shape != x.shape or not addend.is_contiguous()):
            raise RuntimeError("batch_norm_act_: addend must be contiguous and shaped like x")
        _lib.call("pf_channel_bn_apply_f32", _lib.ptr(x), _lib.ptr(x), _lib.ptr(partials), int(partials.shape[1]),
                  N, C, S, int(samples_per_stat), float(samples_per_stat) * S, _lib.ptr(bn.weight.detach()),
                  _lib.ptr(bn.bias.detach()), _lib.ptr(bn.running_mean if track else None),
                  _lib.ptr(bn.running_var if track else None), float(bn.momentum), float(bn.eps), int(bool(relu)),
                  _lib.ptr(addend), _lib.stream(), algo_bytes=(8.0 if addend is None else 12.0) * N * C * S)
        bump_counter(bn, G)
        return x
    else:
        sc, sh = eval_affine(bn, G, C)
        scale = sc.unsqueeze(0).expand(G, C).contiguous()
        shift = sh.unsqueeze(0).expand(G, C).contiguous()
        _lib.call("pf_channel_affine_f32", _lib.ptr(x), _lib.ptr(x), _lib.ptr(scale), _lib.ptr(shift), N, C, S,
                  int(samples_per_stat), int(bool(relu)), _lib.stream(), algo_bytes=8.0 * N * C * S)
    return x if addend is None else x.add_(addend)


def batch_norm_act2_(x1, bn1, partials1, x2, bn2, partials2, samples_per_stat):
    N, C = x1.shape[:2]
    S = x1[0, 0].numel()
    if x2.shape != x1.shape or not (x1.is_contiguous() and x2.is_contiguous()):
        raise RuntimeError("batch_norm_act2_: the two tensors must be contiguous and of one shape")
    for bn in (bn1, bn2):
        if bn.momentum is None:
            raise NotImplementedError("cumulative-average BatchNorm momentum is not supported")
    def side(bn):
        track = bn.track_running_stats and bn.running_mean is not None
        return (_lib.ptr(bn.weight.detach()), _lib.ptr(bn.bias.detach()), _lib.ptr(bn.running_mean if track else None),
                _lib.ptr(bn.running_var if track else None), float(bn.momentum), float(bn.eps))
    a, b = side(bn1), side(bn2)
    _lib.call("pf_channel_bn_apply2_f32", _lib.ptr(x1), _lib.ptr(partials1), int(partials1.shape[1]), *a,
              _lib.ptr(x2), _lib.ptr(partials2), int(partials2.shape[1]), *b, _lib.ptr(x1), N, C, S,
              int(samples_per_stat), float(samples_per_stat) * S, _lib.stream(), algo_bytes=12.0 * N * C * S)
    G = N // samples_per_stat
    bump_counter(bn1, G)
    bump_counter(bn2, G)
    return x1


def edge_conv_fused(X, point_major, ldx, K, G, Ng, idx, conv1_w, conv2_w, bn, concat, Y, ldy,
                    groups_per_stat=1, join=None, codes=None, lattice=None, keep=None):
    C = conv1_w.shape[0]
    k = idx.shape[-1] if idx is not None else int(codes.shape[-1])
    lat = tuple(int(v) for v in lattice) if lattice is not None else (0, 1, 1)
    if codes is None:
        lat = (0, lat[1], lat[2])
    if keep is not None:
        keep["plane"] = lat[1] * lat[2] if lat[1] * lat[2] > 1 else 0
    dev = Y.device
    S = G // groups_per_stat
    training = bn.training or not bn.track_running_stats
    Wt, _ = pack_weight_t(conv1_w, conv2_w)
    LE = torch.empty((G * Ng, 2 * C), dtype=_F32, device=dev)
    cbn = 2 * C if concat else C
    scale = torch.empty((S, cbn), dtype=_F32, device=dev)
    shift = torch.empty((S, cbn), dtype=_F32, device=dev)
    n_pairs = float(groups_per_stat) * Ng * k
    part_l = pointwise_gemm(X, point_major, ldx, Wt, LE, 2 * C, G, Ng, K, 2 * C, groups_per_stat=groups_per_stat,
                            want_stats=(concat and training))
    if join is not None:
        torch.cuda.current_stream().wait_stream(join)
    rows4 = None
    if training:
        T = stat_blocks(G, Ng)
        part_d = stat_rows(G, T, C, dev)
        _lib.call("pf_edge_stats_f32", _lib.ptr(LE), 2 * C, C, _lib.ptr(idx), k, G, Ng, _lib.ptr(part_d),
                  _lib.ptr(codes), lat[0], lat[1], lat[2], _lib.stream(),
                  algo_bytes=float(G) * Ng * (4.0 * C + (1.0 if codes is not None else 8.0) * k + 4.0 * C * k))
        if keep is not None:
            from . import train_ops
            rows4 = torch.empty((4, S, cbn), dtype=_F32, device=dev)

            def job4(partials, count, unbias_n, col, ch0):
                j = bn_job(bn, partials, 0, C, count, unbias_n, G, groups_per_stat, rows4[0][:, col:], rows4[1][:, col:],
                           ch0=ch0)
                j.rows4 = 1
                return j

            if not train_ops.TRAIN_LAZY_BN:
                if concat:
                    train_ops.bn_train_rows(bn, part_l, 0, C, float(groups_per_stat) * Ng, G, groups_per_stat,
                                            unbias_n=n_pairs, rows=rows4, col_out=0, ch0=0, bump=False)
                    train_ops.bn_train_rows(bn, part_d, 0, C, n_pairs, G, groups_per_stat, rows=rows4, col_out=C, ch0=C,
                                            bump=False)
                else:
                    train_ops.bn_train_rows(bn, part_d, 0, C, n_pairs, G, groups_per_stat, rows=rows4, bump=False)
            elif concat:
                bn_finalize_jobs([job4(part_l, float(groups_per_stat) * Ng, n_pairs, 0, 0),
                                  job4(part_d, n_pairs, n_pairs, C, C)])
            else:
                bn_finalize_jobs([job4(part_d, n_pairs, n_pairs, 0, 0)])
            scale, shift = rows4[0], rows4[1]
        elif concat:
            bn_finalize_jobs([
                bn_job(bn, part_l, 0, C, float(groups_per_stat) * Ng, n_pairs, G, groups_per_stat, scale, shift),
                bn_job(bn, part_d, 0, C, n_pairs, n_pairs, G, groups_per_stat, scale[:, C:], shift[:, C:], ch0=C)])
        else:
            bn_affine(bn, part_d, 0, C, n_pairs, n_pairs, G, groups_per_stat, scale, shift, ch0=0)
        bump_counter(bn, S)
    else:
        sc, sh = eval_affine(bn, S, cbn)
        scale.copy_(sc.unsqueeze(0).expand(S, cbn))
        shift.copy_(sh.unsqueeze(0).expand(S, cbn))
    if keep is not None:
        if not training:
            raise RuntimeError("edge_conv_fused(keep=...) needs a train-mode BatchNorm")
        keep.update(LE=LE, scale=rows4[0], shift=rows4[1], mean=rows4[2], invstd=rows4[3])
    _lib.call("pf_edge_apply_f32", _lib.ptr(LE), 2 * C, C, _lib.ptr(idx), k, G, Ng, _lib.ptr(scale),
              _lib.ptr(shift), cbn, groups_per_stat, int(bool(concat)), _lib.ptr(Y), int(ldy), _lib.ptr(codes),
              lat[0], lat[1], lat[2], _lib.stream(),
              algo_bytes=float(G) * Ng * (4.0 * C + (1.0 if codes is not None else 8.0) * k + 4.0 * C * k + 4.0 * cbn))
    return Y


_inverse_cache = _collections.OrderedDict()


def knn_inverse(idx, G, Ng, k):
    key = (idx.data_ptr(), idx._version, str(idx.device), G, Ng, k)
    hit = _inverse_cache.get(key)
    if hit is not None and hit[0]() is idx:
        return hit[1], hit[2]
    dev = idx.device
    order = torch.empty((G * Ng * k,), dtype=torch.int32, device=dev)
    start = torch.empty((G * Ng + 1,), dtype=torch.int32, device=dev)
    nbytes = int(_lib.load().pf_knn_inverse_workspace(int(G), int(Ng), int(k)))
    work = torch.empty((max(nbytes, 1),), dtype=torch.uint8, device=dev)
    _lib.call("pf_knn_inverse", _lib.ptr(idx), int(k), int(G), int(Ng), _lib.ptr(order), _lib.ptr(start), _lib.ptr(work),
              nbytes, _lib.stream(), algo_bytes=8.0 * G * Ng * k * 4)
    try:
        _inverse_cache[key] = (_weakref.ref(idx), order, start)
    except TypeError:
        return order, start
    while len(_inverse_cache) > 8:
        _inverse_cache.popitem(last=False)
    return order, start


DETERMINISTIC_BACKWARD = True
EDGE_BWD_SUMS = _os.environ.get("PF_EDGE_BWD_SUMS", "1") != "0"


def edge_conv_backward(keep, idx, grad_y, C, k, G, Ng, groups_per_stat, concat, into=None, grad_acc=None):
    LE, scale, shift, mean, invstd = keep["LE"], keep["scale"], keep["shift"], keep["mean"], keep["invstd"]
    dev = LE.device
    cbn = 2 * C if concat else C
    S = G // groups_per_stat
    T = stat_blocks(G, Ng)
    partials = torch.empty((G, T, cbn, 2), dtype=torch.float64, device=dev)
    grad_le = torch.empty((G * Ng, 2 * C), dtype=_F32, device=dev)
    two_walks = DETERMINISTIC_BACKWARD and EDGE_BWD_SUMS
    if grad_acc is not None and not two_walks:
        grad_y, grad_acc = grad_y + grad_acc, None
    if two_walks:
        _lib.call("pf_edge_backward_sums_f32", _lib.ptr(LE), 2 * C, C, _lib.ptr(idx), k, G, Ng, _lib.ptr(grad_y),
                  int(grad_y.stride(0)), _lib.ptr(scale), _lib.ptr(shift), _lib.ptr(mean), _lib.ptr(invstd), cbn,
                  groups_per_stat, int(bool(concat)), _lib.ptr(partials), _lib.ptr(grad_le), _lib.ptr(grad_acc),
                  0 if grad_acc is None else int(grad_acc.stride(0)), int(keep.get("plane", 0)), _lib.stream(),
                  algo_bytes=float(G) * Ng * (12.0 * C + 8.0 * k + 4.0 * C * k + 4.0 * cbn))
        if grad_acc is not None:
            grad_y = grad_acc
    else:
        _lib.call("pf_edge_backward_reduce_f32", _lib.ptr(LE), 2 * C, C, _lib.ptr(idx), k, G, Ng, _lib.ptr(grad_y),
                  int(grad_y.stride(0)), _lib.ptr(scale), _lib.ptr(shift), _lib.ptr(mean), _lib.ptr(invstd), cbn,
                  groups_per_stat, int(bool(concat)), _lib.ptr(partials), _lib.stream(),
                  algo_bytes=float(G) * Ng * (4.0 * C + 8.0 * k + 4.0 * C * k + 4.0 * cbn))
    c1 = torch.empty((S, cbn), dtype=_F32, device=dev)
    c2 = torch.empty((S, cbn), dtype=_F32, device=dev)
    if into is None:
        dgamma = torch.empty((cbn,), dtype=_F32, device=dev)
        dbeta = torch.empty((cbn,), dtype=_F32, device=dev)
    else:
        dgamma, dbeta = into
    _lib.call("pf_edge_backward_coeffs_f32", _lib.ptr(partials), G, T, cbn, C, int(bool(concat)), groups_per_stat, Ng, k,
              _lib.ptr(c1), _lib.ptr(c2), _lib.ptr(dgamma), _lib.ptr(dbeta), 0 if into is None else 1, _lib.stream(),
              algo_bytes=16.0 * G * T * cbn)
    order, start = knn_inverse(idx, G, Ng, k) if DETERMINISTIC_BACKWARD else (None, None)
    if two_walks:
        _lib.call("pf_edge_backward_finish_f32", _lib.ptr(LE), 2 * C, C, k, G, Ng, _lib.ptr(grad_y),
                  int(grad_y.stride(0)), _lib.ptr(scale), _lib.ptr(shift), _lib.ptr(mean), _lib.ptr(invstd), _lib.ptr(c1),
                  _lib.ptr(c2), cbn, groups_per_stat, int(bool(concat)), _lib.ptr(grad_le), _lib.ptr(order),
                  _lib.ptr(start), int(keep.get("plane", 0)), _lib.stream(),
                  algo_bytes=float(G) * Ng * (16.0 * C + 4.0 * k + 8.0 * C * k + 4.0 * cbn))
    else:
        _lib.call("pf_edge_backward_apply_f32", _lib.ptr(LE), 2 * C, C, _lib.ptr(idx), k, G, Ng, _lib.ptr(grad_y),
                  int(grad_y.stride(0)), _lib.ptr(scale), _lib.ptr(shift), _lib.ptr(mean), _lib.ptr(invstd), _lib.ptr(c1),
                  _lib.ptr(c2), cbn, groups_per_stat, int(bool(concat)), _lib.ptr(grad_le), _lib.ptr(order), _lib.ptr(start),
                  _lib.stream(), algo_bytes=float(G) * Ng * (8.0 * C + 8.0 * k + 8.0 * C * k + 4.0 * cbn))
    return (grad_le, dgamma, dbeta) if into is None else (grad_le, None, None)


def _bn_affine_from_gemm(bn, partials, C, G, Ng, groups_per_stat, dev, lazy=False):
    S = G // groups_per_stat
    scale = torch.empty((S, C), dtype=_F32, device=dev)
    shift = torch.empty((S, C), dtype=_F32, device=dev)
    if bn.training or not bn.track_running_stats:
        n = float(groups_per_stat) * Ng
        bump_counter(bn, S)
        if lazy and LAZY_BN and groups_per_stat * partials.shape[1] * C <= LAZY_MAX_ELEMS:
            job = bn_job(bn, partials, 0, C, n, n, G, groups_per_stat, scale, shift)
            return LazyAffine(job, (partials, scale, shift) + _bn_tensors(bn), scale, shift)
        bn_affine(bn, partials, 0, C, n, n, G, groups_per_stat, scale, shift)
    else:
        sc, sh = eval_affine(bn, S, C)
        scale.copy_(sc.unsqueeze(0).expand(S, C))
        shift.copy_(sh.unsqueeze(0).expand(S, C))
    return scale, shift


def resize_maps(maps, h, w):
    V, C, IH, IW = maps.shape
    if IH == h and IW == w:
        return maps
    out = torch.empty((V, C, h, w), dtype=_F32, device=maps.device)
    _lib.call("pf_resize_bilinear_f32", _lib.ptr(maps), _lib.ptr(out), V * C, IH, IW, h, w, _lib.stream(),
              algo_bytes=4.0 * V * C * (IH * IW + h * w))
    return out


class RawLevel(object):

    def __init__(self, raw, affine):
        self.raw, self.affine = raw, affine


def flow_pyramid(pyramid, h, w):
    maps = [(m.raw if isinstance(m, RawLevel) else m) for m in pyramid]
    rows = [(affine_rows(m.affine) if isinstance(m, RawLevel) else None) for m in pyramid]
    V = maps[0].shape[0]
    outs = [torch.empty((V, h, w, int(m.shape[1])), dtype=_F32, device=m.device) for m in maps]
    args = []
    for m in maps:
        args += [_lib.ptr(m), int(m.shape[1]), int(m.shape[2]), int(m.shape[3])]
    sc = sh = None
    if any(r is not None for r in rows):
        sc = (ctypes.c_void_p * 3)(*[None if r is None else r[0].data_ptr() for r in rows])
        sh = (ctypes.c_void_p * 3)(*[None if r is None else r[1].data_ptr() for r in rows])
    _lib.call("pf_flow_pyramid_f32", *args, V, h, w, _lib.ptr(outs[0]), _lib.ptr(outs[1]), _lib.ptr(outs[2]), sc, sh,
              _lib.stream(), algo_bytes=sum(4.0 * m.numel() + 4.0 * o.numel() for m, o in zip(maps, outs)))
    return outs


def flow_features(levels, depth, interval, cam, h, w, ratio):
    V = levels[0].shape[0]
    c1, c2, c3 = (int(l.shape[3]) for l in levels)
    G = ratio * ratio
    Ng = 5 * (h // ratio) * (w // ratio)
    dev = depth.device
    feature = torch.empty((G, Ng, c1 + c2 + c3 + 24), dtype=_F32, device=dev)
    xyz = torch.empty((G, 3, Ng), dtype=_F32, device=dev)
    _lib.call("pf_flow_features_f32",
              _lib.ptr(levels[0]), _lib.ptr(levels[1]), _lib.ptr(levels[2]), c1, c2, c3, V, h, w, _lib.ptr(depth),
              int(depth.shape[-2]), int(depth.shape[-1]), _lib.ptr(interval), _lib.ptr(cam), int(ratio),
              _lib.ptr(feature), _lib.ptr(xyz), _lib.stream(),
              algo_bytes=4.0 * V * (c1 + c2 + c3) * h * w + 4.0 * G * Ng * (c1 + c2 + c3 + 24 + 3) + 4.0 * h * w)
    return feature, xyz


def flow_chain(feature, xyz, depth, interval, h, w, ratio, edge_convs, flow_mlp, k=16, point_major=True, idx=None):
    dev = depth.device
    if point_major:
        G, Ng, Cin = feature.shape
    else:
        G, Cin, Ng = feature.shape
    hs, ws = h // ratio, w // ratio
    aux, codes, lattice = None, None, None
    if idx is not None:
        if tuple(idx.shape) != (G, Ng, k) or idx.dtype != torch.int64:
            raise RuntimeError("flow_chain: idx must be int64 (G, Ng, k)")
        idx = idx.contiguous()
    else:
        use_codes = k == 16
        lattice = (5, hs, ws) if use_codes else None

        def _knn():
            out = knn_lattice(xyz.view(G, 3, 5, hs, ws), 5, k, with_codes=use_codes, with_idx=not use_codes)
            return out if use_codes else (out, None)

        if CONCURRENCY >= 2:
            main = torch.cuda.current_stream()
            aux = side_stream(dev, 1)
            aux.wait_stream(main)
            with torch.cuda.stream(aux):
                idx, codes = _knn()
                (codes if use_codes else idx).record_stream(main)
        else:
            idx, codes = _knn()

    widths = []
    for m in edge_convs:
        c = m.conv1.weight.shape[0]
        widths.append(2 * c if m.concat else c)
    ctot = sum(widths)
    edges = torch.empty((G * Ng, ctot), dtype=_F32, device=dev)
    col = 0
    X, pm, ldx, K = feature, bool(point_major), (Cin if point_major else 0), Cin
    for li, (m, wdt) in enumerate(zip(edge_convs, widths)):
        Y = edges[:, col:]
        edge_conv_fused(X, pm, ldx, K, G, Ng, idx, m.conv1.weight, m.conv2.weight, m.bn, m.concat, Y, ctot,
                        join=(aux if li == 0 else None), codes=codes, lattice=lattice)
        X, pm, ldx, K = Y, True, ctot, wdt
        col += wdt

    shared, last = flow_mlp[0], flow_mlp[1]
    X, ldx, K = edges, ctot, ctot
    affine = None
    for layer in shared:
        Wt, cout = pack_weight_t(layer.conv.weight)
        Z = torch.empty((G * Ng, cout), dtype=_F32, device=dev)
        bn = layer.bn
        part = pointwise_gemm(X, True, ldx, Wt, Z, cout, G, Ng, K, cout, in_affine=affine, want_stats=True)
        affine = _bn_affine_from_gemm(bn, part, cout, G, Ng, 1, dev, lazy=True)
        X, ldx, K = Z, cout, cout
    if K != 16 or last.weight.shape[0] != 1:
        raise NotImplementedError("flow head kernel is built for the reference widths (..., 16, 1)")
    depth_out = torch.empty((h, w), dtype=_F32, device=dev)
    flow_prob = torch.empty((5, h, w), dtype=_F32, device=dev)
    w_out = last.weight.detach().reshape(-1).to(_F32).contiguous()
    sc, sh, in_bn = _split_affine(affine)
    _lib.call("pf_flow_head_f32", _lib.ptr(X), ldx, _lib.ptr(sc), _lib.ptr(sh), 16, in_bn,
              _lib.ptr(w_out), _lib.ptr(depth), int(depth.shape[-2]), int(depth.shape[-1]), _lib.ptr(interval), h, w,
              ratio, _lib.ptr(flow_prob), _lib.ptr(depth_out), _lib.stream(),
              algo_bytes=4.0 * G * Ng * 16 + 4.0 * h * w * 7)
    return depth_out, flow_prob


def flow_iteration(pyramid, depth, interval, cam, h, w, ratio, edge_convs, flow_mlp, k=16):
    levels = flow_pyramid(pyramid, h, w)
    feature, xyz = flow_features(levels, depth, interval, cam, h, w, ratio)
    return flow_chain(feature, xyz, depth, interval, h, w, ratio, edge_convs, flow_mlp, k=k)


def soft_argmin_prob(cost, depth_start, depth_end, depth_interval):
    return soft_argmin_params(cost, torch.stack([depth_start, depth_end, depth_interval], dim=1).to(_F32))


def soft_argmin_params(cost, params):
    B, D, H, W = cost.shape
    cost = cost.contiguous()
    params = params.contiguous()
    depth = torch.empty((B, 1, H, W), dtype=_F32, device=cost.device)
    prob = torch.empty((B, 1, H, W), dtype=_F32, device=cost.device)
    _lib.call("pf_softargmin_prob_f32", _lib.ptr(cost), _lib.ptr(params), _lib.ptr(depth), _lib.ptr(prob),
              B, D, H * W, _lib.stream(), algo_bytes=4.0 * B * H * W * (D + 2))
    return depth, prob
```

Before: 1094.

## Fold lazy BN finalize into edge apply and flow pyramid kernels; widen edge tiles

Edge-conv training now uses wide (512-thread, double-tile) stats and apply kernels. The apply kernel resolves the batch-norm scale and shift itself from the partial sums instead of relying on a separate finalize launch. Feature-tower raw levels also keep their BN lazy, so the flow pyramid resize resolves the affine in-kernel. This removes finalize kernel launches and the global round trips for scale and shift. In exchange, every block redundantly reduces the partials, and the wide blocks halve the block count.

```diff
diff --git a/include/pointflow_hip.h b/include/pointflow_hip.h
--- a/include/pointflow_hip.h
+++ b/include/pointflow_hip.h
@@ -70,6 +70,11 @@
 int pf_flow_pyramid_f32(const float* in1, int c1, int h1, int w1, const float* in2, int c2, int h2, int w2,
                         const float* in3, int c3, int h3, int w3, int V, int h, int w, float* out1, float* out2,
                         float* out3, const float* const* in_scale, const float* const* in_shift, void* stream);
+struct pf_bn_job;
+int pf_flow_pyramid_bn_f32(const float* in1, int c1, int h1, int w1, const float* in2, int c2, int h2, int w2,
+                           const float* in3, int c3, int h3, int w3, int V, int h, int w, float* out1, float* out2,
+                           float* out3, const float* const* in_scale, const float* const* in_shift,
+                           const struct pf_bn_job* const* in_bn, void* stream);
 
 int pf_flow_features_f32(const float* maps1, const float* maps2, const float* maps3, int c1, int c2, int c3,
                          int V, int h, int w, const float* depth_in, int dh, int dw, const float* interval,
@@ -108,12 +113,17 @@
 
 int pf_edge_stats_f32(const float* LE, int64_t ldle, int C, const int64_t* idx, int k, int G, int Ng,
                       double* partials, const uint8_t* codes, int lat_ks, int lat_h, int lat_w, void* stream);
-
+int pf_edge_wide_blocks(int G, int Ng);
+int pf_edge_stats_wide_f32(const float* LE, int64_t ldle, int C, const int64_t* idx, int k, int G, int Ng,
+                           double* partials, const uint8_t* codes, int lat_ks, int lat_h, int lat_w, void* stream);
 
 int pf_edge_apply_f32(const float* LE, int64_t ldle, int C, const int64_t* idx, int k, int G, int Ng,
                       const float* scale, const float* shift, int ld_affine, int groups_per_stat,
                       int concat, float* Y, int64_t ldy, const uint8_t* codes, int lat_ks, int lat_h, int lat_w,
                       void* stream);
+int pf_edge_apply_bn_f32(const float* LE, int64_t ldle, int C, const int64_t* idx, int k, int G, int Ng,
+                         const pf_bn_job* bn_central, const pf_bn_job* bn_diff, int groups_per_stat, float* Y,
+                         int64_t ldy, const uint8_t* codes, int lat_ks, int lat_h, int lat_w, void* stream);
 
 int pf_edge_backward_reduce_f32(const float* LE, int64_t ldle, int C, const int64_t* idx, int k, int G, int Ng,
                                 const float* grad_y, int64_t ldg, const float* scale, const float* shift,
diff --git a/pointmvsnet_amd/_lib.py b/pointmvsnet_amd/_lib.py
--- a/pointmvsnet_amd/_lib.py
+++ b/pointmvsnet_amd/_lib.py
@@ -45,6 +45,8 @@
     "pf_resize_bilinear_f32": ([_vp, _vp, _i64, _i64, _i64, _i64, _i64, _vp], _i),
     "pf_flow_pyramid_f32": ([_vp, _i, _i, _i, _vp, _i, _i, _i, _vp, _i, _i, _i, _i, _i, _i, _vp, _vp, _vp,
                              ctypes.POINTER(_vp), ctypes.POINTER(_vp), _vp], _i),
+    "pf_flow_pyramid_bn_f32": ([_vp, _i, _i, _i, _vp, _i, _i, _i, _vp, _i, _i, _i, _i, _i, _i, _vp, _vp, _vp,
+                                ctypes.POINTER(_vp), ctypes.POINTER(_vp), ctypes.POINTER(ctypes.POINTER(BnJob)), _vp], _i),
     "pf_flow_features_f32": ([_vp, _vp, _vp, _i, _i, _i, _i, _i, _i, _vp, _i, _i, _vp, _vp, _i, _vp, _vp, _vp], _i),
     "pf_stat_blocks": ([_i, _i], _i),
     "pf_gemm_blocks": ([_i, _i], _i),
@@ -81,6 +83,10 @@
                                   _i64, _i64, _i64, _i, _d, _vp], _i),
     "pf_channel_bn_fused_f32": ([_vp, _vp, _i64, _i64, _i64, _i, _vp, _vp, _vp, _vp, _f, _f, _i, _vp, _vp, _i, _vp], _i),
     "pf_edge_stats_f32": ([_vp, _i64, _i, _vp, _i, _i, _i, _vp, _vp, _i, _i, _i, _vp], _i),
+    "pf_edge_wide_blocks": ([_i, _i], _i),
+    "pf_edge_stats_wide_f32": ([_vp, _i64, _i, _vp, _i, _i, _i, _vp, _vp, _i, _i, _i, _vp], _i),
+    "pf_edge_apply_bn_f32": ([_vp, _i64, _i, _vp, _i, _i, _i, ctypes.POINTER(BnJob), ctypes.POINTER(BnJob), _i, _vp, _i64,
+                              _vp, _i, _i, _i, _vp], _i),
     "pf_edge_backward_reduce_f32": ([_vp, _i64, _i, _vp, _i, _i, _i, _vp, _i64, _vp, _vp, _vp, _vp, _i, _i, _i, _vp, _vp], _i),
     "pf_edge_backward_apply_f32": ([_vp, _i64, _i, _vp, _i, _i, _i, _vp, _i64, _vp, _vp, _vp, _vp, _vp, _vp, _i, _i, _i,
                                     _vp, _vp, _vp, _vp], _i),
diff --git a/pointmvsnet_amd/csrc/edgeconv.hip b/pointmvsnet_amd/csrc/edgeconv.hip
--- a/pointmvsnet_amd/csrc/edgeconv.hip
+++ b/pointmvsnet_amd/csrc/edgeconv.hip
@@ -424,28 +424,29 @@
   }
 }
 
-template <int C, int K>
-__global__ __launch_bounds__(256) void edge_stats_kernel(const float* __restrict__ LE, int64_t ldle,
+template <int C, int K, int W = 1>
+__global__ __launch_bounds__(256 * W) void edge_stats_kernel(const float* __restrict__ LE, int64_t ldle,
                                                          const int64_t* __restrict__ idx, int k, int Ng,
                                                          double* __restrict__ partials, int T,
                                                          unsigned* __restrict__ status,
                                                          const uint8_t* __restrict__ codes, Lattice lat) {
   constexpr int Q = C / 4;
-  constexpr int PPB = 256 / Q;
-  __shared__ double red[256 * 8];
+  constexpr int THREADS = 256 * W, UNIT = TILE * W;
+  constexpr int PPB = THREADS / Q;
+  __shared__ double red[THREADS * 8];
   __shared__ int lut[256];
   if (K == 16 && codes != nullptr) build_code_lut(lut, lat);
   const int tid = threadIdx.x;
   const int q = tid % Q, pl = tid / Q;
   const int g = blockIdx.y, tb = blockIdx.x;
-  const int tiles = (Ng + TILE - 1) / TILE;
+  const int tiles = (Ng + UNIT - 1) / UNIT;
   const int64_t gbase = (int64_t)g * Ng;
   double ds[4] = {0, 0, 0, 0}, dq[4] = {0, 0, 0, 0};
   bool bad = false;
   const int tile0 = xcd_tile(tb, lat);
   for (int tile = tile0; tile < tiles; tile += T) {
-    const int n0 = tile * TILE;
-    for (int p = pl; p < TILE; p += PPB) {
+    const int n0 = tile * UNIT;
+    for (int p = pl; p < UNIT; p += PPB) {
       const int n = n0 + p;
       if (n >= Ng) break;
       const int64_t row = gbase + n;
@@ -499,36 +500,55 @@
   }
 }
 
-template <int C, int K>
-__global__ __launch_bounds__(256) void edge_apply_kernel(const float* __restrict__ LE, int64_t ldle,
+constexpr int kEdgeResolveBatch = 8;
+template <int C, int K, int W = 1, bool BN = false>
+__global__ __launch_bounds__(256 * W) void edge_apply_kernel(const float* __restrict__ LE, int64_t ldle,
                                                          const int64_t* __restrict__ idx, int k, int Ng,
                                                          const float* __restrict__ scale,
                                                          const float* __restrict__ shift, int ld_affine,
                                                          int groups_per_stat, int concat, float* __restrict__ Y,
                                                          int64_t ldy, int T, const uint8_t* __restrict__ codes,
-                                                         Lattice lat) {
+                                                         Lattice lat, pf_bn_job jc, pf_bn_job jd) {
   constexpr int Q = C / 4;
-  constexpr int PPB = 256 / Q;
+  constexpr int THREADS = 256 * W, UNIT = TILE * W;
+  constexpr int PPB = THREADS / Q;
   __shared__ int lut[256];
+  __shared__ __attribute__((aligned(16))) float sm_aff[BN ? 4 * C : 1];
+  __shared__ double sm_red[BN ? 2 * THREADS : 1];
   if (K == 16 && codes != nullptr) build_code_lut(lut, lat);
+  if constexpr (BN) {
+    const int s = blockIdx.y / groups_per_stat;
+    if (concat) pf_bn_resolve<THREADS, kEdgeResolveBatch>(jc, s, sm_aff, sm_aff + 2 * C, sm_red);
+    pf_bn_resolve<THREADS, kEdgeResolveBatch>(jd, s, sm_aff + C, sm_aff + 3 * C, sm_red);
+  }
   const int tid = threadIdx.x;
   const int q = tid % Q, pl = tid / Q;
   const int g = blockIdx.y, tb = blockIdx.x;
-  const int tiles = (Ng + TILE - 1) / TILE;
+  const int tiles = (Ng + UNIT - 1) / UNIT;
   const int64_t gbase = (int64_t)g * Ng;
-  const int64_t so = (int64_t)(g / groups_per_stat) * ld_affine;
-  const int doff = concat ? C : 0;
-  const float4 dsc = ld4(scale + so + doff + 4 * q), dsh = ld4(shift + so + doff + 4 * q);
-  float4 csc = {0, 0, 0, 0}, csh = {0, 0, 0, 0};
-  if (concat) {
-    csc = ld4(scale + so + 4 * q);
-    csh = ld4(shift + so + 4 * q);
+  float4 dsc, dsh, csc = {0, 0, 0, 0}, csh = {0, 0, 0, 0};
+  if constexpr (BN) {
+    dsc = ld4(sm_aff + C + 4 * q);
+    dsh = ld4(sm_aff + 3 * C + 4 * q);
+    if (concat) {
+      csc = ld4(sm_aff + 4 * q);
+      csh = ld4(sm_aff + 2 * C + 4 * q);
+    }
+  } else {
+    const int64_t so = (int64_t)(g / groups_per_stat) * ld_affine;
+    const int doff = concat ? C : 0;
+    dsc = ld4(scale + so + doff + 4 * q);
+    dsh = ld4(shift + so + doff + 4 * q);
+    if (concat) {
+      csc = ld4(scale + so + 4 * q);
+      csh = ld4(shift + so + 4 * q);
+    }
   }
   const float kf = (float)k;
   bool bad = false;
   for (int tile = xcd_tile(tb, lat); tile < tiles; tile += T) {
-    const int n0 = tile * TILE;
-    for (int p = pl; p < TILE; p += PPB) {
+    const int n0 = tile * UNIT;
+    for (int p = pl; p < UNIT; p += PPB) {
       const int n = n0 + p;
       if (n >= Ng) break;
       const int64_t row = gbase + n;
@@ -1282,10 +1302,24 @@
   if (!on || plane <= 1 || plane % unit != 0 || (plane / unit) % 8 != 0 || Ng % plane != 0 || blocks != Ng / unit) return 0;
   return (int)(plane / unit / 8);
 }
-static void lattice_band(Lattice& lat, int Ng, int T) { lat.band = xcd_band((int64_t)lat.H * lat.W, TILE, Ng, T); }
-
-int pf_edge_stats_f32(const float* LE, int64_t ldle, int C, const int64_t* idx, int k, int G, int Ng,
-                      double* partials, const uint8_t* codes, int lat_ks, int lat_h, int lat_w, void* stream) {
+constexpr int kWide = 2;
+static void lattice_band(Lattice& lat, int Ng, int T, int w = 1) {
+  lat.band = xcd_band((int64_t)lat.H * lat.W, TILE * w, Ng, T);
+}
+
+int pf_edge_wide_blocks(int G, int Ng) {
+  if (G <= 0 || Ng <= 0) return 0;
+  const int tiles = (Ng + kWide * TILE - 1) / (kWide * TILE);
+  int cap = PF_STAT_CAP / kWide / G;
+  cap = cap < 16 ? 16 : cap;
+  if (tiles <= cap) return tiles;
+  const int per = (tiles + cap - 1) / cap;
+  return (tiles + per - 1) / per;
+}
+
+static int edge_stats_launch(const float* LE, int64_t ldle, int C, const int64_t* idx, int k, int G, int Ng,
+                             double* partials, const uint8_t* codes, int lat_ks, int lat_h, int lat_w, void* stream,
+                             bool wide) {
   PF_REQUIRE(G >= 0 && Ng >= 0 && k >= 1 && ldle >= 2 * (int64_t)C && (ldle % 4) == 0 && G <= 65535);
   if (C != 32 && C != 64 && C != 128) return PF_ERR_UNSUPPORTED;
   if (G == 0 || Ng == 0) return PF_OK;
@@ -1297,11 +1331,19 @@
   }
   unsigned* status = pf_status_ptr();
   PF_REQUIRE(status != nullptr);
-  const int T = pf_stat_blocks(G, Ng);
-  lattice_band(lat, Ng, T);
+  const int T = wide ? pf_edge_wide_blocks(G, Ng) : pf_stat_blocks(G, Ng);
+  lattice_band(lat, Ng, T, wide ? kWide : 1);
   dim3 grid((unsigned)T, (unsigned)G);
   hipStream_t s = (hipStream_t)stream;
-#define PF_ES(CV, KV) hipLaunchKernelGGL((edge_stats_kernel<CV, KV>), grid, dim3(256), 0, s, LE, ldle, idx, k, Ng, partials, T, status, codes, lat)
+#define PF_ES(CV, KV)                                                                                                  \
+  do {                                                                                                                 \
+    if (wide)                                                                                                          \
+      hipLaunchKernelGGL((edge_stats_kernel<CV, KV, kWide>), grid, dim3(256 * kWide), 0, s, LE, ldle, idx, k, Ng,      \
+                         partials, T, status, codes, lat);                                                             \
+    else                                                                                                               \
+      hipLaunchKernelGGL((edge_stats_kernel<CV, KV>), grid, dim3(256), 0, s, LE, ldle, idx, k, Ng, partials, T,       \
+                         status, codes, lat);                                                                          \
+  } while (0)
   if (k == 16) {
     if (C == 32) PF_ES(32, 16); else if (C == 64) PF_ES(64, 16); else PF_ES(128, 16);
   } else {
@@ -1309,6 +1351,16 @@
   }
 #undef PF_ES
   return pf_launch_status();
+}
+
+int pf_edge_stats_f32(const float* LE, int64_t ldle, int C, const int64_t* idx, int k, int G, int Ng,
+                      double* partials, const uint8_t* codes, int lat_ks, int lat_h, int lat_w, void* stream) {
+  return edge_stats_launch(LE, ldle, C, idx, k, G, Ng, partials, codes, lat_ks, lat_h, lat_w, stream, false);
+}
+
+int pf_edge_stats_wide_f32(const float* LE, int64_t ldle, int C, const int64_t* idx, int k, int G, int Ng,
+                           double* partials, const uint8_t* codes, int lat_ks, int lat_h, int lat_w, void* stream) {
+  return edge_stats_launch(LE, ldle, C, idx, k, G, Ng, partials, codes, lat_ks, lat_h, lat_w, stream, true);
 }
 
 int pf_bn_finalize_jobs_f32(const pf_bn_job* jobs, int njobs, void* stream) {
@@ -1376,9 +1428,48 @@
   lattice_band(lat, Ng, T);
   dim3 grid((unsigned)T, (unsigned)G);
   hipStream_t s = (hipStream_t)stream;
+  const pf_bn_job no_bn = {};
 #define PF_EA(CV, KV)                                                                                         \
   hipLaunchKernelGGL((edge_apply_kernel<CV, KV>), grid, dim3(256), 0, s, LE, ldle, idx, k, Ng, scale, shift, \
-                     ld_affine, groups_per_stat, concat, Y, ldy, T, codes, lat)
+                     ld_affine, groups_per_stat, concat, Y, ldy, T, codes, lat, no_bn, no_bn)
+  if (k == 16) {
+    if (C == 32) PF_EA(32, 16); else if (C == 64) PF_EA(64, 16); else PF_EA(128, 16);
+  } else {
+    if (C == 32) PF_EA(32, 0); else if (C == 64) PF_EA(64, 0); else PF_EA(128, 0);
+  }
+#undef PF_EA
+  return pf_launch_status();
+}
+
+int pf_edge_apply_bn_f32(const float* LE, int64_t ldle, int C, const int64_t* idx, int k, int G, int Ng,
+                         const pf_bn_job* bn_central, const pf_bn_job* bn_diff, int groups_per_stat, float* Y,
+                         int64_t ldy, const uint8_t* codes, int lat_ks, int lat_h, int lat_w, void* stream) {
+  const int concat = bn_central != nullptr;
+  PF_REQUIRE(G >= 0 && Ng >= 0 && k >= 1 && ldle >= 2 * (int64_t)C && (ldle % 4) == 0 && G <= 65535);
+  PF_REQUIRE(groups_per_stat >= 1 && (ldy % 4) == 0 && ldy >= (concat ? 2 : 1) * (int64_t)C);
+  if (C != 32 && C != 64 && C != 128) return PF_ERR_UNSUPPORTED;
+  if (G == 0 || Ng == 0) return PF_OK;
+  PF_REQUIRE(LE && Y && bn_diff != nullptr && (G % groups_per_stat) == 0);
+  for (const pf_bn_job* j : {bn_central, bn_diff}) {
+    if (j == nullptr) continue;
+    PF_REQUIRE(j->G == G && j->groups_per_stat == groups_per_stat);
+    const int rc = pf_bn_in_check(j, C, G / groups_per_stat);
+    if (rc != PF_OK) return rc;
+  }
+  Lattice lat;
+  {
+    const int rc = check_lattice(idx, codes, k, Ng, lat_ks, lat_h, lat_w, lat);
+    if (rc != PF_OK) return rc;
+  }
+  const int T = pf_edge_wide_blocks(G, Ng);
+  lattice_band(lat, Ng, T, kWide);
+  dim3 grid((unsigned)T, (unsigned)G);
+  hipStream_t s = (hipStream_t)stream;
+  const pf_bn_job jc = concat ? *bn_central : *bn_diff;
+#define PF_EA(CV, KV)                                                                                              \
+  hipLaunchKernelGGL((edge_apply_kernel<CV, KV, kWide, true>), grid, dim3(256 * kWide), 0, s, LE, ldle, idx, k, Ng, \
+                     (const float*)nullptr, (const float*)nullptr, 0, groups_per_stat, concat, Y, ldy, T, codes,   \
+                     lat, jc, *bn_diff)
   if (k == 16) {
     if (C == 32) PF_EA(32, 16); else if (C == 64) PF_EA(64, 16); else PF_EA(128, 16);
   } else {
diff --git a/pointmvsnet_amd/csrc/fetch.hip b/pointmvsnet_amd/csrc/fetch.hip
--- a/pointmvsnet_amd/csrc/fetch.hip
+++ b/pointmvsnet_amd/csrc/fetch.hip
@@ -3,6 +3,7 @@
 #include <stdlib.h>
 
 #include "pf_common.h"
+#include "pf_bn_resolve.h"
 
 namespace {
 
@@ -290,19 +291,45 @@
 struct Pyramid {
   PyramidLevel l[3];
 };
-
-__global__ __launch_bounds__(256) void pyramid_resize_kernel(Pyramid py, int V, int OH, int OW, int cq_max) {
+struct PyramidJobs {
+  pf_bn_job bn[3];
+};
+
+template <bool IN_BN>
+__global__ __launch_bounds__(256) void pyramid_resize_kernel(Pyramid py, int V, int OH, int OW, int cq_max,
+                                                             PyramidJobs jobs) {
   const PyramidLevel L = py.l[blockIdx.z];
   const int v = blockIdx.y / cq_max, cq = blockIdx.y - v * cq_max;
   const int i = blockIdx.x * blockDim.x + threadIdx.x;
-  if (4 * cq >= L.C || i >= OH * OW) return;
+  if (4 * cq >= L.C) return;
+  __shared__ float sm_aff[IN_BN ? 8 : 1];
+  __shared__ double sm_red[IN_BN ? 2 * 256 : 1];
+  bool lazy = false;
+  if constexpr (IN_BN) {
+    lazy = jobs.bn[blockIdx.z].partials != nullptr;
+    if (lazy) {
+      pf_bn_job J = jobs.bn[blockIdx.z];
+      J.col0 += 4 * cq;
+      J.gamma += 4 * cq;
+      J.beta += 4 * cq;
+      J.C = 4;
+      pf_bn_resolve<256>(J, v / J.groups_per_stat, sm_aff, sm_aff + 4, sm_red);
+    }
+  }
+  if (i >= OH * OW) return;
   const int oy = i / OW, ox = i - oy * OW;
   const int plane = L.IH * L.IW;
   const float* src = L.in + ((int64_t)v * L.C + 4 * cq) * plane;
   float r[4];
   float sc[4] = {1.0f, 1.0f, 1.0f, 1.0f}, sh[4] = {0.0f, 0.0f, 0.0f, 0.0f};
-  const bool aff = L.scale != nullptr;
-  if (aff) {
+  const bool aff = lazy || L.scale != nullptr;
+  if (lazy) {
+#pragma unroll
+    for (int c = 0; c < 4; ++c) {
+      sc[c] = sm_aff[c];
+      sh[c] = sm_aff[4 + c];
+    }
+  } else if (aff) {
 #pragma unroll
     for (int c = 0; c < 4; ++c) {
       sc[c] = L.scale[(int64_t)v * L.C + 4 * cq + c];
@@ -665,9 +692,10 @@
   return pf_launch_status();
 }
 
-int pf_flow_pyramid_f32(const float* in1, int c1, int h1, int w1, const float* in2, int c2, int h2, int w2,
-                        const float* in3, int c3, int h3, int w3, int V, int h, int w, float* out1, float* out2,
-                        float* out3, const float* const* in_scale, const float* const* in_shift, void* stream) {
+static int flow_pyramid_launch(const float* in1, int c1, int h1, int w1, const float* in2, int c2, int h2, int w2,
+                               const float* in3, int c3, int h3, int w3, int V, int h, int w, float* out1, float* out2,
+                               float* out3, const float* const* in_scale, const float* const* in_shift,
+                               const pf_bn_job* const* in_bn, void* stream) {
   PF_REQUIRE(V >= 1 && h >= 1 && w >= 1 && c1 >= 0 && c2 >= 0 && c3 >= 0);
   PF_REQUIRE((in_scale == nullptr) == (in_shift == nullptr));
   const float* sc[3] = {nullptr, nullptr, nullptr};
@@ -691,8 +719,38 @@
   py.l[1] = PyramidLevel{in2, out2, sc[1], sh[1], c2, h2, w2};
   py.l[2] = PyramidLevel{in3, out3, sc[2], sh[2], c3, h3, w3};
   dim3 grid((unsigned)pf_cdiv((int64_t)h * w, 256), (unsigned)(V * (cmax / 4)), 3);
-  hipLaunchKernelGGL(pyramid_resize_kernel, grid, dim3(256), 0, (hipStream_t)stream, py, V, h, w, cmax / 4);
+  PyramidJobs jobs = {};
+  bool any = false;
+  const int cl[3] = {c1, c2, c3};
+  for (int l = 0; in_bn != nullptr && l < 3; ++l) {
+    if (in_bn[l] == nullptr || cl[l] == 0) continue;
+    PF_REQUIRE(sc[l] == nullptr);
+    const int rc = pf_bn_in_check(in_bn[l], cl[l], V / in_bn[l]->groups_per_stat);
+    if (rc != PF_OK) return rc;
+    PF_REQUIRE(in_bn[l]->G == V);
+    jobs.bn[l] = *in_bn[l];
+    any = true;
+  }
+  if (any)
+    hipLaunchKernelGGL(pyramid_resize_kernel<true>, grid, dim3(256), 0, (hipStream_t)stream, py, V, h, w, cmax / 4, jobs);
+  else
+    hipLaunchKernelGGL(pyramid_resize_kernel<false>, grid, dim3(256), 0, (hipStream_t)stream, py, V, h, w, cmax / 4, jobs);
   return pf_launch_status();
+}
+
+int pf_flow_pyramid_f32(const float* in1, int c1, int h1, int w1, const float* in2, int c2, int h2, int w2,
+                        const float* in3, int c3, int h3, int w3, int V, int h, int w, float* out1, float* out2,
+                        float* out3, const float* const* in_scale, const float* const* in_shift, void* stream) {
+  return flow_pyramid_launch(in1, c1, h1, w1, in2, c2, h2, w2, in3, c3, h3, w3, V, h, w, out1, out2, out3, in_scale,
+                             in_shift, nullptr, stream);
+}
+
+int pf_flow_pyramid_bn_f32(const float* in1, int c1, int h1, int w1, const float* in2, int c2, int h2, int w2,
+                           const float* in3, int c3, int h3, int w3, int V, int h, int w, float* out1, float* out2,
+                           float* out3, const float* const* in_scale, const float* const* in_shift,
+                           const pf_bn_job* const* in_bn, void* stream) {
+  return flow_pyramid_launch(in1, c1, h1, w1, in2, c2, h2, w2, in3, c3, h3, w3, V, h, w, out1, out2, out3, in_scale,
+                             in_shift, in_bn, stream);
 }
 
 int pf_flow_features_f32(const float* maps1, const float* maps2, const float* maps3, int c1, int c2, int c3,
diff --git a/pointmvsnet_amd/csrc/pf_bn_resolve.h b/pointmvsnet_amd/csrc/pf_bn_resolve.h
--- a/pointmvsnet_amd/csrc/pf_bn_resolve.h
+++ b/pointmvsnet_amd/csrc/pf_bn_resolve.h
@@ -17,7 +17,7 @@
 }
 
 #if defined(__HIPCC__)
-template <int THREADS>
+template <int THREADS, int BATCH = kResolveBatch>
 __device__ __forceinline__ void pf_bn_resolve(const pf_bn_job& J, int s, float* sm_scale, float* sm_shift,
                                               double* red) {
   const int tid = threadIdx.x;
@@ -31,12 +31,12 @@
   if (sl < slices) {
     const double2* base = reinterpret_cast<const double2*>(J.partials) + (int64_t)s * per_stat * J.pcols + J.col0 + c;
     const int r0 = sl * per, r1 = min(per_stat, r0 + per);
-    for (int r = r0; r < r1; r += kResolveBatch) {
-      double2 v[kResolveBatch];
+    for (int r = r0; r < r1; r += BATCH) {
+      double2 v[BATCH];
 #pragma unroll
-      for (int u = 0; u < kResolveBatch; ++u) v[u] = base[(int64_t)min(r + u, r1 - 1) * J.pcols];
+      for (int u = 0; u < BATCH; ++u) v[u] = base[(int64_t)min(r + u, r1 - 1) * J.pcols];
 #pragma unroll
-      for (int u = 0; u < kResolveBatch; ++u) {
+      for (int u = 0; u < BATCH; ++u) {
         a += (r + u < r1) ? v[u].x : 0.0;
         b += (r + u < r1) ? v[u].y : 0.0;
       }
diff --git a/pointmvsnet_amd/model.py b/pointmvsnet_amd/model.py
--- a/pointmvsnet_amd/model.py
+++ b/pointmvsnet_amd/model.py
@@ -359,7 +359,11 @@
             pointflow.stamp("flow_tower_end")
             for p in pyramids.values():
                 if isinstance(p, pointflow.RawLevel):
-                    for t in (p.raw,) + (tuple(pointflow.affine_rows(p.affine)) if p.affine is not None else ()):
+                    if isinstance(p.affine, pointflow.LazyAffine):
+                        held = tuple(t for t in p.affine.keep if t.is_cuda)
+                    else:
+                        held = tuple(p.affine) if p.affine is not None else ()
+                    for t in (p.raw,) + held:
                         t.record_stream(main)
                 else:
                     p.record_stream(main)
diff --git a/pointmvsnet_amd/networks.py b/pointmvsnet_amd/networks.py
--- a/pointmvsnet_amd/networks.py
+++ b/pointmvsnet_amd/networks.py
@@ -212,7 +212,7 @@
             wanted = stage_end and name in need
             as_raw = wanted and name in raw and B == 1 and (nconv is None or pointflow.conv2d_wide_preferred(nconv))
             defer = (as_raw or not wanted) and nconv is not None and pointflow.conv2d_wide_preferred(nconv)
-            lazy = bool(defer) and not as_raw
+            lazy = bool(defer)
             conv = block.conv if hasattr(block, "bn") else block
             cl = (wanted and name in channel_last and not hasattr(block, "bn") and conv.out_channels >= 32
                   and pointflow.conv2d_wide_preferred(conv))
@@ -258,10 +258,16 @@
             y, partials = pointflow.conv2d_wide_sets(x, convs, pending, 1, has_bn, interleaved=(i == 1),
                                                      channel_last_sets=(0,) if last else ())
         raw_level = stage_end and name != "conv0"
-        pending = pointflow.bn_affine_rows_sets(y, [cb.bn, fb.bn], 1, partials, lazy=not raw_level,
+        pending = pointflow.bn_affine_rows_sets(y, [cb.bn, fb.bn], 1, partials, lazy=True,
                                                 interleaved=(i == 0)) if has_bn else None
         if raw_level:
-            levels[name] = pointflow.RawLevel(y[V:], None if pending is None else pending.rows_of(1))
+            if pending is None:
+                aff = None
+            elif pending.lazies is not None:
+                aff = pending.lazies[1]
+            else:
+                aff = pending.rows_of(1)
+            levels[name] = pointflow.RawLevel(y[V:], aff)
         x = y
     C = x.shape[1]
     return x[:V].view(1, V, x.shape[2], x.shape[3], C), levels
diff --git a/pointmvsnet_amd/pointflow.py b/pointmvsnet_amd/pointflow.py
--- a/pointmvsnet_amd/pointflow.py
+++ b/pointmvsnet_amd/pointflow.py
@@ -880,6 +880,28 @@
     if join is not None:
         torch.cuda.current_stream().wait_stream(join)
     rows4 = None
+    Tw = int(_lib.load().pf_edge_wide_blocks(int(G), int(Ng)))
+    if (training and keep is None and LAZY_BN and groups_per_stat * Tw * C <= LAZY_MAX_ELEMS
+            and (part_l is None or groups_per_stat * part_l.shape[1] * C <= LAZY_MAX_ELEMS)):
+        part_d = stat_rows(G, Tw, C, dev)
+        gather_bytes = float(G) * Ng * (4.0 * C + (1.0 if codes is not None else 8.0) * k + 4.0 * C * k)
+        _lib.call("pf_edge_stats_wide_f32", _lib.ptr(LE), 2 * C, C, _lib.ptr(idx), k, G, Ng, _lib.ptr(part_d),
+                  _lib.ptr(codes), lat[0], lat[1], lat[2], _lib.stream(), algo_bytes=gather_bytes)
+        held = (part_l, part_d, scale, shift) + _bn_tensors(bn)
+        zc = None
+        if concat:
+            zc = LazyAffine(bn_job(bn, part_l, 0, C, float(groups_per_stat) * Ng, n_pairs, G, groups_per_stat, scale,
+                                   shift), held, scale, shift)
+            zd = LazyAffine(bn_job(bn, part_d, 0, C, n_pairs, n_pairs, G, groups_per_stat, scale[:, C:], shift[:, C:],
+                                   ch0=C), held, scale, shift)
+        else:
+            zd = LazyAffine(bn_job(bn, part_d, 0, C, n_pairs, n_pairs, G, groups_per_stat, scale, shift, ch0=0), held,
+                            scale, shift)
+        bump_counter(bn, S)
+        _lib.call("pf_edge_apply_bn_f32", _lib.ptr(LE), 2 * C, C, _lib.ptr(idx), k, G, Ng,
+                  None if zc is None else zc.job_ptr(), zd.job_ptr(), groups_per_stat, _lib.ptr(Y), int(ldy),
+                  _lib.ptr(codes), lat[0], lat[1], lat[2], _lib.stream(), algo_bytes=gather_bytes + 4.0 * G * Ng * cbn)
+        return Y
     if training:
         T = stat_blocks(G, Ng)
         part_d = stat_rows(G, T, C, dev)
@@ -1045,7 +1067,8 @@
 
 def flow_pyramid(pyramid, h, w):
     maps = [(m.raw if isinstance(m, RawLevel) else m) for m in pyramid]
-    rows = [(affine_rows(m.affine) if isinstance(m, RawLevel) else None) for m in pyramid]
+    lazy = [isinstance(m, RawLevel) and isinstance(m.affine, LazyAffine) and not m.affine.done for m in pyramid]
+    rows = [(affine_rows(m.affine) if isinstance(m, RawLevel) and not z else None) for m, z in zip(pyramid, lazy)]
     V = maps[0].shape[0]
     outs = [torch.empty((V, h, w, int(m.shape[1])), dtype=_F32, device=m.device) for m in maps]
     args = []
@@ -1055,8 +1078,15 @@
     if any(r is not None for r in rows):
         sc = (ctypes.c_void_p * 3)(*[None if r is None else r[0].data_ptr() for r in rows])
         sh = (ctypes.c_void_p * 3)(*[None if r is None else r[1].data_ptr() for r in rows])
+    nbytes = sum(4.0 * m.numel() + 4.0 * o.numel() for m, o in zip(maps, outs))
+    if any(lazy):
+        JobP = ctypes.POINTER(_lib.BnJob)
+        jobs = (JobP * 3)(*[(m.affine.job_ptr() if z else JobP()) for m, z in zip(pyramid, lazy)])
+        _lib.call("pf_flow_pyramid_bn_f32", *args, V, h, w, _lib.ptr(outs[0]), _lib.ptr(outs[1]), _lib.ptr(outs[2]), sc,
+                  sh, jobs, _lib.stream(), algo_bytes=nbytes)
+        return outs
     _lib.call("pf_flow_pyramid_f32", *args, V, h, w, _lib.ptr(outs[0]), _lib.ptr(outs[1]), _lib.ptr(outs[2]), sc, sh,
-              _lib.stream(), algo_bytes=sum(4.0 * m.numel() + 4.0 * o.numel() for m, o in zip(maps, outs)))
+              _lib.stream(), algo_bytes=nbytes)
     return outs
 
 
```

Result: slower. 1062 (-3.0%).
